# saninsteinn/django-assistant-bot

Measured on AMD Instinct MI355X. Metric: RAG queries/sec + p50 end-to-end latency, bge-base + Llama-3-8B, 1/2/4/8 MI355X, higher is better.
Workload: dtype bf16; 1 GPU; model=bge-base-en + llama-3-8b, global_batch=128, seq_len=1090, parallelism=dp1, mode=batch, index_rows=1000000, index=single shard, local top-k (no collective), sampling=temperature=1.0 top_k=50 top_p=0.95 ignore_eos, graphs=True

## Files before the change

### django_assistant_bot_amd/csrc/bindings.cpp

```cpp
#include <hip/hip_runtime.h>
#include <pybind11/numpy.h>
#include <pybind11/pybind11.h>
#include <pybind11/stl.h>

#include <stdexcept>
#include <string>

#include "kernels/launchers.h"
#include "runtime/json_grammar.h"
#include "runtime/kv_manager.h"
#include "runtime/rag.h"
#include "runtime/tokenizer.h"
#include "runtime/trace.h"

namespace py = pybind11;
using u = uintptr_t;

#define VP(x) reinterpret_cast<void*>(x)
#define CVP(x) reinterpret_cast<const void*>(x)
#define ST(x) reinterpret_cast<hipStream_t>(x)

static void check(int err, const char* name) {
  if (err) throw std::runtime_error(std::string("dab kernel '") + name + "' failed: " + hipGetErrorString((hipError_t)err));
}

PYBIND11_MODULE(_native, m) {
  m.doc() = "MI355X (gfx950) kernels and native runtime of django_assistant_bot_amd";
  m.def("roctx_available", &dab::trace::available);
  m.def("allreduce_signal_bytes", &dab::allreduce_signal_bytes);
  m.def("custom_allreduce", [](const std::vector<uintptr_t>& bases, int rank, u data, long nbytes, long half_bytes,
                               long spin_limit, u s) {
    check(dab::custom_allreduce(bases, rank, VP(data), nbytes, half_bytes, spin_limit, ST(s)), "custom_allreduce");
  });
  m.def("custom_allreduce_rmsnorm", [](const std::vector<uintptr_t>& bases, int rank, u slabs, int S, long slab_stride,
                                       u x, u res_in, u res_out, u out, u w, int rows, int cols, float eps,
                                       long half_bytes, long spin_limit, u s) {
    check(dab::custom_allreduce_rmsnorm(bases, rank, (const float*)slabs, S, slab_stride, CVP(x), CVP(res_in),
                                        VP(res_out), VP(out), CVP(w), rows, cols, eps, half_bytes, spin_limit, ST(s)),
          "custom_allreduce_rmsnorm");
  });
  m.def("allreduce_buffer_alloc", [](long bytes, bool uncached) {
    uintptr_t p = 0;
    check(dab::allreduce_buffer_alloc(bytes, uncached ? 1 : 0, &p), "allreduce_buffer_alloc");
    return p;
  }, py::arg("bytes"), py::arg("uncached") = true);
  m.def("allreduce_buffer_free", [](u ptr) { check(dab::allreduce_buffer_free(ptr), "allreduce_buffer_free"); });
  m.def("ipc_get_handle", [](u ptr) {
    std::string h;
    check(dab::ipc_get_handle(ptr, &h), "ipc_get_handle");
    return py::bytes(h);
  });
  m.def("ipc_open_handle", [](const std::string& h) {
    uintptr_t p = 0;
    check(dab::ipc_open_handle(h, &p), "ipc_open_handle");
    return p;
  });
  m.def("ipc_probe", [](u ptr) { check(dab::ipc_probe(ptr), "ipc_probe"); });
  m.def("ipc_close_handle", [](u ptr) { check(dab::ipc_close_handle(ptr), "ipc_close_handle"); });
  m.def("allreduce_error", &dab::allreduce_error, py::arg("base"), py::arg("clear") = 1);
  m.def("allreduce_error_async", [](u base, u host_word, u s) {
    check(dab::allreduce_error_async(base, VP(host_word), ST(s)), "allreduce_error_async");
  });
  m.def("roctx_push", [](const std::string& name) { return dab::trace::range_push(name.c_str()); });
  m.def("roctx_pop", &dab::trace::range_pop);
  m.def("roctx_mark", [](const std::string& name) { dab::trace::mark(name.c_str()); });

  m.def("rmsnorm", [](u out, u res_out, u x, u res_in, u w, int rows, int cols, float eps, u s) {
    check(dab::rmsnorm(VP(out), VP(res_out), CVP(x), CVP(res_in), CVP(w), rows, cols, eps, ST(s)), "rmsnorm");
  });
  m.def("layernorm", [](u out, u x, u res_in, u gamma, u beta, int rows, int cols, float eps, u s) {
    check(dab::layernorm(VP(out), CVP(x), CVP(res_in), CVP(gamma), CVP(beta), rows, cols, eps, ST(s)), "layernorm");
  });
  m.def("bert_embed", [](u out, u ids, u pos_ids, u type_ids, u word, u pos, u type, u gamma, u beta, int rows, int cols,
                         float eps, u s) {
    check(dab::bert_embed(VP(out), (const int*)ids, (const int*)pos_ids, (const int*)type_ids, CVP(word), CVP(pos),
                          CVP(type), CVP(gamma), CVP(beta), rows, cols, eps, ST(s)),
          "bert_embed");
  });
  m.def("embed_gather", [](u out, u ids, u table, int rows, int cols, u s) {
    check(dab::embed_gather(VP(out), (const int*)ids, CVP(table), rows, cols, ST(s)), "embed_gather");
  });
  m.def("mean_pool", [](u out, u out_bf16, u hidden, u cu, int batch, int cols, int normalize, u s) {
    check(dab::mean_pool((float*)out, VP(out_bf16), CVP(hidden), (const int*)cu, batch, cols, normalize, ST(s)),
          "mean_pool");
  });
  m.def("gelu", [](u out, u x, u bias, size_t rows, int cols, u s) {
    check(dab::gelu(VP(out), CVP(x), CVP(bias), rows, cols, ST(s)), "gelu");
  });
  m.def("silu_mul", [](u out, u x, size_t rows, int F, u s, int interleaved) {
    check(dab::silu_mul(VP(out), CVP(x), rows, F, ST(s), interleaved), "silu_mul");
  }, py::arg("out"), py::arg("x"), py::arg("rows"), py::arg("F"), py::arg("s"), py::arg("interleaved") = 0);
  m.def("rope_kv_write", [](u qkv, int ld, u positions, u cos_sin, u q_out, u k_cache, u v_cache, u slots, int T,
                            int Hq, int Hkv, int D, int block_size, u s, u slabs, int S, long slab_stride,
                            int slab_bf16) {
    check(dab::rope_kv_write(CVP(qkv), ld, (const int*)positions, CVP(cos_sin), VP(q_out), VP(k_cache), VP(v_cache),
                             (const int64_t*)slots, T, Hq, Hkv, D, block_size, ST(s), CVP(slabs), S, slab_stride,
                             slab_bf16),
          "rope_kv_write");
  }, py::arg("qkv"), py::arg("ld"), py::arg("positions"), py::arg("cos_sin"), py::arg("q_out"), py::arg("k_cache"),
     py::arg("v_cache"), py::arg("slots"), py::arg("T"), py::arg("Hq"), py::arg("Hkv"), py::arg("D"),
     py::arg("block_size"), py::arg("s"), py::arg("slabs") = 0, py::arg("S") = 0, py::arg("slab_stride") = 0,
     py::arg("slab_bf16") = 0);
  m.def("rmsnorm_slabs", [](u out, u res_out, u slabs, int S, long slab_stride, u res_in, u w, int rows, int cols,
                            float eps, u s, int slab_bf16) {
    check(dab::rmsnorm_slabs(VP(out), VP(res_out), CVP(slabs), S, slab_stride, CVP(res_in), CVP(w), rows, cols, eps,
                             ST(s), slab_bf16),
          "rmsnorm_slabs");
  }, py::arg("out"), py::arg("res_out"), py::arg("slabs"), py::arg("S"), py::arg("slab_stride"), py::arg("res_in"),
     py::arg("w"), py::arg("rows"), py::arg("cols"), py::arg("eps"), py::arg("s"), py::arg("slab_bf16") = 0);
  m.def("flash_attention",
        [](u q, long qst, long qsh, u k, u v, long kvst, long kvsh, u kc, u vc, u bt, int max_blocks, int bs, u out,
           long ost, long osh, u cu_q, u cu_k, u ctx_k, int batch, int max_sq, int Hq, int Hkv, int D, int causal,
           int paged, float scale, u s) {
          check(dab::flash_attention(CVP(q), qst, qsh, CVP(k), CVP(v), kvst, kvsh, CVP(kc), CVP(vc), (const int*)bt,
                                     max_blocks, bs, VP(out), ost, osh, (const int*)cu_q, (const int*)cu_k,
                                     (const int*)ctx_k, batch, max_sq, Hq, Hkv, D, causal, paged, scale, ST(s)),
                "flash_attention");
        });
  m.def("flash_attention_rope",
        [](u q, long qst, long qsh, u kc, u vc, u bt, int max_blocks, int bs, u out, long ost, long osh, u cu_q,
           u ctx_k, int batch, int max_sq, int Hq, int Hkv, int D, int causal, float scale, u rope_pos, u rope_cs,
           u s) {
          check(dab::flash_attention(CVP(q), qst, qsh, nullptr, nullptr, 0, 0, CVP(kc), CVP(vc), (const int*)bt,
                                     max_blocks, bs, VP(out), ost, osh, (const int*)cu_q, nullptr, (const int*)ctx_k,
                                     batch, max_sq, Hq, Hkv, D, causal, 1, scale, ST(s), (const int*)rope_pos,
                                     CVP(rope_cs)),
                "flash_attention_rope");
        });
  m.def("create_cu_masked_stream", [](std::vector<uint32_t> mask) {
    hipStream_t st = nullptr;
    check(hipExtStreamCreateWithCUMask(&st, (uint32_t)mask.size(), mask.data()), "hipExtStreamCreateWithCUMask");
    return reinterpret_cast<uintptr_t>(st);
  });
  m.def("destroy_stream", [](u s) { check(hipStreamDestroy(ST(s)), "hipStreamDestroy"); });
  m.def("paged_decode_attention", [](u q, u kc, u vc, u bt, int max_blocks, int bs, u ctx, u out, u po, u pm, u pl,
                                     u cnt, int batch, int Hq, int Hkv, int D, int part_size, int max_parts,
                                     float scale, u s, u order, u w0, long w0_bytes, u w1, long w1_bytes,
                                     int w_blocks) {
    dab::L3Warm warm{{(const char*)w0, (const char*)w1}, {w0_bytes, w1_bytes}, w_blocks};
    check(dab::paged_decode_attention(CVP(q), CVP(kc), CVP(vc), (const int*)bt, max_blocks, bs, (const int*)ctx, VP(out),
                                      (float*)po, (float*)pm, (float*)pl, (int*)cnt, batch, Hq, Hkv, D, part_size,
                                      max_parts, scale, ST(s), (const int*)order, &warm),
          "paged_decode_attention");
  }, py::arg("q"), py::arg("kc"), py::arg("vc"), py::arg("bt"), py::arg("max_blocks"), py::arg("bs"), py::arg("ctx"),
     py::arg("out"), py::arg("po"), py::arg("pm"), py::arg("pl"), py::arg("cnt"), py::arg("batch"), py::arg("Hq"),
     py::arg("Hkv"), py::arg("D"), py::arg("part_size"), py::arg("max_parts"), py::arg("scale"), py::arg("s"),
     py::arg("order") = 0, py::arg("w0") = 0, py::arg("w0_bytes") = 0, py::arg("w1") = 0, py::arg("w1_bytes") = 0,
     py::arg("w_blocks") = 0);
  m.def("rope_kv_write_fp8", [](u qkv, int ld, u positions, u cos_sin, u q_out, u k_data, u k_exp, u v_data, u v_exp,
                                u slots, int T, int Hq, int Hkv, int D, int block_size, u s, u slabs, int S,
                                long slab_stride, int slab_bf16) {
    check(dab::rope_kv_write_fp8(CVP(qkv), ld, (const int*)positions, CVP(cos_sin), VP(q_out), VP(k_data), VP(k_exp),
                                 VP(v_data), VP(v_exp), (const int64_t*)slots, T, Hq, Hkv, D, block_size, ST(s),
                                 CVP(slabs), S, slab_stride, slab_bf16),
          "rope_kv_write_fp8");
  }, py::arg("qkv"), py::arg("ld"), py::arg("positions"), py::arg("cos_sin"), py::arg("q_out"), py::arg("k_data"),
     py::arg("k_exp"), py::arg("v_data"), py::arg("v_exp"), py::arg("slots"), py::arg("T"), py::arg("Hq"),
     py::arg("Hkv"), py::arg("D"), py::arg("block_size"), py::arg("s"), py::arg("slabs") = 0, py::arg("S") = 0,
     py::arg("slab_stride") = 0, py::arg("slab_bf16") = 0);
  m.def("kv_fp8_dequant_blocks", [](u k_data, u k_exp, u v_data, u v_exp, u ids, int n, u k_out, u v_out, int Hkv,
                                    int block_size, int D, u s) {
    check(dab::kv_fp8_dequant_blocks(CVP(k_data), CVP(k_exp), CVP(v_data), CVP(v_exp), (const int*)ids, n, VP(k_out),
                                     VP(v_out), Hkv, block_size, D, ST(s)),
          "kv_fp8_dequant_blocks");
  });
  m.def("paged_decode_attention_fp8", [](u q, u k_data, u k_exp, u v_data, u v_exp, u bt, int max_blocks, int bs, u ctx,
                                         u out, u po, u pm, u pl, u cnt, int batch, int Hq, int Hkv, int D,
                                         int part_size, int max_parts, float scale, u s, u order) {
    check(dab::paged_decode_attention_fp8(CVP(q), CVP(k_data), CVP(k_exp), CVP(v_data), CVP(v_exp), (const int*)bt,
                                          max_blocks, bs, (const int*)ctx, VP(out), (float*)po, (float*)pm, (float*)pl,
                                          (int*)cnt, batch, Hq, Hkv, D, part_size, max_parts, scale, ST(s),
                                          (const int*)order),
          "paged_decode_attention_fp8");
  });
  m.def("gemm_bt", [](u A, long lda, u B, long ldb, u C, long ldc, u bias, u residual, long ldr, int M, int N, int K,
                      int epilogue, int out_f32, u row_group, u q_group, u allow, int allow_words, u s, int b_rows,
                      int b_group) {
    check(dab::gemm_bt(CVP(A), lda, CVP(B), ldb, VP(C), ldc, CVP(bias), CVP(residual), ldr, M, N, K, epilogue, out_f32,
                       (const int*)row_group, (const int*)q_group, (const uint32_t*)allow, allow_words, ST(s), b_rows,
                       b_group),
          "gemm_bt");
  }, py::arg("A"), py::arg("lda"), py::arg("B"), py::arg("ldb"), py::arg("C"), py::arg("ldc"), py::arg("bias"),
     py::arg("residual"), py::arg("ldr"), py::arg("M"), py::arg("N"), py::arg("K"), py::arg("epilogue"),
     py::arg("out_f32"), py::arg("row_group"), py::arg("q_group"), py::arg("allow"), py::arg("allow_words"),
     py::arg("s"), py::arg("b_rows") = 0, py::arg("b_group") = 1);
  m.def("gemm_mid_ok", &dab::gemm_mid_ok);
  m.def("gemm_mid_slab_bytes", &dab::gemm_mid_slab_bytes);
  m.def("gemm_mid_counters", &dab::gemm_mid_counters);
  m.def("gemm_mid", [](u A, long lda, u B, u C, long ldc, u residual, long ldr, int M, int N, int K, int epilogue,
                       u slabs, long slab_bytes, u cnt, int n_cnt, u s, int variant, int b_group) {
    check(dab::gemm_mid(CVP(A), lda, CVP(B), VP(C), ldc, CVP(residual), ldr, M, N, K, epilogue, VP(slabs), slab_bytes,
                        (int*)cnt, n_cnt, ST(s), variant, b_group),
          "gemm_mid");
  }, py::arg("A"), py::arg("lda"), py::arg("B"), py::arg("C"), py::arg("ldc"), py::arg("residual"), py::arg("ldr"),
     py::arg("M"), py::arg("N"), py::arg("K"), py::arg("epilogue"), py::arg("slabs"), py::arg("slab_bytes"),
     py::arg("cnt"), py::arg("n_cnt"), py::arg("s"), py::arg("variant") = 0, py::arg("b_group") = 1);
  m.def("gemm256_ok", &dab::gemm256_ok);
  m.def("gemm256_stamped", [](u A, long lda, u B, u C, u bias, u residual, int M, int N, int K, int epilogue,
                              int b_shuf, u stamps, int stamp_tiles, u s, int store_aux) {
    const int r = dab::gemm256_stamped(CVP(A), lda, CVP(B), VP(C), CVP(bias), CVP(residual), M, N, K, epilogue, b_shuf,
                                       VP(stamps), stamp_tiles, ST(s), store_aux);
    if (r < 0) check(-r, "gemm256_stamped");
    return r;
  }, py::arg("A"), py::arg("lda"), py::arg("B"), py::arg("C"), py::arg("bias"), py::arg("residual"), py::arg("M"),
     py::arg("N"), py::arg("K"), py::arg("epilogue"), py::arg("b_shuf"), py::arg("stamps"), py::arg("stamp_tiles"),
     py::arg("s"), py::arg("store_aux") = 0);
  m.def("gemm256_candidates_stamped", [](u A, long lda, u B, int M, int N, int K, int b_rows, u thr, u cnt, u cand_val,
                                          u cand_idx, int cap, u stamps, int stamp_tiles, u s) {
    const int r = dab::gemm256_candidates_stamped(CVP(A), lda, CVP(B), M, N, K, b_rows, (const float*)thr, (int*)cnt,
                                                  (float*)cand_val, (int*)cand_idx, cap, VP(stamps), stamp_tiles, ST(s));
    if (r < 0) check(-r, "gemm256_candidates_stamped");
    return r;
  });
  m.def("gemm256", [](u A, long lda, u B, long ldb, u C, long ldc, u bias, u residual, long ldr, int M, int N, int K,
                      int epilogue, u s, int b_shuf, int b_group, u rows, int src_rows) {
    check(dab::gemm256(CVP(A), lda, CVP(B), ldb, VP(C), ldc, CVP(bias), CVP(residual), ldr, M, N, K, epilogue, ST(s),
                       b_shuf, b_group, reinterpret_cast<const int*>(rows), src_rows),
          "gemm256");
  }, py::arg("A"), py::arg("lda"), py::arg("B"), py::arg("ldb"), py::arg("C"), py::arg("ldc"), py::arg("bias"),
     py::arg("residual"), py::arg("ldr"), py::arg("M"), py::arg("N"), py::arg("K"), py::arg("epilogue"), py::arg("s"),
     py::arg("b_shuf") = 0, py::arg("b_group") = 1, py::arg("rows") = 0, py::arg("src_rows") = 0);
  m.def("gemm_score_candidates", [](u A, long lda, u B, long ldb, int M, int N, int K, u row_group, u q_group, u thr,
                                    u cnt, u cand_val, u cand_idx, int cap, u s) {
    check(dab::gemm_score_candidates(CVP(A), lda, CVP(B), ldb, M, N, K, reinterpret_cast<const int*>(row_group),
                                     reinterpret_cast<const int*>(q_group), reinterpret_cast<const float*>(thr),
                                     reinterpret_cast<int*>(cnt), reinterpret_cast<float*>(cand_val),
                                     reinterpret_cast<int*>(cand_idx), cap, ST(s)),
          "gemm_score_candidates");
  });
  m.def("score_candidates_shuf", [](u A, long lda, u Wshuf, int M, int N, int K, u row_group, u q_group, u thr,
                                    u cnt, u cand_val, u cand_idx, int cap, u s, int b_rows) {
    auto* rg = reinterpret_cast<const int*>(row_group);
    auto* qg = reinterpret_cast<const int*>(q_group);
    auto* th = reinterpret_cast<const float*>(thr);
    auto* ct = reinterpret_cast<int*>(cnt);
    auto* cv = reinterpret_cast<float*>(cand_val);
    auto* ci = reinterpret_cast<int*>(cand_idx);
    int rc = hipErrorInvalidValue;
    if (K % 256 == 0 && ((M <= 64 && K <= 1024) || (M <= 96 && K <= 768)))
      rc = dab::index_scan_candidates_shuf(CVP(A), lda, CVP(Wshuf), M, N, K, rg, qg, th, ct, cv, ci, cap, ST(s));
    else if (M <= 64 || K % 128)
      rc = dab::stream_score_candidates_shuf(CVP(A), lda, CVP(Wshuf), M, N, K, rg, qg, th, ct, cv, ci, cap, ST(s));
    else
      rc = dab::gemm_score_candidates(CVP(A), lda, CVP(Wshuf), K, M, N, K, rg, qg, th, ct, cv, ci, cap, ST(s), b_rows);
    check(rc, "score_candidates_shuf");
  }, py::arg("A"), py::arg("lda"), py::arg("Wshuf"), py::arg("M"), py::arg("N"), py::arg("K"), py::arg("row_group"),
     py::arg("q_group"), py::arg("thr"), py::arg("cnt"), py::arg("cand_val"), py::arg("cand_idx"), py::arg("cap"),
     py::arg("s"), py::arg("b_rows") = 0);
  m.def("stream_gemm", [](u X, long ldx, u W, long ldw, u out, long ldo, u residual, long ldr, int M, int N, int K,
                          int S, int epilogue, u s, int nt, int cfg, float norm_eps, int slab_bf16, int w_group) {
    check(dab::stream_gemm(CVP(X), ldx, CVP(W), ldw, VP(out), ldo, CVP(residual), ldr, M, N, K, S, epilogue, ST(s), nt,
                           cfg, norm_eps, slab_bf16, w_group),
          "stream_gemm");
  }, py::arg("X"), py::arg("ldx"), py::arg("W"), py::arg("ldw"), py::arg("out"), py::arg("ldo"), py::arg("residual"),
     py::arg("ldr"), py::arg("M"), py::arg("N"), py::arg("K"), py::arg("S"), py::arg("epilogue"), py::arg("s"),
     py::arg("nt"), py::arg("cfg"), py::arg("norm_eps") = 0.f, py::arg("slab_bf16") = 0, py::arg("w_group") = 1);
  m.def("stream_gemm_fp8", [](u X, long ldx, u W, u w_exps, u out, long ldo, u residual, long ldr, int M, int N, int K,
                              int S, int epilogue, u s, int nt, int cfg, float norm_eps, int slab_bf16, int w_group) {
    check(dab::stream_gemm_fp8(CVP(X), ldx, CVP(W), CVP(w_exps), VP(out), ldo, CVP(residual), ldr, M, N, K, S, epilogue,
                               ST(s), nt, cfg, norm_eps, slab_bf16, w_group),
          "stream_gemm_fp8");
  }, py::arg("X"), py::arg("ldx"), py::arg("W"), py::arg("w_exps"), py::arg("out"), py::arg("ldo"), py::arg("residual"),
     py::arg("ldr"), py::arg("M"), py::arg("N"), py::arg("K"), py::arg("S"), py::arg("epilogue"), py::arg("s"),
     py::arg("nt"), py::arg("cfg"), py::arg("norm_eps") = 0.f, py::arg("slab_bf16") = 0, py::arg("w_group") = 1);
  m.def("stream_gemm_fp8_ok", &dab::stream_gemm_fp8_ok);
  m.def("stream_gemm_fp8_nwin", &dab::stream_gemm_fp8_nwin);
  m.def("stream_gemm_fp8_set_deep", &dab::stream_gemm_fp8_set_deep);
  m.def("stream_gemm_fp8_deep", &dab::stream_gemm_fp8_deep);
  m.def("stream_gemm_bn", &dab::stream_gemm_bn);
  m.def("stream_gemm_max_m", &dab::stream_gemm_max_m);
  m.def("stream_gemm_set_slice_xcd", &dab::stream_gemm_set_slice_xcd);
  m.def("stream_gemm_slice_xcd", &dab::stream_gemm_slice_xcd);
  m.def("stream_gemm_shuffled", &dab::stream_gemm_shuffled);
  m.def("slab_reduce", [](u out, long ldo, u slabs, int S, int M, int N, u residual, long ldr, u s, int slab_bf16) {
    check(dab::slab_reduce(VP(out), ldo, CVP(slabs), S, M, N, CVP(residual), ldr, ST(s), slab_bf16), "slab_reduce");
  }, py::arg("out"), py::arg("ldo"), py::arg("slabs"), py::arg("S"), py::arg("M"), py::arg("N"), py::arg("residual"),
     py::arg("ldr"), py::arg("s"), py::arg("slab_bf16") = 0);
  m.def("sample_tokens", [](u logits, int f32, long ld, int rows, int vocab, u temp, u top_k, u top_p,
                            unsigned long long seed, u counters, u out_tokens, u out_logprobs, u s) {
    check(dab::sample_tokens(CVP(logits), f32, ld, rows, vocab, (const float*)temp, (const int*)top_k,
                             (const float*)top_p, seed, (int64_t*)counters, (int*)out_tokens, (float*)out_logprobs,
                             ST(s)),
          "sample_tokens");
  });
  m.def("topk_rows", [](u scores, long ld, int rows, int n, int k, u out_vals, u out_idx, long long base, u out_idx64,
                        u s) {
    check(dab::topk_rows((const float*)scores, ld, rows, n, k, (float*)out_vals, (int*)out_idx, base,
                         (int64_t*)out_idx64, ST(s)),
          "topk_rows");
  });

  m.def("sample_tokens_2stage", [](u logits, int f32, long ld, int rows, int vocab, u temp, u top_k, u top_p,
                                   unsigned long long seed, u counters, u out_tokens, u ws, size_t ws_bytes, u s) {
    check(dab::sample_tokens_2stage(CVP(logits), f32, ld, rows, vocab, (const float*)temp, (const int*)top_k,
                                    (const float*)top_p, seed, (int64_t*)counters, (int*)out_tokens, VP(ws), ws_bytes,
                                    ST(s)),
          "sample_tokens_2stage");
  });
  m.def("mask_logits", [](u logits, int f32, long ld, int rows, int vocab, u mask, int words, u row_flags, u s,
                          long mask_ld) {
    check(dab::mask_logits(VP(logits), f32, ld, rows, vocab, (const uint32_t*)mask, words, (const int*)row_flags,
                           ST(s), mask_ld),
          "mask_logits");
  });
  m.def("sample_candidates", [](u logits, int f32, long ld, int rows, int vocab, int base, u keys, u idx, int ncand,
                                u s) {
    check(dab::sample_candidates(CVP(logits), f32, ld, rows, vocab, base, (uint32_t*)keys, (int*)idx, ncand, ST(s)),
          "sample_candidates");
  });
  m.def("sample_merge", [](u keys, u idx, int ncand, int rows, int vocab, u temp, u top_k, u top_p,
                           unsigned long long seed, u counters, u out_tokens, u s) {
    check(dab::sample_merge((const uint32_t*)keys, (const int*)idx, ncand, rows, vocab, (const float*)temp,
                            (const int*)top_k, (const float*)top_p, seed, (int64_t*)counters, (int*)out_tokens, ST(s)),
          "sample_merge");
  });
  m.def("topk_rows_2stage", [](u scores, long ld, int rows, int n, int k, u out_vals, u out_idx, long long base,
                               u out_idx64, u ws, size_t ws_bytes, u s) {
    check(dab::topk_rows_2stage((const float*)scores, ld, rows, n, k, (float*)out_vals, (int*)out_idx, base,
                                (int64_t*)out_idx64, VP(ws), ws_bytes, ST(s)),
          "topk_rows_2stage");
  });

  py::class_<dab::TokenizerConfig>(m, "TokenizerConfig")
      .def(py::init<>())
      .def_readwrite("vocab_size", &dab::TokenizerConfig::vocab_size)
      .def_readwrite("first_id", &dab::TokenizerConfig::first_id)
      .def_readwrite("last_id", &dab::TokenizerConfig::last_id)
      .def_readwrite("pad_id", &dab::TokenizerConfig::pad_id)
      .def_readwrite("unk_id", &dab::TokenizerConfig::unk_id)
      .def_readwrite("cls_id", &dab::TokenizerConfig::cls_id)
      .def_readwrite("sep_id", &dab::TokenizerConfig::sep_id)
      .def_readwrite("max_word_chars", &dab::TokenizerConfig::max_word_chars);
  py::class_<dab::HashTokenizer>(m, "HashTokenizer")
      .def(py::init<const dab::TokenizerConfig&>())
      .def("encode", &dab::HashTokenizer::encode, py::arg("text"), py::arg("add_special") = true,
           py::arg("max_len") = 0)
      .def(
          "encode_batch",
          [](const dab::HashTokenizer& t, const std::vector<std::string>& texts, bool add_special, int max_len,
             int threads) {
            std::vector<int32_t> ids;
            std::vector<int64_t> offs;
            {
              py::gil_scoped_release rel;
              t.encode_batch(texts, add_special, max_len, threads, ids, offs);
            }
            py::array_t<int32_t> a(ids.size());
            std::copy(ids.begin(), ids.end(), a.mutable_data());
            py::array_t<int64_t> o(offs.size());
            std::copy(offs.begin(), offs.end(), o.mutable_data());
            return py::make_tuple(a, o);
          },
          py::arg("texts"), py::arg("add_special") = true, py::arg("max_len") = 0, py::arg("threads") = 8)
      .def("decode", &dab::HashTokenizer::decode, py::arg("ids"), py::arg("skip_special") = true)
      .def("token_texts",
           [](const dab::HashTokenizer& t) {
             py::list out;
             for (const auto& w : t.token_texts()) out.append(py::bytes(w));
             return out;
           })
      .def_static("count_words", &dab::HashTokenizer::count_words);

  py::class_<dab::JsonVocab, std::shared_ptr<dab::JsonVocab>>(m, "JsonVocab")
      .def(py::init([](const std::vector<py::bytes>& toks, const std::vector<int32_t>& eos) {
             std::vector<std::string> t;
             t.reserve(toks.size());
             for (const auto& b : toks) t.emplace_back(b);
             return std::make_shared<dab::JsonVocab>(t, eos);
           }),
           py::arg("tokens"), py::arg("eos_ids"))
      .def("vocab_size", &dab::JsonVocab::vocab_size)
      .def("words", &dab::JsonVocab::words)
      .def("trie_nodes", &dab::JsonVocab::trie_nodes)
      .def("cache_entries", &dab::JsonVocab::cache_entries);
  py::class_<dab::JsonMatcher>(m, "JsonMatcher")
      .def(py::init<std::shared_ptr<dab::JsonVocab>, int, int>(), py::arg("vocab"), py::arg("max_depth") = 24,
           py::arg("max_ws") = 8)
      .def("fill_mask",
           [](dab::JsonMatcher& j, int remaining, u out) {
             py::gil_scoped_release rel;
             return j.fill_mask(remaining, (uint32_t*)out);
           })
      .def("advance", &dab::JsonMatcher::advance)
      .def("done", &dab::JsonMatcher::done)
      .def("broken", &dab::JsonMatcher::broken)
      .def("completion", [](const dab::JsonMatcher& j) { return py::bytes(j.completion()); })
      .def("completion_len", &dab::JsonMatcher::completion_len)
      .def("text", [](const dab::JsonMatcher& j) { return py::bytes(j.text()); });
  py::class_<dab::SchemaAutomaton, std::shared_ptr<dab::SchemaAutomaton>>(m, "SchemaAutomaton")
      .def(py::init<std::shared_ptr<dab::JsonVocab>, int, int, const std::vector<int32_t>&,
                    const std::vector<std::vector<int32_t>>&, const std::vector<std::vector<int32_t>>&>(),
           py::arg("vocab"), py::arg("n_states"), py::arg("start"), py::arg("accept"), py::arg("edges"),
           py::arg("eps"))
      .def("dfa_states", &dab::SchemaAutomaton::dfa_states)
      .def("accepts", [](dab::SchemaAutomaton& a, const py::bytes& b) {
        int d = a.start();
        for (unsigned char c : std::string(b)) {
          d = a.step(d, c);
          if (d < 0) return false;
        }
        return a.accepting(d);
      });
  py::class_<dab::SchemaMatcher>(m, "SchemaMatcher")
      .def(py::init<std::shared_ptr<dab::SchemaAutomaton>>(), py::arg("automaton"))
      .def("fill_mask",
           [](dab::SchemaMatcher& j, int remaining, u out) {
             py::gil_scoped_release rel;
             return j.fill_mask(remaining, (uint32_t*)out);
           })
      .def("advance", &dab::SchemaMatcher::advance)
      .def("done", &dab::SchemaMatcher::done)
      .def("broken", &dab::SchemaMatcher::broken)
      .def("completion_len", &dab::SchemaMatcher::completion_len)
      .def("text", [](const dab::SchemaMatcher& j) { return py::bytes(j.text()); });
  m.def("json_accepts", [](const py::bytes& b, bool complete, int max_depth, int max_ws) {
    return dab::json_accepts(std::string(b), complete, max_depth, max_ws);
  }, py::arg("bytes"), py::arg("complete") = true, py::arg("max_depth") = 64, py::arg("max_ws") = 255);

  py::class_<dab::KVBlockManager>(m, "KVBlockManager")
      .def(py::init<int, int, bool>(), py::arg("num_blocks"), py::arg("block_size"), py::arg("prefix_cache") = true)
      .def("add_sequence", &dab::KVBlockManager::add_sequence)
      .def("extend", &dab::KVBlockManager::extend)
      .def("append_tokens", &dab::KVBlockManager::append_tokens)
      .def("commit_prefix", &dab::KVBlockManager::commit_prefix)
      .def("free_sequence", &dab::KVBlockManager::free_sequence)
      .def("has", &dab::KVBlockManager::has)
      .def("num_tokens", &dab::KVBlockManager::num_tokens)
      .def("capacity_tokens", &dab::KVBlockManager::capacity_tokens)
      .def("num_free_blocks", &dab::KVBlockManager::num_free_blocks)
      .def("num_blocks", &dab::KVBlockManager::num_blocks)
      .def("block_size", &dab::KVBlockManager::block_size)
      .def("prefix_hits", &dab::KVBlockManager::prefix_hits)
      .def("blocks", &dab::KVBlockManager::blocks)
      .def("slot_mapping_into",
           [](const dab::KVBlockManager& k, int64_t seq, int start, int n, u out) {
             k.slot_mapping(seq, start, n, (int64_t*)out);
           })
      .def("prepare_decode_into",
           [](dab::KVBlockManager& k, const std::vector<int64_t>& seqs, const std::vector<int32_t>& toks,
              int max_blocks, u ids, u pos, u slots, u ctx, u bt) {
             return k.prepare_decode(seqs, toks, max_blocks, (int32_t*)ids, (int32_t*)pos, (int64_t*)slots,
                                     (int32_t*)ctx, (int32_t*)bt);
           })
      .def("block_table_into", [](const dab::KVBlockManager& k, const std::vector<int64_t>& seqs, int max_blocks,
                                  u out) { k.block_table(seqs, max_blocks, (int32_t*)out); });

  m.def(
      "aggregate_documents",
      [](py::array_t<float, py::array::c_style | py::array::forcecast> dist,
         py::array_t<int64_t, py::array::c_style | py::array::forcecast> doc_ids, int max_scores_n, int top_n) {
        if (dist.size() != doc_ids.size()) throw std::invalid_argument("distances / doc_ids length mismatch");
        auto r = dab::aggregate_documents(dist.data(), doc_ids.data(), (int)dist.size(), max_scores_n, top_n);
        py::list out;
        for (auto& d : r) out.append(py::make_tuple(d.doc_id, d.score));
        return out;
      },
      py::arg("distances"), py::arg("doc_ids"), py::arg("max_scores_n"), py::arg("top_n"));
  m.def(
      "merge_topk",
      [](py::array_t<float, py::array::c_style | py::array::forcecast> vals,
         py::array_t<int64_t, py::array::c_style | py::array::forcecast> ids, int k_out) {
        if (vals.ndim() != 2 || ids.ndim() != 2 || vals.shape(0) != ids.shape(0) || vals.shape(1) != ids.shape(1))
          throw std::invalid_argument("vals / ids must be [S, k] arrays of the same shape");
        const int S = (int)vals.shape(0), k = (int)vals.shape(1);
        py::array_t<float> ov(k_out);
        py::array_t<int64_t> oi(k_out);
        dab::merge_topk(vals.data(), ids.data(), S, k, k_out, ov.mutable_data(), oi.mutable_data());
        return py::make_tuple(ov, oi);
      },
      py::arg("vals"), py::arg("ids"), py::arg("k_out"));
}
```

### django_assistant_bot_amd/csrc/kernels/launchers.h

```cpp
#pragma once
#include <hip/hip_runtime.h>
#include <stddef.h>
#include <stdint.h>

#include <string>
#include <vector>

namespace dab {

inline int div_up_host(int a, int b) { return (a + b - 1) / b; }

struct L3Warm {
  const char* ptr[2];
  long bytes[2];
  int blocks;
};

int rmsnorm(void* out, void* res_out, const void* x, const void* res_in, const void* w, int rows, int cols, float eps,
            hipStream_t s);
int rmsnorm_slabs(void* out, void* res_out, const void* slabs, int S, long slab_stride, const void* res_in,
                  const void* w, int rows, int cols, float eps, hipStream_t s, int slab_bf16 = 0);
int layernorm(void* out, const void* x, const void* res_in, const void* gamma, const void* beta, int rows, int cols,
              float eps, hipStream_t s);
int bert_embed(void* out, const int* ids, const int* pos_ids, const int* type_ids, const void* word, const void* pos,
               const void* type, const void* gamma, const void* beta, int rows, int cols, float eps, hipStream_t s);
int embed_gather(void* out, const int* ids, const void* table, int rows, int cols, hipStream_t s);
int mean_pool(float* out, void* out_bf16, const void* hidden, const int* cu_seqlens, int batch, int cols,
              int normalize, hipStream_t s);

int gelu(void* out, const void* x, const void* bias, size_t rows, int cols, hipStream_t s);
int silu_mul(void* out, const void* x, size_t rows, int F, hipStream_t s, int interleaved = 0);
int rope_kv_write(const void* qkv, int ld, const int* positions, const void* cos_sin, void* q_out, void* k_cache,
                  void* v_cache, const int64_t* slots, int T, int Hq, int Hkv, int D, int block_size, hipStream_t s,
                  const void* slabs = nullptr, int S = 0, long slab_stride = 0, int slab_bf16 = 0);

int flash_attention(const void* q, long q_stride_tok, long q_stride_head, const void* k, const void* v,
                    long kv_stride_tok, long kv_stride_head, const void* k_cache, const void* v_cache,
                    const int* block_tables, int max_blocks, int block_size, void* out, long o_stride_tok,
                    long o_stride_head, const int* cu_q, const int* cu_k, const int* ctx_k, int batch,
                    int max_seqlen_q, int Hq, int Hkv, int D, int causal, int paged, float scale, hipStream_t s,
                    const int* rope_pos = nullptr, const void* rope_cs = nullptr);
int paged_decode_attention(const void* q, const void* k_cache, const void* v_cache, const int* block_tables,
                           int max_blocks, int block_size, const int* ctx_lens, void* out, float* part_o,
                           float* part_m, float* part_l, int* counters, int batch, int Hq, int Hkv, int D,
                           int part_size, int max_parts, float scale, hipStream_t s,
                           const int* order = nullptr, const L3Warm* warm = nullptr);

int rope_kv_write_fp8(const void* qkv, int ld, const int* positions, const void* cos_sin, void* q_out, void* k_data,
                      void* k_exp, void* v_data, void* v_exp, const int64_t* slots, int T, int Hq, int Hkv, int D,
                      int block_size, hipStream_t s, const void* slabs = nullptr, int S = 0, long slab_stride = 0,
                      int slab_bf16 = 0);
int kv_fp8_dequant_blocks(const void* k_data, const void* k_exp, const void* v_data, const void* v_exp,
                          const int* block_ids, int n, void* k_out, void* v_out, int Hkv, int block_size, int D,
                          hipStream_t s);
int paged_decode_attention_fp8(const void* q, const void* k_data, const void* k_exp, const void* v_data,
                               const void* v_exp, const int* block_tables, int max_blocks, int block_size,
                               const int* ctx_lens, void* out, float* part_o, float* part_m, float* part_l,
                               int* counters, int batch, int Hq, int Hkv, int D, int part_size, int max_parts,
                               float scale, hipStream_t s, const int* order = nullptr);

int gemm_bt(const void* A, long lda, const void* B, long ldb, void* C, long ldc, const void* bias, const void* residual,
            long ldr, int M, int N, int K, int epilogue, int out_f32, const int* row_group, const int* q_group,
            const uint32_t* allow, int allow_words, hipStream_t s, int b_rows = 0, int b_group = 1);

int gemm256_ok(int M, int N, int K, long lda, long ldb);
int gemm256_candidates(const void* A, long lda, const void* B, long ldb, int M, int N, int K, const int* row_group,
                       const int* q_group, const float* thr, int* cnt, float* cand_val, int* cand_idx, int cap,
                       hipStream_t s, int b_rows = 0);
int gemm256_candidates_stamped(const void* A, long lda, const void* B, int M, int N, int K, int b_rows,
                               const float* thr, int* cnt, float* cand_val, int* cand_idx, int cap, void* stamps,
                               int stamp_tiles, hipStream_t s);
int gemm256_stamped(const void* A, long lda, const void* B, void* C, const void* bias, const void* residual, int M,
                    int N, int K, int epilogue, int b_shuf, void* stamps, int stamp_tiles, hipStream_t s, int store_aux);
int gemm256(const void* A, long lda, const void* B, long ldb, void* C, long ldc, const void* bias,
            const void* residual, long ldr, int M, int N, int K, int epilogue, hipStream_t s, int b_shuf = 0,
            int b_group = 1, const int* rows = nullptr, int src_rows = 0);

int gemm_mid_ok(int M, int N, int K, long lda);
long gemm_mid_slab_bytes();
int gemm_mid_counters(int M, int N);
int gemm_mid(const void* A, long lda, const void* B, void* C, long ldc, const void* residual, long ldr, int M, int N,
             int K, int epilogue, void* slabs, long slab_bytes, int* cnt, int n_cnt, hipStream_t s, int variant = 0,
             int b_group = 1);

int stream_gemm(const void* X, long ldx, const void* W, long ldw, void* out, long ldo, const void* residual, long ldr,
                int M, int N, int K, int S, int epilogue, hipStream_t s, int nt_weights, int cfg, float norm_eps = 0.f,
                int slab_bf16 = 0, int w_group = 1);
int stream_gemm_bn(int cfg);
int stream_gemm_fp8(const void* X, long ldx, const void* W, const void* w_exps, void* out, long ldo,
                    const void* residual, long ldr, int M, int N, int K, int S, int epilogue, hipStream_t s,
                    int nt_weights, int cfg, float norm_eps = 0.f, int slab_bf16 = 0, int w_group = 1);
int stream_gemm_fp8_ok(int cfg);
int stream_gemm_fp8_nwin(int cfg);
void stream_gemm_fp8_set_deep(int on);
int stream_gemm_fp8_deep();
int slab_reduce(void* out, long ldo, const void* slabs, int S, int M, int N, const void* residual, long ldr,
                hipStream_t s, int slab_bf16 = 0);
int index_scan_candidates(const void* X, long ldx, const void* W, long ldw, int M, int N, int K, const int* row_group,
                          const int* q_group, const float* thr, int* cnt, float* cand_val, int* cand_idx, int cap,
                          hipStream_t s);
int index_scan_candidates_shuf(const void* X, long ldx, const void* W, int M, int N, int K, const int* row_group,
                               const int* q_group, const float* thr, int* cnt, float* cand_val, int* cand_idx,
                               int cap, hipStream_t s);
int stream_score_candidates(const void* X, long ldx, const void* W, long ldw, int M, int N, int K, const int* row_group,
                            const int* q_group, const float* thr, int* cnt, float* cand_val, int* cand_idx, int cap,
                            hipStream_t s);
int stream_score_candidates_shuf(const void* X, long ldx, const void* W, int M, int N, int K, const int* row_group,
                                 const int* q_group, const float* thr, int* cnt, float* cand_val, int* cand_idx,
                                 int cap, hipStream_t s);
int stream_gemm_max_m(int cfg);
void stream_gemm_set_slice_xcd(int on);
int stream_gemm_slice_xcd();
int stream_gemm_shuffled(int cfg);

int mask_logits(void* logits, int logits_f32, long ld, int rows, int vocab, const uint32_t* mask, int words,
                const int* row_flags, hipStream_t s, long mask_ld = 0);
int sample_candidates(const void* logits, int logits_f32, long ld, int rows, int vocab, int index_base,
                      uint32_t* cand_key, int* cand_idx, int ncand, hipStream_t s);
int sample_merge(const uint32_t* cand_key, const int* cand_idx, int ncand, int rows, int vocab,
                 const float* temperature, const int* top_k, const float* top_p, unsigned long long seed,
                 int64_t* counters, int* out_tokens, hipStream_t s);
int sample_tokens(const void* logits, int logits_f32, long ld, int rows, int vocab, const float* temperature,
                  const int* top_k, const float* top_p, unsigned long long seed, int64_t* counters, int* out_tokens,
                  float* out_logprobs, hipStream_t s);
int topk_rows(const float* scores, long ld, int rows, int n, int k, float* out_vals, int* out_idx, int64_t index_base,
              int64_t* out_idx64, hipStream_t s);

int sample_tokens_2stage(const void* logits, int logits_f32, long ld, int rows, int vocab, const float* temperature,
                         const int* top_k, const float* top_p, unsigned long long seed, int64_t* counters,
                         int* out_tokens, void* workspace, size_t workspace_bytes, hipStream_t s);
int topk_rows_2stage(const float* scores, long ld, int rows, int n, int k, float* out_vals, int* out_idx,
                     int64_t index_base, int64_t* out_idx64, void* workspace, size_t workspace_bytes, hipStream_t s);

int gemm_score_candidates(const void* A, long lda, const void* B, long ldb, int M, int N, int K, const int* row_group,
                          const int* q_group, const float* thr, int* cnt, float* cand_val, int* cand_idx, int cap,
                          hipStream_t s, int b_rows = 0);

size_t allreduce_signal_bytes();
int custom_allreduce_rmsnorm(const std::vector<uintptr_t>& bases, int rank, const float* slabs, int S,
                             long slab_stride, const void* x, const void* res_in, void* res_out, void* out,
                             const void* w, int rows, int cols, float eps, long half_bytes, long spin_limit,
                             hipStream_t s);
int custom_allreduce(const std::vector<uintptr_t>& bases, int rank, void* data, long nbytes, long half_bytes,
                     long spin_limit, hipStream_t s);
int allreduce_buffer_alloc(long bytes, int uncached, uintptr_t* out);
int allreduce_buffer_free(uintptr_t ptr);
int ipc_get_handle(uintptr_t ptr, std::string* handle);
int ipc_open_handle(const std::string& handle, uintptr_t* out);
int ipc_close_handle(uintptr_t ptr);
int ipc_probe(uintptr_t ptr);
int allreduce_error(uintptr_t base, int clear);
int allreduce_error_async(uintptr_t base, void* host_word, hipStream_t s);

}
```

### django_assistant_bot_amd/csrc/kernels/select.hip

```cpp
#include "common.h"
#include "launchers.h"

namespace dab {

constexpr uint32_t kNegInfKey = 0x007FFFFFu;


constexpr int SEL_NT = 1024;
constexpr int SEL_MAXK = 1024;

struct SelShared {
  uint32_t hist[256];
  uint32_t bcast[4];
  uint32_t cnt_gt, cnt_eq;
  uint32_t cand_key[SEL_MAXK];
  int cand_idx[SEL_MAXK];
};

__device__ __forceinline__ int wave_append(uint32_t* counter, bool pred) {
  const unsigned long long m = __ballot(pred);
  if (!m) return -1;
  const int lane = threadIdx.x & 63;
  const int leader = __ffsll((long long)m) - 1;
  uint32_t base = 0;
  if (lane == leader) base = atomicAdd(counter, (uint32_t)__popcll(m));
  base = __shfl(base, leader, 64);
  const unsigned long long below = lane ? (m & ((1ull << lane) - 1ull)) : 0ull;
  return pred ? (int)(base + __popcll(below)) : -1;
}

template <class KeyAt>
__device__ uint32_t radix_kth(KeyAt key_at, int n, int k, SelShared& sh, uint32_t& ties_needed) {
  uint32_t prefix = 0, pmask = 0, kk = (uint32_t)k;
  const int tid = threadIdx.x, lane = tid & 63;
  for (int shift = 24; shift >= 0; shift -= 8) {
    for (int i = tid; i < 256; i += SEL_NT) sh.hist[i] = 0;
    __syncthreads();
    for (int i0 = 0; i0 < n; i0 += SEL_NT) {
      const int i = i0 + tid;
      int bin = -1;
      if (i < n) {
        const uint32_t key = key_at(i);
        if ((key & pmask) == prefix) bin = (int)((key >> shift) & 255u);
      }
      unsigned long long active = __ballot(bin >= 0);
      while (active) {
        const int leader = __ffsll((long long)active) - 1;
        const int lb = __shfl(bin, leader, 64);
        const unsigned long long eq = __ballot(bin == lb);
        if (lane == leader) atomicAdd(&sh.hist[lb], (uint32_t)__popcll(eq));
        active &= ~eq;
      }
    }
    __syncthreads();
    if (tid < 64) {
      uint32_t c[4], sum = 0;
#pragma unroll
      for (int j = 0; j < 4; ++j) {
        c[j] = sh.hist[255 - 4 * tid - j];
        sum += c[j];
      }
      uint32_t incl = sum;
#pragma unroll
      for (int o = 1; o < 64; o <<= 1) {
        const uint32_t t = __shfl_up(incl, o, 64);
        if (tid >= o) incl += t;
      }
      const uint32_t excl = incl - sum;
      if (excl < kk && kk <= incl) {
        uint32_t acc = excl;
#pragma unroll
        for (int j = 0; j < 4; ++j) {
          if (acc + c[j] >= kk) {
            sh.bcast[0] = 255u - 4u * tid - j;
            sh.bcast[1] = kk - acc;
            break;
          }
          acc += c[j];
        }
      }
    }
    __syncthreads();
    const uint32_t digit = sh.bcast[0];
    kk = sh.bcast[1];
    prefix |= digit << shift;
    pmask |= 255u << shift;
    __syncthreads();
  }
  ties_needed = kk;
  return prefix;
}

template <bool TIES_ALL = false, class KeyAt>
__device__ int select_topk(KeyAt key_at, int n, int k, SelShared& sh) {
  const int tid = threadIdx.x;
  uint32_t ties;
  const uint32_t kth = radix_kth(key_at, n, k, sh, ties);
  const uint32_t n_gt0 = (uint32_t)k - ties;
  if (TIES_ALL && kth > kNegInfKey) ties = (uint32_t)SEL_MAXK - n_gt0;
  if (tid == 0) {
    sh.cnt_gt = 0;
    sh.cnt_eq = 0;
  }
  __syncthreads();
  const uint32_t n_gt = n_gt0;
  for (int i0 = 0; i0 < n; i0 += SEL_NT) {
    const int i = i0 + tid;
    uint32_t key = 0;
    if (i < n) key = key_at(i);
    const int pg = wave_append(&sh.cnt_gt, i < n && key > kth);
    if (pg >= 0) {
      sh.cand_key[pg] = key;
      sh.cand_idx[pg] = i;
    }
    const int pe = wave_append(&sh.cnt_eq, i < n && key == kth);
    if (pe >= 0 && (uint32_t)pe < ties) {
      sh.cand_key[n_gt + pe] = key;
      sh.cand_idx[n_gt + pe] = i;
    }
  }
  __syncthreads();
  if (TIES_ALL) k = (int)(n_gt + min(sh.cnt_eq, ties));
  int P = 1;
  while (P < k) P <<= 1;
  for (int i = k + tid; i < P; i += SEL_NT) {
    sh.cand_key[i] = 0u;
    sh.cand_idx[i] = 0x7fffffff;
  }
  __syncthreads();
  for (int size = 2; size <= P; size <<= 1) {
    for (int stride = size >> 1; stride > 0; stride >>= 1) {
      for (int t = tid; t < P; t += SEL_NT) {
        const int u = t ^ stride;
        if (u > t) {
          const bool desc = (t & size) == 0;
          const uint32_t ka = sh.cand_key[t], kb = sh.cand_key[u];
          const int ia = sh.cand_idx[t], ib = sh.cand_idx[u];
          const bool a_first = ka > kb || (ka == kb && ia < ib);
          if (a_first != desc) {
            sh.cand_key[t] = kb;
            sh.cand_key[u] = ka;
            sh.cand_idx[t] = ib;
            sh.cand_idx[u] = ia;
          }
        }
      }
      __syncthreads();
    }
  }
  return k;
}

__device__ __forceinline__ unsigned long long splitmix64(unsigned long long x) {
  x += 0x9E3779B97F4A7C15ull;
  x = (x ^ (x >> 30)) * 0xBF58476D1CE4E5B9ull;
  x = (x ^ (x >> 27)) * 0x94D049BB133111EBull;
  return x ^ (x >> 31);
}

__global__ __launch_bounds__(SEL_NT) void sample_kernel(const void* __restrict__ logits, int logits_f32, long ld,
                                                        int vocab, const float* __restrict__ temperature,
                                                        const int* __restrict__ top_k,
                                                        const float* __restrict__ top_p, unsigned long long seed,
                                                        int64_t* __restrict__ counters, int* __restrict__ out_tokens,
                                                        float* __restrict__ out_logprobs) {
  __shared__ SelShared sh;
  __shared__ float probs[SEL_MAXK];
  const int row = blockIdx.x;
  const float T = temperature ? temperature[row] : 1.f;
  int k = (T <= 0.f) ? 1 : (top_k && top_k[row] > 0 ? top_k[row] : SEL_MAXK);
  if (k > SEL_MAXK) k = SEL_MAXK;
  if (k > vocab) k = vocab;
  const float P = top_p ? top_p[row] : 1.f;
  const bool f32 = logits_f32 != 0;
  const float* lf = reinterpret_cast<const float*>(logits) + (size_t)row * ld;
  const bf16* lb = reinterpret_cast<const bf16*>(logits) + (size_t)row * ld;
  auto key_at = [&](int i) -> uint32_t { return float_key(f32 ? lf[i] : bf2f(lb[i])); };
  k = select_topk<true>(key_at, vocab, k, sh);
  if (threadIdx.x != 0) return;
  if (T <= 0.f) {
    out_tokens[row] = sh.cand_idx[0];
    if (out_logprobs) out_logprobs[row] = 0.f;
    return;
  }
  const float x0 = key_float(sh.cand_key[0]) / T;
  float total = 0.f;
  for (int i = 0; i < k; ++i) {
    const float e = __expf(key_float(sh.cand_key[i]) / T - x0);
    probs[i] = e;
    total += e;
  }
  int keep = k;
  if (P < 1.f) {
    const float thr = (1.f - P) * total;
    float cum = 0.f;
    keep = k;
    for (int i = k - 1; i >= 1; --i) {
      cum += probs[i];
      if (cum <= thr) keep = i;
      else break;
    }
  }
  float kept = 0.f;
  for (int i = 0; i < keep; ++i) kept += probs[i];
  const long long c = counters ? counters[row] : 0;
  if (counters) counters[row] = c + 1;
  const unsigned long long r =
      splitmix64(seed ^ splitmix64((unsigned long long)c * 0x9E3779B97F4A7C15ull + (unsigned long long)row));
  const float u = (float)(r >> 40) * (1.f / 16777216.f);
  const float target = u * kept;
  float acc = 0.f;
  int pick = keep - 1;
  for (int i = 0; i < keep; ++i) {
    acc += probs[i];
    if (acc > target) {
      pick = i;
      break;
    }
  }
  out_tokens[row] = sh.cand_idx[pick];
  if (out_logprobs) out_logprobs[row] = __logf(probs[pick] / kept);
}

__global__ __launch_bounds__(SEL_NT) void topk_rows_kernel(const float* __restrict__ scores, long ld, int n, int k,
                                                           float* __restrict__ out_vals, int* __restrict__ out_idx,
                                                           int64_t index_base, int64_t* __restrict__ out_idx64) {
  __shared__ SelShared sh;
  const int row = blockIdx.x;
  const float* s = scores + (size_t)row * ld;
  auto key_at = [&](int i) -> uint32_t { return float_key(s[i]); };
  select_topk(key_at, n, k, sh);
  for (int i = threadIdx.x; i < k; i += SEL_NT) {
    out_vals[(size_t)row * k + i] = key_float(sh.cand_key[i]);
    if (out_idx) out_idx[(size_t)row * k + i] = sh.cand_idx[i];
    if (out_idx64) out_idx64[(size_t)row * k + i] = index_base + sh.cand_idx[i];
  }
}


constexpr int CH_NT = 256;
constexpr int CH_FAST_MAXK = 64;
constexpr int CH_FAST_CAP = 512;

struct ChunkFast {
  u32x4 tmax[CH_NT / 4];
  u32x4 kv[CH_FAST_CAP / 2];
  uint32_t n, thr;
};

template <int PT>
__global__ __launch_bounds__(CH_NT) void chunk_topk_kernel(const void* __restrict__ src, int src_bf16, long ld, int n,
                                                           int k, int kc, uint32_t* __restrict__ cand_key,
                                                           int* __restrict__ cand_idx, int index_base = 0) {
  __shared__ uint32_t hist[256];
  __shared__ uint32_t bc[2];
  __shared__ uint32_t cnt[2];
  __shared__ ChunkFast fst;
  const int row = blockIdx.y, c = blockIdx.x, nchunks = gridDim.x;
  const int chunk = CH_NT * PT;
  const int start = c * chunk;
  const int len = min(chunk, n - start);
  const int tid = threadIdx.x, lane = tid & 63;
  const float* sf = reinterpret_cast<const float*>(src) + (size_t)row * ld + start;
  const bf16* sb = reinterpret_cast<const bf16*>(src) + (size_t)row * ld + start;
  static_assert(CH_NT == 256 && PT % 8 == 0, "idx_of assumes 256 threads and whole 16-B vectors");
  const int lg = src_bf16 ? 3 : 2;
  auto idx_of = [&](int j) { return ((j >> lg) << (8 + lg)) + (tid << lg) + (j & ((1 << lg) - 1)); };
  const bool vec_ok = ((reinterpret_cast<uintptr_t>(src_bf16 ? (const void*)sb : (const void*)sf)) & 15) == 0;
  uint32_t key[PT];
  if (src_bf16) {
#pragma unroll
    for (int v = 0; v < PT / 8; ++v) {
      const int i0 = v * (CH_NT * 8) + tid * 8;
      if (vec_ok && i0 + 8 <= len) {
        float f[8];
        unpack8(*reinterpret_cast<const u32x4*>(sb + i0), f);
#pragma unroll
        for (int e = 0; e < 8; ++e) key[8 * v + e] = float_key(f[e]);
      } else {
#pragma unroll
        for (int e = 0; e < 8; ++e) key[8 * v + e] = i0 + e < len ? float_key(bf2f(sb[i0 + e])) : 0u;
      }
    }
  } else {
#pragma unroll
    for (int v = 0; v < PT / 4; ++v) {
      const int i0 = v * (CH_NT * 4) + tid * 4;
      if (vec_ok && i0 + 4 <= len) {
        const f32x4 f = *reinterpret_cast<const f32x4*>(sf + i0);
#pragma unroll
        for (int e = 0; e < 4; ++e) key[4 * v + e] = float_key(f[e]);
      } else {
#pragma unroll
        for (int e = 0; e < 4; ++e) key[4 * v + e] = i0 + e < len ? float_key(sf[i0 + e]) : 0u;
      }
    }
  }
  const int kk = min(k, len);
  uint32_t* ok = cand_key + ((size_t)row * nchunks + c) * kc;
  int* oi = cand_idx + ((size_t)row * nchunks + c) * kc;
  if (kk <= CH_FAST_MAXK) {
    uint32_t m = 0;
#pragma unroll
    for (int j = 0; j < PT; ++j)
      if (idx_of(j) < len) m = max(m, key[j]);
    reinterpret_cast<uint32_t*>(fst.tmax)[tid] = m;
    if (tid == 0) fst.n = 0;
    __syncthreads();
    int rank = 0;
#pragma unroll 4
    for (int j4 = 0; j4 < CH_NT / 4; ++j4) {
      const u32x4 o4 = fst.tmax[j4];
#pragma unroll
      for (int e = 0; e < 4; ++e) rank += (o4[e] > m) || (o4[e] == m && 4 * j4 + e < tid);
    }
    if (rank == kk - 1) fst.thr = m;
    __syncthreads();
    const uint32_t t = fst.thr;
#pragma unroll
    for (int j = 0; j < PT; ++j) {
      const int i = idx_of(j);
      const int slot = wave_append(&fst.n, i < len && key[j] >= t);
      if (slot >= 0 && slot < CH_FAST_CAP) {
        uint32_t* e2 = reinterpret_cast<uint32_t*>(fst.kv) + 2 * slot;
        e2[0] = key[j];
        e2[1] = (uint32_t)(index_base + start + i);
      }
    }
    __syncthreads();
    const int ns = (int)fst.n;
    if (ns <= CH_FAST_CAP) {
      const int ns8 = min(CH_FAST_CAP, (ns + 7) & ~7);
      if (tid < ns8 - ns) {
        uint32_t* e2 = reinterpret_cast<uint32_t*>(fst.kv) + 2 * (ns + tid);
        e2[0] = 0u;
        e2[1] = 0xffffffffu;
      }
      __syncthreads();
      for (int a = tid; a < ns; a += CH_NT) {
        const uint32_t* ea = reinterpret_cast<const uint32_t*>(fst.kv) + 2 * a;
        const uint32_t ka = ea[0], ia = ea[1];
        int r = 0;
        for (int u2 = 0; u2 < ns8 / 2; u2 += 4) {
          u32x4 q[4];
#pragma unroll
          for (int z = 0; z < 4; ++z) q[z] = fst.kv[u2 + z];
#pragma unroll
          for (int z = 0; z < 4; ++z) {
            r += (q[z][0] > ka) || (q[z][0] == ka && q[z][1] < ia);
            r += (q[z][2] > ka) || (q[z][2] == ka && q[z][3] < ia);
          }
        }
        if (r < kk) {
          ok[r] = ka;
          oi[r] = (int)ia;
        }
      }
      for (int i = kk + tid; i < kc; i += CH_NT) {
        ok[i] = 0u;
        oi[i] = -1;
      }
      return;
    }
    __syncthreads();
  }
  uint32_t prefix = 0, pmask = 0, need = (uint32_t)kk;
  for (int shift = 24; shift >= 0; shift -= 8) {
    for (int i = tid; i < 256; i += CH_NT) hist[i] = 0;
    __syncthreads();
#pragma unroll
    for (int j = 0; j < PT; ++j) {
      const int i = idx_of(j);
      const int bin = (i < len && (key[j] & pmask) == prefix) ? (int)((key[j] >> shift) & 255u) : -1;
      const int b0 = __builtin_amdgcn_readfirstlane(bin);
      if (__all(bin == b0)) {
        if (lane == 0 && b0 >= 0) atomicAdd(&hist[b0], 64u);
      } else if (bin >= 0) {
        atomicAdd(&hist[bin], 1u);
      }
    }
    __syncthreads();
    if (tid < 64) {
      uint32_t cc[4], sum = 0;
#pragma unroll
      for (int j = 0; j < 4; ++j) {
        cc[j] = hist[255 - 4 * tid - j];
        sum += cc[j];
      }
      uint32_t incl = sum;
#pragma unroll
      for (int o = 1; o < 64; o <<= 1) {
        const uint32_t t = __shfl_up(incl, o, 64);
        if (tid >= o) incl += t;
      }
      const uint32_t excl = incl - sum;
      if (excl < need && need <= incl) {
        uint32_t acc = excl;
#pragma unroll
        for (int j = 0; j < 4; ++j) {
          if (acc + cc[j] >= need) {
            bc[0] = 255u - 4u * tid - j;
            bc[1] = need - acc;
            break;
          }
          acc += cc[j];
        }
      }
    }
    __syncthreads();
    prefix |= bc[0] << shift;
    pmask |= 255u << shift;
    need = bc[1];
    __syncthreads();
  }
  if (tid == 0) {
    cnt[0] = 0;
    cnt[1] = 0;
  }
  __syncthreads();
  const uint32_t n_gt = (uint32_t)kk - need;
#pragma unroll
  for (int j = 0; j < PT; ++j) {
    const int i = idx_of(j);
    const bool valid = i < len;
    const int pg = wave_append(&cnt[0], valid && key[j] > prefix);
    if (pg >= 0) {
      ok[pg] = key[j];
      oi[pg] = index_base + start + i;
    }
    const int pe = wave_append(&cnt[1], valid && key[j] == prefix);
    if (pe >= 0 && (uint32_t)pe < need) {
      ok[n_gt + pe] = key[j];
      oi[n_gt + pe] = index_base + start + i;
    }
  }
  for (int i = kk + tid; i < kc; i += CH_NT) {
    ok[i] = 0u;
    oi[i] = -1;
  }
}

__global__ __launch_bounds__(SEL_NT) void sample_merge_kernel(const uint32_t* __restrict__ cand_key,
                                                              const int* __restrict__ cand_idx, int ncand,
                                                              const float* __restrict__ temperature,
                                                              const int* __restrict__ top_k,
                                                              const float* __restrict__ top_p, int vocab,
                                                              unsigned long long seed, int64_t* __restrict__ counters,
                                                              int* __restrict__ out_tokens) {
  __shared__ uint32_t skey[SEL_MAXK];
  __shared__ int sidx[SEL_MAXK];
  __shared__ float probs[SEL_MAXK];
  const int row = blockIdx.x, tid = threadIdx.x;
  const float T = temperature ? temperature[row] : 1.f;
  int k = (T <= 0.f) ? 1 : (top_k && top_k[row] > 0 ? top_k[row] : 64);
  k = min(k, min(64, vocab));
  const int nc = min(ncand, SEL_MAXK);
  for (int i = tid; i < SEL_MAXK; i += SEL_NT) {
    skey[i] = i < ncand ? cand_key[(size_t)row * ncand + i] : 0u;
    sidx[i] = i < ncand ? cand_idx[(size_t)row * ncand + i] : 0x7fffffff;
  }
  __syncthreads();
  for (int size = 2; size <= SEL_MAXK; size <<= 1) {
    for (int stride = size >> 1; stride > 0; stride >>= 1) {
      for (int t = tid; t < SEL_MAXK; t += SEL_NT) {
        const int u2 = t ^ stride;
        if (u2 > t) {
          const bool desc = (t & size) == 0;
          const uint32_t ka = skey[t], kb = skey[u2];
          const int ia = sidx[t], ib = sidx[u2];
          const bool a_first = ka > kb || (ka == kb && ia < ib);
          if (a_first != desc) {
            skey[t] = kb;
            skey[u2] = ka;
            sidx[t] = ib;
            sidx[u2] = ia;
          }
        }
      }
      __syncthreads();
    }
  }
  if (tid != 0) return;
  if (T <= 0.f) {
    out_tokens[row] = sidx[0];
    return;
  }
  while (k < nc && skey[k] == skey[k - 1] && skey[k] > kNegInfKey) ++k;
  const float P = top_p ? top_p[row] : 1.f;
  const float x0 = key_float(skey[0]) / T;
  float total = 0.f;
  for (int i = 0; i < k; ++i) {
    const float e = __expf(key_float(skey[i]) / T - x0);
    probs[i] = e;
    total += e;
  }
  int keep = k;
  if (P < 1.f) {
    const float thr = (1.f - P) * total;
    float cum = 0.f;
    for (int i = k - 1; i >= 1; --i) {
      cum += probs[i];
      if (cum <= thr) keep = i;
      else break;
    }
  }
  float kept = 0.f;
  for (int i = 0; i < keep; ++i) kept += probs[i];
  const long long cval = counters ? counters[row] : 0;
  if (counters) counters[row] = cval + 1;
  const unsigned long long r =
      splitmix64(seed ^ splitmix64((unsigned long long)cval * 0x9E3779B97F4A7C15ull + (unsigned long long)row));
  const float uu = (float)(r >> 40) * (1.f / 16777216.f);
  const float target = uu * kept;
  float acc = 0.f;
  int pick = keep - 1;
  for (int i = 0; i < keep; ++i) {
    acc += probs[i];
    if (acc > target) {
      pick = i;
      break;
    }
  }
  out_tokens[row] = sidx[pick];
}

__global__ __launch_bounds__(SEL_NT) void topk_merge_kernel(const uint32_t* __restrict__ cand_key,
                                                            const int* __restrict__ cand_idx, int ncand, int k,
                                                            float* __restrict__ out_vals, int* __restrict__ out_idx,
                                                            int64_t index_base, int64_t* __restrict__ out_idx64) {
  __shared__ SelShared sh;
  const int row = blockIdx.x;
  const uint32_t* ck = cand_key + (size_t)row * ncand;
  const int* ci = cand_idx + (size_t)row * ncand;
  auto key_at = [&](int i) -> uint32_t { return ck[i]; };
  select_topk(key_at, ncand, k, sh);
  for (int i = threadIdx.x; i < k; i += SEL_NT) {
    const int pos = sh.cand_idx[i];
    const int idx = (pos >= 0 && pos < ncand) ? ci[pos] : -1;
    out_vals[(size_t)row * k + i] = key_float(sh.cand_key[i]);
    if (out_idx) out_idx[(size_t)row * k + i] = idx;
    if (out_idx64) out_idx64[(size_t)row * k + i] = idx >= 0 ? index_base + idx : -1;
  }
}

int sample_tokens_2stage(const void* logits, int logits_f32, long ld, int rows, int vocab, const float* temperature,
                         const int* top_k, const float* top_p, unsigned long long seed, int64_t* counters,
                         int* out_tokens, void* workspace, size_t workspace_bytes, hipStream_t s) {
  if (rows <= 0) return 0;
  constexpr int PT = 32, KC = 64;
  const int chunk = CH_NT * PT;
  const int nchunks = (vocab + chunk - 1) / chunk;
  const int ncand = nchunks * KC;
  const size_t need = (size_t)rows * ncand * 8;
  if (ncand > SEL_MAXK || workspace_bytes < need) return hipErrorInvalidValue;
  uint32_t* ck = reinterpret_cast<uint32_t*>(workspace);
  int* ci = reinterpret_cast<int*>(ck + (size_t)rows * ncand);
  hipLaunchKernelGGL(chunk_topk_kernel<PT>, dim3(nchunks, rows), dim3(CH_NT), 0, s, logits, logits_f32 ? 0 : 1, ld,
                     vocab, KC, KC, ck, ci);
  hipLaunchKernelGGL(sample_merge_kernel, dim3(rows), dim3(SEL_NT), 0, s, ck, ci, ncand, temperature, top_k, top_p,
                     vocab, seed, counters, out_tokens);
  return hipGetLastError();
}

int sample_candidates(const void* logits, int logits_f32, long ld, int rows, int vocab, int index_base,
                      uint32_t* cand_key, int* cand_idx, int ncand, hipStream_t s) {
  if (rows <= 0) return 0;
  constexpr int PT = 32, KC = 64;
  const int nchunks = (vocab + CH_NT * PT - 1) / (CH_NT * PT);
  if (vocab <= 0 || ncand != nchunks * KC) return hipErrorInvalidValue;
  hipLaunchKernelGGL(chunk_topk_kernel<PT>, dim3(nchunks, rows), dim3(CH_NT), 0, s, logits, logits_f32 ? 0 : 1, ld,
                     vocab, KC, KC, cand_key, cand_idx, index_base);
  return hipGetLastError();
}

int sample_merge(const uint32_t* cand_key, const int* cand_idx, int ncand, int rows, int vocab,
                 const float* temperature, const int* top_k, const float* top_p, unsigned long long seed,
                 int64_t* counters, int* out_tokens, hipStream_t s) {
  if (rows <= 0) return 0;
  if (ncand <= 0 || ncand > SEL_MAXK) return hipErrorInvalidValue;
  hipLaunchKernelGGL(sample_merge_kernel, dim3(rows), dim3(SEL_NT), 0, s, cand_key, cand_idx, ncand, temperature, top_k,
                     top_p, vocab, seed, counters, out_tokens);
  return hipGetLastError();
}

int topk_rows_2stage(const float* scores, long ld, int rows, int n, int k, float* out_vals, int* out_idx,
                     int64_t index_base, int64_t* out_idx64, void* workspace, size_t workspace_bytes, hipStream_t s) {
  if (rows <= 0) return 0;
  if (k < 1 || k > SEL_MAXK || k > n) return hipErrorInvalidValue;
  constexpr int PT = 32;
  const int chunk = CH_NT * PT;
  const int kc = ((k + 63) / 64) * 64;
  const int nchunks = (n + chunk - 1) / chunk;
  const int ncand = nchunks * kc;
  if (workspace_bytes < (size_t)rows * ncand * 8) return hipErrorInvalidValue;
  uint32_t* ck = reinterpret_cast<uint32_t*>(workspace);
  int* ci = reinterpret_cast<int*>(ck + (size_t)rows * ncand);
  hipLaunchKernelGGL(chunk_topk_kernel<PT>, dim3(nchunks, rows), dim3(CH_NT), 0, s, scores, 0, ld, n, k, kc, ck, ci);
  hipLaunchKernelGGL(topk_merge_kernel, dim3(rows), dim3(SEL_NT), 0, s, ck, ci, ncand, k, out_vals, out_idx,
                     index_base, out_idx64);
  return hipGetLastError();
}

__global__ __launch_bounds__(256) void mask_logits_kernel(void* __restrict__ logits, int logits_f32, long ld,
                                                          int vocab, const uint32_t* __restrict__ mask, int words,
                                                          long mask_ld, const int* __restrict__ row_flags) {
  const int row = blockIdx.y;
  if (row_flags[row] == 0) return;
  const int w = blockIdx.x * 256 + threadIdx.x;
  if (w >= words) return;
  const uint32_t bits = mask[(size_t)row * mask_ld + w];
  if (bits == 0xFFFFFFFFu) return;
  const int t0 = w * 32, n = min(32, vocab - t0);
  if (logits_f32) {
    float* l = reinterpret_cast<float*>(logits) + (size_t)row * ld + t0;
    for (int j = 0; j < n; ++j)
      if (!((bits >> j) & 1u)) l[j] = -INFINITY;
  } else {
    bf16* l = reinterpret_cast<bf16*>(logits) + (size_t)row * ld + t0;
    for (int j = 0; j < n; ++j)
      if (!((bits >> j) & 1u)) l[j] = f2bf(-INFINITY);
  }
}

int mask_logits(void* logits, int logits_f32, long ld, int rows, int vocab, const uint32_t* mask, int words,
                const int* row_flags, hipStream_t s, long mask_ld) {
  if (rows <= 0) return 0;
  if (mask_ld <= 0) mask_ld = words;
  if (vocab <= 0 || words * 32 < vocab || mask_ld < words) return hipErrorInvalidValue;
  hipLaunchKernelGGL(mask_logits_kernel, dim3((words + 255) / 256, rows), dim3(256), 0, s, logits, logits_f32, ld,
                     vocab, mask, words, mask_ld, row_flags);
  return hipGetLastError();
}

int sample_tokens(const void* logits, int logits_f32, long ld, int rows, int vocab, const float* temperature,
                  const int* top_k, const float* top_p, unsigned long long seed, int64_t* counters, int* out_tokens,
                  float* out_logprobs, hipStream_t s) {
  if (rows <= 0) return 0;
  if (vocab <= 0) return hipErrorInvalidValue;
  hipLaunchKernelGGL(sample_kernel, dim3(rows), dim3(SEL_NT), 0, s, logits, logits_f32, ld, vocab, temperature, top_k,
                     top_p, seed, counters, out_tokens, out_logprobs);
  return hipGetLastError();
}

int topk_rows(const float* scores, long ld, int rows, int n, int k, float* out_vals, int* out_idx, int64_t index_base,
              int64_t* out_idx64, hipStream_t s) {
  if (rows <= 0) return 0;
  if (k < 1 || k > SEL_MAXK || k > n) return hipErrorInvalidValue;
  hipLaunchKernelGGL(topk_rows_kernel, dim3(rows), dim3(SEL_NT), 0, s, scores, ld, n, k, out_vals, out_idx, index_base,
                     out_idx64);
  return hipGetLastError();
}

}
```

### django_assistant_bot_amd/csrc/runtime/kv_manager.cpp

```cpp
#include "kv_manager.h"

#include <algorithm>
#include <functional>
#include <iterator>
#include <stdexcept>

namespace dab {

KVBlockManager::KVBlockManager(int num_blocks, int block_size, bool prefix_cache)
    : num_blocks_(num_blocks), block_size_(block_size), prefix_cache_(prefix_cache) {
  if (num_blocks <= 0 || block_size <= 0) throw std::invalid_argument("num_blocks and block_size must be > 0");
  free_.reserve(num_blocks);
  for (int b = 0; b < num_blocks; ++b) free_.push_back(b);
  lru_cap_ = std::max(64, num_blocks / 4);
  ref_.assign(num_blocks, 0);
  block_hash_.assign(num_blocks, 0);
  lru_pos_.resize(num_blocks);
  in_lru_.assign(num_blocks, 0);
}

uint64_t KVBlockManager::chain_hash(uint64_t parent, const int32_t* toks, int n) const {
  uint64_t h = parent ^ 0x9E3779B97F4A7C15ull;
  for (int i = 0; i < n; ++i) {
    h ^= (uint64_t)(uint32_t)toks[i] + 0x9E3779B97F4A7C15ull + (h << 6) + (h >> 2);
    h *= 0x100000001B3ull;
  }
  return h ? h : 1;
}

int32_t KVBlockManager::alloc_block() {
  int32_t b;
  if (!free_.empty()) {
    std::pop_heap(free_.begin(), free_.end(), std::greater<int32_t>());
    b = free_.back();
    free_.pop_back();
  } else if (!lru_.empty()) {
    b = lru_.front();
    lru_.pop_front();
    in_lru_[b] = 0;
    cached_.erase(block_hash_[b]);
    block_hash_[b] = 0;
  } else {
    return -1;
  }
  ref_[b] = 1;
  return b;
}

void KVBlockManager::release_block(int32_t b) {
  if (--ref_[b] > 0) return;
  if (prefix_cache_ && block_hash_[b] != 0) {
    lru_.push_back(b);
    lru_pos_[b] = std::prev(lru_.end());
    in_lru_[b] = 1;
    if ((int)lru_.size() > lru_cap_) {
      const int32_t e = lru_.front();
      lru_.pop_front();
      in_lru_[e] = 0;
      cached_.erase(block_hash_[e]);
      block_hash_[e] = 0;
      push_free(e);
    }
  } else {
    block_hash_[b] = 0;
    push_free(b);
  }
}

void KVBlockManager::push_free(int32_t b) {
  free_.push_back(b);
  std::push_heap(free_.begin(), free_.end(), std::greater<int32_t>());
}

int KVBlockManager::add_sequence(int64_t seq_id, const std::vector<int32_t>& tokens, int reserve) {
  if (seqs_.count(seq_id)) throw std::invalid_argument("sequence already registered");
  const int n = (int)tokens.size();
  const int need_tokens = n + (reserve > 0 ? reserve : 0);
  const int need_blocks = (need_tokens + block_size_ - 1) / block_size_;
  std::vector<int32_t> hit_blocks;
  std::vector<uint64_t> hit_hashes;
  if (prefix_cache_ && n > 1) {
    const int max_full = (n - 1) / block_size_;
    uint64_t h = 0;
    for (int i = 0; i < max_full; ++i) {
      h = chain_hash(h, tokens.data() + (size_t)i * block_size_, block_size_);
      auto it = cached_.find(h);
      if (it == cached_.end()) break;
      hit_blocks.push_back(it->second);
      hit_hashes.push_back(h);
    }
  }
  int reused_from_lru = 0;
  for (int32_t b : hit_blocks) reused_from_lru += in_lru_[b] ? 1 : 0;
  const int fresh = need_blocks - (int)hit_blocks.size();
  if (fresh > num_free_blocks() - reused_from_lru) return -1;
  Seq s;
  for (int32_t b : hit_blocks) {
    if (in_lru_[b]) {
      lru_.erase(lru_pos_[b]);
      in_lru_[b] = 0;
    }
    ++ref_[b];
    s.blocks.push_back(b);
  }
  s.hashes = hit_hashes;
  for (int i = 0; i < fresh; ++i) s.blocks.push_back(alloc_block());
  s.tokens = tokens;
  const int cached_tokens = (int)hit_blocks.size() * block_size_;
  prefix_hits_ += cached_tokens;
  seqs_.emplace(seq_id, std::move(s));
  return cached_tokens;
}

bool KVBlockManager::extend(int64_t seq_id, int n) {
  auto it = seqs_.find(seq_id);
  if (it == seqs_.end()) throw std::invalid_argument("unknown sequence");
  Seq& s = it->second;
  const int need = (int)s.tokens.size() + n;
  const int need_blocks = (need + block_size_ - 1) / block_size_;
  const int more = need_blocks - (int)s.blocks.size();
  if (more <= 0) return true;
  if (more > num_free_blocks()) return false;
  for (int i = 0; i < more; ++i) s.blocks.push_back(alloc_block());
  return true;
}

void KVBlockManager::append_tokens(int64_t seq_id, const std::vector<int32_t>& tokens) {
  auto it = seqs_.find(seq_id);
  if (it == seqs_.end()) throw std::invalid_argument("unknown sequence");
  Seq& s = it->second;
  s.tokens.insert(s.tokens.end(), tokens.begin(), tokens.end());
  if ((int)s.tokens.size() > (int)s.blocks.size() * block_size_) throw std::runtime_error("KV capacity exceeded");
}

void KVBlockManager::commit_prefix(int64_t seq_id, int n_computed) {
  if (!prefix_cache_) return;
  auto it = seqs_.find(seq_id);
  if (it == seqs_.end()) return;
  Seq& s = it->second;
  const int full = std::min<int>(n_computed, (int)s.tokens.size()) / block_size_;
  uint64_t h = s.hashes.empty() ? 0 : s.hashes.back();
  for (int i = (int)s.hashes.size(); i < full && i < (int)s.blocks.size(); ++i) {
    h = chain_hash(h, s.tokens.data() + (size_t)i * block_size_, block_size_);
    s.hashes.push_back(h);
    const int32_t b = s.blocks[i];
    if (block_hash_[b] == 0 && !cached_.count(h)) {
      block_hash_[b] = h;
      cached_[h] = b;
    }
  }
}

void KVBlockManager::free_sequence(int64_t seq_id) {
  auto it = seqs_.find(seq_id);
  if (it == seqs_.end()) return;
  for (int32_t b : it->second.blocks) release_block(b);
  seqs_.erase(it);
}

int KVBlockManager::num_tokens(int64_t seq_id) const {
  auto it = seqs_.find(seq_id);
  return it == seqs_.end() ? 0 : (int)it->second.tokens.size();
}

int KVBlockManager::capacity_tokens(int64_t seq_id) const {
  auto it = seqs_.find(seq_id);
  return it == seqs_.end() ? 0 : (int)it->second.blocks.size() * block_size_;
}

const std::vector<int32_t>& KVBlockManager::blocks(int64_t seq_id) const {
  auto it = seqs_.find(seq_id);
  if (it == seqs_.end()) throw std::invalid_argument("unknown sequence");
  return it->second.blocks;
}

void KVBlockManager::slot_mapping(int64_t seq_id, int start, int n, int64_t* out) const {
  const auto& bl = blocks(seq_id);
  for (int i = 0; i < n; ++i) {
    const int pos = start + i;
    const int bi = pos / block_size_;
    if (bi >= (int)bl.size()) throw std::out_of_range("slot beyond allocated blocks");
    out[i] = (int64_t)bl[bi] * block_size_ + (pos % block_size_);
  }
}

int KVBlockManager::prepare_decode(const std::vector<int64_t>& seq_ids, const std::vector<int32_t>& tokens,
                                   int max_blocks, int32_t* ids, int32_t* pos, int64_t* slots, int32_t* ctx,
                                   int32_t* block_table) {
  if (seq_ids.size() != tokens.size()) throw std::invalid_argument("seq_ids / tokens length mismatch");
  for (size_t i = 0; i < seq_ids.size(); ++i)
    if (!extend(seq_ids[i], 1)) return (int)i;
  for (size_t i = 0; i < seq_ids.size(); ++i) {
    Seq& s = seqs_.at(seq_ids[i]);
    s.tokens.push_back(tokens[i]);
    const int p = (int)s.tokens.size() - 1;
    ids[i] = tokens[i];
    pos[i] = p;
    slots[i] = (int64_t)s.blocks[p / block_size_] * block_size_ + (p % block_size_);
    ctx[i] = p + 1;
    if ((int)s.blocks.size() > max_blocks) throw std::out_of_range("block table wider than max_blocks");
    int32_t* row = block_table + i * (size_t)max_blocks;
    std::copy(s.blocks.begin(), s.blocks.end(), row);
    std::fill(row + s.blocks.size(), row + max_blocks, 0);
  }
  return -1;
}

void KVBlockManager::block_table(const std::vector<int64_t>& seq_ids, int max_blocks, int32_t* out) const {
  for (size_t r = 0; r < seq_ids.size(); ++r) {
    int32_t* row = out + r * max_blocks;
    int i = 0;
    if (seq_ids[r] >= 0) {
      const auto& bl = blocks(seq_ids[r]);
      if ((int)bl.size() > max_blocks) throw std::out_of_range("block table wider than max_blocks");
      for (; i < (int)bl.size(); ++i) row[i] = bl[i];
    }
    for (; i < max_blocks; ++i) row[i] = 0;
  }
}

}
```

### django_assistant_bot_amd/csrc/runtime/kv_manager.h

```cpp
#pragma once
#include <cstdint>
#include <list>
#include <unordered_map>
#include <vector>

namespace dab {

class KVBlockManager {
 public:
  KVBlockManager(int num_blocks, int block_size, bool prefix_cache);

  int add_sequence(int64_t seq_id, const std::vector<int32_t>& tokens, int reserve);
  bool extend(int64_t seq_id, int n);
  void append_tokens(int64_t seq_id, const std::vector<int32_t>& tokens);
  void commit_prefix(int64_t seq_id, int n_computed);
  void free_sequence(int64_t seq_id);

  bool has(int64_t seq_id) const { return seqs_.count(seq_id) != 0; }
  int num_tokens(int64_t seq_id) const;
  int capacity_tokens(int64_t seq_id) const;
  int num_free_blocks() const { return (int)free_.size() + (int)lru_.size(); }
  int num_blocks() const { return num_blocks_; }
  int block_size() const { return block_size_; }
  int64_t prefix_hits() const { return prefix_hits_; }
  const std::vector<int32_t>& blocks(int64_t seq_id) const;

  int prepare_decode(const std::vector<int64_t>& seq_ids, const std::vector<int32_t>& tokens, int max_blocks,
                     int32_t* ids, int32_t* pos, int64_t* slots, int32_t* ctx, int32_t* block_table);
  void slot_mapping(int64_t seq_id, int start, int n, int64_t* out) const;
  void block_table(const std::vector<int64_t>& seq_ids, int max_blocks, int32_t* out) const;

 private:
  struct Seq {
    std::vector<int32_t> blocks;
    std::vector<int32_t> tokens;
    std::vector<uint64_t> hashes;
  };
  int num_blocks_, block_size_;
  bool prefix_cache_;
  std::vector<int32_t> free_;
  int lru_cap_ = 64;
  std::vector<int32_t> ref_;
  std::vector<uint64_t> block_hash_;
  std::unordered_map<uint64_t, int32_t> cached_;
  std::list<int32_t> lru_;
  std::vector<std::list<int32_t>::iterator> lru_pos_;
  std::vector<char> in_lru_;
  std::unordered_map<int64_t, Seq> seqs_;
  int64_t prefix_hits_ = 0;

  int32_t alloc_block();
  void push_free(int32_t b);
  void release_block(int32_t b);
  uint64_t chain_hash(uint64_t parent, const int32_t* toks, int n) const;
};

}
```

### django_assistant_bot_amd/engine/llm_engine.py

```python
from __future__ import annotations

import itertools
import math
import os
import time
from collections import deque
from dataclasses import dataclass, field

import numpy as np
import torch

from .. import ops
from ..models import AttnMeta, KVCache, LlamaModel, decoder_config, random_decoder_weights
from ..models.configs import DecoderConfig
from ..ops._lib import native
from ..utils import trace
from .tokenizer import Tokenizer


@dataclass
class SamplingParams:
    max_new_tokens: int = 1024
    temperature: float = 1.0
    top_k: int = 50
    top_p: float = 0.95
    ignore_eos: bool = False
    max_length: int | None = None
    seed: int | None = None
    stop_token_ids: tuple = ()
    do_sample: bool = True
    timeout_s: float | None = None
    json_mode: bool = False
    json_schema: dict | str | None = None


@dataclass
class GenerationOutput:
    request_id: int
    prompt_ids: list
    token_ids: list
    text: str
    finish_reason: str
    usage: dict
    timings: dict


@dataclass
class _Req:
    rid: int
    prompt: list
    params: SamplingParams
    arrival: float
    out: list = field(default_factory=list)
    computed: int = 0
    admitted: bool = False
    first_token_t: float = 0.0
    finish_t: float = 0.0
    finish_reason: str = ""
    rng_base: int = 0
    prefill_s: float = 0.0
    preempted: int = 0
    matcher: object = None

    @property
    def seq(self):
        return self.rid

    def full_prompt(self):
        return self.prompt + self.out if self.preempted else self.prompt




def _bucket_sizes(max_batch):
    b = [1, 2, 4, 8, 16, 24, 32, 48, 64, 96, 128, 160, 192, 224, 256, 320, 384, 448, 512]
    return [x for x in b if x < max_batch] + [max_batch]


class LLMEngine:
    def __init__(self, model: str | DecoderConfig = "llama-3-8b", device=None, weights: dict | None = None,
                 checkpoint: str | None = None, seed: int = 0, max_batch: int = 256, block_size: int = 64,
                 max_model_len: int | None = None, kv_cache_gb: float | None = None, num_blocks: int | None = None,
                 max_prefill_tokens: int = 16384, use_graphs: bool = True, prefix_cache: bool = True,
                 tp_group=None, tp_size: int = 1, tp_rank: int = 0, interleaved_mlp: bool = True,
                 part_size: int = 512, kv_memory_fraction: float = 0.85, mixed_prefill_tokens: int = 0,
                 pipeline_decode: bool = True, shared_model: LlamaModel | None = None,
                 kv_cache_dtype: str | None = None, kv_scratch_blocks: int | None = None,
                 weight_dtype: str | None = None):
        self.cfg = decoder_config(model) if isinstance(model, str) else model
        cfg = self.cfg
        if shared_model is not None:
            have = getattr(shared_model, "weight_dtype", "bf16")
            if weight_dtype is not None and weight_dtype != have:
                raise ValueError(f"weight_dtype={weight_dtype!r} conflicts with the shared model's {have!r}")
            weight_dtype = have
        elif weight_dtype is None:
            weight_dtype = os.environ.get("DAB_WEIGHT_DTYPE") or "bf16"
        if weight_dtype not in ("bf16", "fp8"):
            raise ValueError(f"weight_dtype must be 'bf16' or 'fp8', got {weight_dtype!r}")
        if weight_dtype == "fp8" and tp_size > 1:
            raise ValueError("weight_dtype='fp8' does not support tensor parallelism (tp_size > 1) yet")
        self.weight_dtype = weight_dtype
        if kv_cache_dtype is None:
            kv_cache_dtype = os.environ.get("DAB_KV_CACHE_DTYPE") or "bf16"
        if kv_cache_dtype not in ("bf16", "fp8"):
            raise ValueError(f"kv_cache_dtype must be 'bf16' or 'fp8', got {kv_cache_dtype!r}")
        if kv_cache_dtype == "fp8" and tp_size > 1:
            raise ValueError("kv_cache_dtype='fp8' does not support tensor parallelism (tp_size > 1) yet")
        self.kv_cache_dtype = kv_cache_dtype
        if checkpoint is None and weights is None and shared_model is None:
            from ..models.configs import checkpoint_dir

            checkpoint = checkpoint_dir(model)
        self.device = torch.device(device if device is not None else ("cuda" if torch.cuda.is_available() else "cpu"))
        self.is_gpu = self.device.type == "cuda"
        if kv_cache_dtype == "fp8" and self.is_gpu and cfg.head_dim != 128:
            raise ValueError(f"kv_cache_dtype='fp8' needs head_dim 128 on the GPU (model has {cfg.head_dim})")
        self.tp_group, self.tp_size, self.tp_rank = tp_group, tp_size, tp_rank
        own_weights = weights is None
        if shared_model is not None:
            weights = {}
        elif weights is None:
            if checkpoint:
                from ..models import load_decoder_checkpoint

                weights = load_decoder_checkpoint(checkpoint, cfg, tp_rank=tp_rank, tp_size=tp_size,
                                                  interleave_mlp=interleaved_mlp)
            else:
                weights = random_decoder_weights(cfg, self.device, seed=seed, tp_rank=tp_rank, tp_size=tp_size,
                                                 interleave_mlp=interleaved_mlp)
        if shared_model is not None:
            self.model = shared_model
        else:
            self.model = LlamaModel(cfg, weights, self.device, tp_group=tp_group, tp_size=tp_size,
                                    interleaved_mlp=interleaved_mlp, consume=own_weights, tp_rank=tp_rank,
                                    weight_dtype=weight_dtype)
        del weights
        if self.is_gpu and shared_model is None:
            torch.cuda.empty_cache()
        if tp_size > 1 and self.is_gpu and shared_model is None:
            from ..parallel.custom_allreduce import maybe_create

            self.model.custom_ar = maybe_create(tp_group, self.device, tp_size)
        self.tokenizer = Tokenizer.for_decoder(cfg, checkpoint)
        self.max_batch = max_batch
        self.block_size = block_size
        self.max_model_len = min(max_model_len or cfg.max_position, cfg.max_position)
        self.max_blocks_per_seq = math.ceil(self.max_model_len / block_size)
        self.max_prefill_tokens = max_prefill_tokens
        self.mixed_prefill_tokens = mixed_prefill_tokens
        self.part_size = part_size
        self.long_part_size = max(part_size, 2048)
        hkv = cfg.kv_heads // tp_size
        fp8 = kv_cache_dtype == "fp8"
        per_block = KVCache.bytes_per_block(cfg.layers, hkv, block_size, cfg.head_dim, kv_dtype=kv_cache_dtype)
        scratch = 0
        if fp8 and self.is_gpu:
            scratch = kv_scratch_blocks or (math.ceil(max(max_prefill_tokens, self.max_model_len) / block_size) + max_batch)
            scratch = max(int(scratch), self.max_blocks_per_seq)
        if num_blocks is None:
            if kv_cache_gb:
                num_blocks = int(kv_cache_gb * (1 << 30) // per_block)
            elif self.is_gpu:
                free, _ = torch.cuda.mem_get_info(self.device)
                free -= KVCache.scratch_bytes(scratch, hkv, block_size, cfg.head_dim)
                num_blocks = int(free * kv_memory_fraction // per_block)
            else:
                num_blocks = 4 * self.max_blocks_per_seq
            num_blocks = max(2, min(num_blocks, max_batch * self.max_blocks_per_seq + 8))
        self.kv = KVCache(cfg.layers, num_blocks, hkv, block_size, cfg.head_dim, self.device, kv_dtype=kv_cache_dtype,
                          scratch_blocks=scratch)
        self.blocks = native().KVBlockManager(num_blocks, block_size, prefix_cache)
        self._prefix_cache = prefix_cache
        self.seed = seed
        self.waiting: deque[_Req] = deque()
        self.prefilling: list[_Req] = []
        self.running: list[_Req] = []
        self.finished: dict[int, _Req] = {}
        self._ids = itertools.count()
        self.stats = {"prefill_tokens": 0, "decode_tokens": 0, "decode_steps": 0, "prefill_steps": 0,
                      "preemptions": 0, "graph_replays": 0, "mixed_steps": 0,
                      "kv_cache_bits": 8 if fp8 else 16,
                      "weight_bits": 8 if weight_dtype == "fp8" else 16}
        self.use_graphs = use_graphs and self.is_gpu
        dev = self.device
        mb = max_batch
        self._d_ids = torch.zeros(mb, dtype=torch.int32, device=dev)
        self._d_pos = torch.zeros(mb, dtype=torch.int32, device=dev)
        self._d_slots = torch.full((mb,), -1, dtype=torch.int64, device=dev)
        self._d_ctx = torch.ones(mb, dtype=torch.int32, device=dev)
        self._d_bt = torch.zeros((mb, self.max_blocks_per_seq), dtype=torch.int32, device=dev)
        self._d_temp = torch.ones(mb, dtype=torch.float32, device=dev)
        self._d_topk = torch.full((mb,), 50, dtype=torch.int32, device=dev)
        self._d_topp = torch.ones(mb, dtype=torch.float32, device=dev)
        self._d_cnt = torch.zeros(mb, dtype=torch.int64, device=dev)
        self._d_tokens = torch.zeros(mb, dtype=torch.int32, device=dev)
        self._d_order = torch.arange(mb, dtype=torch.int32, device=dev)
        pin = self.is_gpu
        mk = lambda *a, **k: torch.zeros(*a, **k, pin_memory=pin)
        self._h_ids = mk(mb, dtype=torch.int32)
        self._h_pos = mk(mb, dtype=torch.int32)
        self._h_slots = mk(mb, dtype=torch.int64)
        self._h_ctx = mk(mb, dtype=torch.int32)
        self._h_bt = mk((mb, self.max_blocks_per_seq), dtype=torch.int32)
        self._h_temp = mk(mb, dtype=torch.float32)
        self._h_topk = mk(mb, dtype=torch.int32)
        self._h_topp = mk(mb, dtype=torch.float32)
        self._h_cnt = mk(mb, dtype=torch.int64)
        self._h_tokens = mk(mb, dtype=torch.int32)
        self._h_order = mk(mb, dtype=torch.int32)
        self.pipeline_decode = bool(pipeline_decode) and tp_size == 1
        self._h_alt = {k: mk(*(getattr(self, k).shape,), dtype=getattr(self, k).dtype)
                       for k in ("_h_ids", "_h_pos", "_h_slots", "_h_ctx", "_h_bt", "_h_temp", "_h_topk", "_h_topp",
                                 "_h_cnt", "_h_tokens", "_h_order")}
        self._inflight = None
        self._d_mask = None
        self._masked = False
        self._pending_prefill = None
        max_parts = math.ceil(self.max_model_len / part_size)
        self._workspace = ops.DecodeWorkspace(mb, cfg.heads // tp_size, cfg.head_dim, max_parts, dev) if self.is_gpu \
            else None
        self._sample_ws = ops.kernels.sample_workspace(mb, cfg.vocab_size, dev) if self.is_gpu else None
        self.vp = bool(getattr(self.model, "vocab_parallel", False))
        self._vp_cand = None
        if self.vp and self.is_gpu:
            ncl = ops.kernels.sample_candidates_per_row(self.model.vocab_local)
            self._vp_cand = torch.zeros((2, mb, ncl), dtype=torch.int32, device=dev)
        self._graphs: dict = {}
        self._buckets = _bucket_sizes(max_batch)
        self._graph_pool = None
        self.timer = trace.GpuTimer(enabled=self.is_gpu)
        self.fault_hook = None
        self.auto_expire = True

    def add_request(self, prompt_ids: list, params: SamplingParams | None = None, request_id: int | None = None) -> int:
        params = params or SamplingParams()
        rid = next(self._ids) if request_id is None else request_id
        prompt = [int(t) for t in prompt_ids]
        if not prompt:
            prompt = [self.cfg.bos_id]
        if len(prompt) >= self.max_model_len:
            prompt = prompt[-(self.max_model_len - 1):]
        seed = params.seed if params.seed is not None else self.seed
        r = _Req(rid, prompt, params, time.perf_counter(), rng_base=((seed * 1000003 + rid) & 0xFFFFFFFF) << 20)
        r.matcher = self.check_params(params, matcher=True)
        if r.matcher is not None:
            self._ensure_mask_buffers()
        self.waiting.append(r)
        return rid

    def check_params(self, params: SamplingParams, matcher: bool = False):
        if params.json_schema is not None and self.tokenizer.byte_exact:
            from .json_schema import automaton_for, matcher_for

            if not matcher:
                automaton_for(self.tokenizer, self.cfg.eos_ids, params.json_schema)
                return None
            return matcher_for(self.tokenizer, self.cfg.eos_ids, params.json_schema)
        if params.json_mode or params.json_schema is not None:
            from .json_constraint import matcher_for

            if params.json_schema is not None:
                from .json_schema import compile_schema

                compile_schema(params.json_schema)
            return matcher_for(self.tokenizer, self.cfg.eos_ids) if matcher else None
        return None

    def rejected_output(self, rid: int, prompt_ids, reason: str) -> GenerationOutput:
        return GenerationOutput(request_id=rid, prompt_ids=list(prompt_ids), token_ids=[], text="",
                                finish_reason=f"error: {reason}",
                                usage={"prompt_tokens": len(prompt_ids), "completion_tokens": 0,
                                       "total_tokens": len(prompt_ids)},
                                timings={"queue_s": 0.0, "ttft_s": 0.0, "total_s": 0.0, "decode_s": 0.0,
                                         "prefill_s": 0.0})

    def has_unfinished(self) -> bool:
        return bool(self.waiting or self.prefilling or self.running)

    def generate(self, prompts: list, params: SamplingParams | list | None = None) -> list[GenerationOutput]:
        plist = params if isinstance(params, list) else [params or SamplingParams()] * len(prompts)
        rids = []
        for p, sp in zip(prompts, plist):
            ids = self.tokenizer.encode(p) if isinstance(p, str) else p
            rids.append(self.add_request(ids, sp))
        while self.has_unfinished():
            self.step()
        return [self.pop_output(r) for r in rids]

    def pop_output(self, rid: int) -> GenerationOutput:
        r = self.finished.pop(rid)
        n_out = len(r.out)
        return GenerationOutput(
            request_id=rid, prompt_ids=r.prompt, token_ids=list(r.out),
            text=self.tokenizer.decode(r.out), finish_reason=r.finish_reason,
            usage={"prompt_tokens": len(r.prompt), "completion_tokens": n_out, "total_tokens": len(r.prompt) + n_out},
            timings={"queue_s": max(0.0, r.first_token_t - r.arrival - r.prefill_s),
                     "ttft_s": r.first_token_t - r.arrival, "total_s": r.finish_t - r.arrival,
                     "decode_s": r.finish_t - r.first_token_t, "prefill_s": r.prefill_s},
        )

    def step(self) -> list[int]:
        done_before = set(self.finished)
        if self.fault_hook is not None:
            self.fault_hook(self)
        if self.auto_expire:
            self.expire_deadlines()
        if self._pending_prefill is not None:
            chunks = self._schedule_prefill() if not self.running or self.mixed_prefill_tokens <= 0 else []
            if chunks:
                prev, self._pending_prefill = self._pending_prefill, None
                self._run_prefill(chunks)
                self._finish_prefill(prev)
                return [k for k in self.finished if k not in done_before]
            self._finish_prefill(self._pending_prefill)
            self._pending_prefill = None
        if self._inflight is not None and not self._can_pipeline():
            self._finish_inflight()
        if self._can_pipeline():
            self._step_pipelined()
        elif self.running and self.mixed_prefill_tokens > 0 and (self.waiting or self.prefilling):
            batch = self._reserve_decode()
            chunks = self._schedule_prefill(self.mixed_prefill_tokens) if batch else self._schedule_prefill()
            if chunks and batch:
                self._run_mixed(batch, chunks)
            elif chunks:
                self._run_prefill(chunks)
            elif batch:
                self._run_decode(batch)
        else:
            chunks = self._schedule_prefill()
            if chunks:
                self._run_prefill(chunks)
            elif self.running:
                batch = self._reserve_decode()
                if batch:
                    self._run_decode(batch)
        return [k for k in self.finished if k not in done_before]

    def abort(self, rid: int, reason: str = "abort") -> bool:
        if self._inflight is not None:
            self._finish_inflight()
        if self._pending_prefill is not None:
            pend, self._pending_prefill = self._pending_prefill, None
            self._finish_prefill(pend)
        for q in (self.waiting, self.prefilling, self.running):
            for r in q:
                if r.rid == rid:
                    q.remove(r)
                    if r.admitted:
                        self.blocks.free_sequence(r.seq)
                    r.finish_reason = reason
                    r.finish_t = time.perf_counter()
                    self.finished[rid] = r
                    self.stats["aborted"] = self.stats.get("aborted", 0) + 1
                    return True
        return False

    def fail_all(self) -> list[int]:
        ids = [r.rid for q in (self.waiting, self.prefilling, self.running) for r in q]
        self._inflight = None
        self._pending_prefill = None
        self.waiting.clear()
        self.prefilling.clear()
        self.running.clear()
        self.blocks = native().KVBlockManager(self.blocks.num_blocks(), self.block_size, self._prefix_cache)
        self.timer.collect()
        return ids

    def expired(self) -> list[int]:
        now = time.perf_counter()
        return [r.rid for q in (self.waiting, self.prefilling, self.running) for r in q
                if r.params.timeout_s is not None and now - r.arrival > r.params.timeout_s]

    def expire_deadlines(self) -> list[int]:
        ids = self.expired()
        for rid in ids:
            self.abort(rid, "timeout")
        return ids

    def _schedule_prefill(self, budget: int | None = None):
        budget = self.max_prefill_tokens if budget is None else budget
        chunks = []
        for r in self.prefilling:
            if budget <= 0:
                break
            total = len(r.full_prompt())
            n = min(total - r.computed, budget)
            if n > 0:
                chunks.append((r, r.computed, n))
                self.blocks.commit_prefix(r.seq, r.computed + n)
                budget -= n
        while self.waiting and budget > 0 and len(self.running) + len(self.prefilling) < self.max_batch:
            r = self.waiting[0]
            toks = r.full_prompt()
            cached = self.blocks.add_sequence(r.seq, toks, 1)
            if cached < 0:
                if not self.running and not self.prefilling:
                    raise RuntimeError("KV cache too small for a single request")
                break
            self.waiting.popleft()
            r.admitted = True
            r.computed = cached
            self.prefilling.append(r)
            n = min(len(toks) - cached, budget)
            chunks.append((r, cached, n))
            self.blocks.commit_prefix(r.seq, cached + n)
            budget -= n
        return chunks

    def _build_block_tables(self, seqs, out_host):
        self.blocks.block_table_into(seqs, self.max_blocks_per_seq, out_host.data_ptr())

    def _kv_prefill_plan(self, bt, ctx, cu) -> dict:
        if not (self.kv.fp8 and self.is_gpu):
            return {}
        p = ops.kv_prefill_plan(bt, ctx, cu, self.block_size, self.kv.scratch_blocks, self.device)
        return {"kv_blocks": p.blocks, "kv_scratch_bt": p.scratch_bt, "kv_groups": p.groups}

    def _run_prefill(self, chunks):
        t0 = time.perf_counter()
        B = len(chunks)
        T = sum(n for _, _, n in chunks)
        ids = np.empty(T, dtype=np.int32)
        pos = np.empty(T, dtype=np.int32)
        slots = torch.empty(T, dtype=torch.int64)
        cu = np.zeros(B + 1, dtype=np.int32)
        ctx = np.empty(B, dtype=np.int32)
        o = 0
        for i, (r, s, n) in enumerate(chunks):
            toks = r.full_prompt()
            ids[o:o + n] = toks[s:s + n]
            pos[o:o + n] = np.arange(s, s + n, dtype=np.int32)
            self.blocks.slot_mapping_into(r.seq, s, n, slots.data_ptr() + 8 * o)
            o += n
            cu[i + 1] = o
            ctx[i] = s + n
        bt = torch.zeros((B, self.max_blocks_per_seq), dtype=torch.int32)
        self._build_block_tables([r.seq for r, _, _ in chunks], bt)
        to = self._h2d
        meta = AttnMeta(decode=False, positions=to(pos), slots=to(slots), block_tables=to(bt), ctx_lens=to(ctx),
                        cu_q=to(cu), max_q=max(n for _, _, n in chunks), **self._kv_prefill_plan(bt, ctx, cu))
        last_rows = [i for i, (r, s, n) in enumerate(chunks) if s + n == len(r.full_prompt())]
        if last_rows:
            sel = self._h2d(torch.as_tensor([int(cu[i + 1]) - 1 for i in last_rows], dtype=torch.int32))
        else:
            sel = torch.empty(0, dtype=torch.int32, device=self.device)
        with self.timer.phase("prefill"):
            hidden = self.model.forward(to(ids), meta, self.kv, out_rows=sel)
        self.stats["prefill_tokens"] += T
        self.stats["prefill_steps"] += 1
        reqs, toks = [], []
        if last_rows:
            logits = self.model.logits(hidden)
            reqs = [chunks[i][0] for i in last_rows]
            toks = self._sample(logits, reqs, to_host=not self.is_gpu)
        for r, s, n in chunks:
            r.computed = s + n
            self.blocks.commit_prefix(r.seq, s + n)
        pend = (chunks, reqs, toks, t0)
        self._tp_fault_enqueue()
        if self.is_gpu:
            self._pending_prefill = pend
        else:
            self._finish_prefill(pend)

    def _finish_prefill(self, pend):
        chunks, reqs, toks, t0 = pend
        if torch.is_tensor(toks):
            toks = toks.cpu().tolist()
            self._tp_fault_check()
        self._collect_gpu_times(block=bool(reqs))
        now = time.perf_counter()
        for r, s, n in chunks:
            r.prefill_s += now - t0
        if reqs:
            for r, t in zip(reqs, toks):
                self.blocks.commit_prefix(r.seq, len(r.full_prompt()))
                self.prefilling.remove(r)
                r.first_token_t = r.first_token_t or now
                r.preempted = 0
                self.running.append(r)
                self._accept_token(r, int(t), now)

    def _h2d(self, a):
        t = torch.as_tensor(a)
        if not self.is_gpu:
            return t
        return t.pin_memory().to(self.device, non_blocking=True)

    def _run_mixed(self, batch: list, chunks):
        t0 = time.perf_counter()
        dev = self.device
        B = len(batch)
        P = len(chunks)
        Tp = sum(n for _, _, n in chunks)
        Bp = B + (-(Tp + B)) % 64 if self.is_gpu else B
        Bp = min(Bp, self.max_batch)
        T = Tp + Bp
        ids = torch.empty(T, dtype=torch.int32, pin_memory=self.is_gpu)
        pos = torch.empty(T, dtype=torch.int32, pin_memory=self.is_gpu)
        slots = torch.empty(T, dtype=torch.int64, pin_memory=self.is_gpu)
        cu = np.zeros(P + 1, dtype=np.int32)
        ctx = np.empty(P, dtype=np.int32)
        ids_np, pos_np = ids.numpy(), pos.numpy()
        o = 0
        for i, (r, s, n) in enumerate(chunks):
            toks = r.full_prompt()
            ids_np[o:o + n] = toks[s:s + n]
            pos_np[o:o + n] = np.arange(s, s + n, dtype=np.int32)
            self.blocks.slot_mapping_into(r.seq, s, n, slots.data_ptr() + 8 * o)
            o += n
            cu[i + 1] = o
            ctx[i] = s + n
        if Bp > B:
            self._h_ids[B:Bp] = 0
            self._h_pos[B:Bp] = 0
            self._h_slots[B:Bp] = -1
            self._h_ctx[B:Bp] = 1
            self._h_bt[B:Bp] = 0
        ids[Tp:] = self._h_ids[:Bp]
        pos[Tp:] = self._h_pos[:Bp]
        slots[Tp:] = self._h_slots[:Bp]
        bt = torch.zeros((P, self.max_blocks_per_seq), dtype=torch.int32)
        self._build_block_tables([r.seq for r, _, _ in chunks], bt)
        to = lambda a: torch.as_tensor(a).to(dev, non_blocking=True)
        self._d_ctx[:Bp].copy_(self._h_ctx[:Bp], non_blocking=True)
        self._d_bt[:Bp].copy_(self._h_bt[:Bp], non_blocking=True)
        order = None
        if self.is_gpu:
            self._fill_order(Bp)
            self._d_order[:Bp].copy_(self._h_order[:Bp], non_blocking=True)
            order = self._d_order[:Bp]
        meta = AttnMeta(decode=False, positions=to(pos), slots=to(slots), block_tables=to(bt), ctx_lens=to(ctx),
                        cu_q=to(cu), max_q=max(n for _, _, n in chunks), workspace=self._workspace,
                        part_size=self._decode_part(Bp), n_decode=Bp, dec_block_tables=self._d_bt[:Bp],
                        dec_ctx_lens=self._d_ctx[:Bp], order=order, **self._kv_prefill_plan(bt, ctx, cu))
        last_rows = [i for i, (r, s, n) in enumerate(chunks) if s + n == len(r.full_prompt())]
        sel = [int(cu[i + 1]) - 1 for i in last_rows] + list(range(Tp, Tp + B))
        sel_d = torch.as_tensor(sel, dtype=torch.int32).to(dev, non_blocking=True)
        with self.timer.phase("mixed"):
            hidden = self.model.forward(to(ids), meta, self.kv, out_rows=sel_d)
        logits = self.model.logits(hidden)
        preqs = [chunks[i][0] for i in last_rows]
        self._tp_fault_enqueue()
        toks = self._sample(logits, preqs + batch)
        self._tp_fault_check()
        self._collect_gpu_times()
        now = time.perf_counter()
        self.stats["prefill_tokens"] += Tp
        self.stats["decode_tokens"] += B
        self.stats["decode_steps"] += 1
        self.stats["mixed_steps"] += 1
        for r, s, n in chunks:
            r.computed = s + n
            r.prefill_s += now - t0
        for r, t in zip(batch, toks[len(preqs):]):
            self._accept_token(r, int(t), now)
        for r, t in zip(preqs, toks[:len(preqs)]):
            self.blocks.commit_prefix(r.seq, len(r.full_prompt()))
            self.prefilling.remove(r)
            r.first_token_t = r.first_token_t or now
            r.preempted = 0
            self.running.append(r)
            self._accept_token(r, int(t), now)

    def _collect_gpu_times(self, block: bool = True):
        for name, ms in self.timer.collect(block).items():
            key = f"gpu_{name}_ms"
            self.stats[key] = self.stats.get(key, 0.0) + ms

    def _ensure_mask_buffers(self) -> None:
        if getattr(self, "_d_mask", None) is not None:
            return
        W = -(-self.cfg.vocab_size // 32)
        mb = self.max_batch
        pin = self.is_gpu
        self._h_masks = [(torch.zeros((mb, W), dtype=torch.int32, pin_memory=pin),
                          torch.zeros(mb, dtype=torch.int32, pin_memory=pin)) for _ in range(2)]
        self._mask_events = [None, None]
        self._mask_turn = 0
        self._d_mask = torch.zeros((mb, W), dtype=torch.int32, device=self.device)
        self._d_mflag = torch.zeros(mb, dtype=torch.int32, device=self.device)

    def _budget(self, r: _Req) -> int:
        n, p = len(r.out), r.params
        left = min(p.max_new_tokens - n, self.max_model_len - len(r.prompt) - n)
        if p.max_length is not None:
            left = min(left, p.max_length - len(r.prompt) - n)
        return max(left, 1)

    def _fill_masks(self, reqs, n_rows: int) -> bool:
        if not any(r.matcher is not None for r in reqs):
            return False
        t = self._mask_turn
        self._mask_turn ^= 1
        if self._mask_events[t] is not None:
            self._mask_events[t].synchronize()
        h_mask, h_flag = self._h_masks[t]
        h_flag[:n_rows] = 0
        row_bytes = h_mask.shape[1] * 4
        base = h_mask.data_ptr()
        for i, r in enumerate(reqs):
            if r.matcher is not None:
                r.matcher.fill_mask(self._budget(r), base + i * row_bytes)
                h_flag[i] = 1
        self._d_mask[:n_rows].copy_(h_mask[:n_rows], non_blocking=True)
        self._d_mflag[:n_rows].copy_(h_flag[:n_rows], non_blocking=True)
        if self.is_gpu:
            ev = torch.cuda.Event()
            ev.record()
            self._mask_events[t] = ev
        return True

    def _mask(self, logits, rows: int):
        m = self.model
        ops.mask_logits(logits, self._d_mask[:rows], self._d_mflag[:rows], vocab=getattr(m, "vocab_local", None),
                        word_offset=getattr(m, "vocab_start", 0) // 32)

    def _vp_merge(self, cand, temp, topk, topp, cnt, out=None):
        import torch.distributed as dist

        src = cand.contiguous()
        if dist.get_backend(self.tp_group) != "nccl":
            src = src.cpu()
        parts = [torch.empty_like(src) for _ in range(self.tp_size)]
        dist.all_gather(parts, src, group=self.tp_group)
        allc = torch.stack(parts, 2).to(self.device)
        allc = allc.reshape(2, allc.shape[1], -1).contiguous()
        return ops.sample_merge(allc, temp, topk, topp, self.seed, cnt, self.cfg.vocab_size, out=out)

    def _sample(self, logits, reqs, to_host: bool = True):
        n = len(reqs)
        if self._fill_masks(reqs, n):
            self._mask(logits, n)
        temps = torch.tensor([r.params.temperature if r.params.do_sample else 0.0 for r in reqs], dtype=torch.float32)
        topk = torch.tensor([r.params.top_k for r in reqs], dtype=torch.int32)
        topp = torch.tensor([r.params.top_p for r in reqs], dtype=torch.float32)
        cnt = torch.tensor([r.rng_base + len(r.out) for r in reqs], dtype=torch.int64)
        if self.is_gpu:
            fast = all((0 < r.params.top_k <= ops.kernels.SAMPLE_FAST_MAX_K) or not r.params.do_sample
                       or r.params.temperature <= 0 for r in reqs)
            h = self._h2d
            if self.vp and fast:
                cand = ops.sample_candidates(logits, self.model.vocab_local, self.model.vocab_start)
                toks = self._vp_merge(cand, h(temps), h(topk), h(topp), h(cnt))
            else:
                if self.vp:
                    logits = self.model.full_logits(logits)
                toks = ops.sample_tokens(logits, h(temps), h(topk), h(topp), self.seed, h(cnt), fast=fast)
                toks = self._tp_sync_tokens(toks)
            return toks.cpu().tolist() if to_host else toks
        if self.vp:
            logits = self.model.full_logits(logits)
        g = torch.Generator().manual_seed(int(self.seed * 7919 + int(cnt[0]) if n else 0))
        return ops.sample_tokens(logits, temps, topk, topp, self.seed, cnt, generator=g).tolist()

    def _tp_fault_enqueue(self) -> None:
        ar = getattr(self.model, "custom_ar", None)
        if ar is not None and self.is_gpu:
            ar.enqueue_error_check()

    def _tp_fault_check(self) -> None:
        ar = getattr(self.model, "custom_ar", None)
        if ar is not None and self.is_gpu:
            ar.raise_if_error()

    def _tp_sync_tokens(self, toks):
        if self.tp_size > 1:
            import torch.distributed as dist

            src = dist.get_global_rank(self.tp_group, 0) if self.tp_group is not None else 0
            dist.broadcast(toks, src=src, group=self.tp_group)
        return toks

    def _accept_token(self, r: _Req, tok: int, now: float):
        r.out.append(tok)
        p = r.params
        reason = ""
        json_done = False
        if r.matcher is not None:
            if r.matcher.advance(tok):
                json_done = r.matcher.done()
            else:
                self.stats["json_broken"] = self.stats.get("json_broken", 0) + 1
        if json_done:
            reason = "stop"
        elif not p.ignore_eos and (tok in self.cfg.eos_ids or tok in p.stop_token_ids):
            reason = "stop"
        elif len(r.out) >= p.max_new_tokens:
            reason = "length"
        elif p.max_length is not None and len(r.prompt) + len(r.out) >= p.max_length:
            reason = "length"
        elif len(r.prompt) + len(r.out) >= self.max_model_len:
            reason = "length"
        if reason:
            r.finish_reason = reason
            r.finish_t = now
            self.running.remove(r)
            self.blocks.free_sequence(r.seq)
            self.finished[r.rid] = r

    def _preempt_one(self, protect: _Req | None) -> bool:
        for victim in reversed(self.running):
            if victim is protect:
                continue
            self.running.remove(victim)
            self.blocks.free_sequence(victim.seq)
            victim.preempted = 1
            victim.computed = 0
            self.waiting.appendleft(victim)
            self.stats["preemptions"] += 1
            return True
        return False

    def _can_pipeline(self) -> bool:
        return bool(self.pipeline_decode and self.running and not self.waiting and not self.prefilling
                    and not any(r.matcher is not None for r in self.running))

    def _swap_host_buffers(self) -> None:
        for k, alt in self._h_alt.items():
            cur = getattr(self, k)
            setattr(self, k, alt)
            self._h_alt[k] = cur

    def _length_done(self, r: _Req, extra: int) -> bool:
        n, p = len(r.out) + extra, r.params
        return (n >= p.max_new_tokens or (p.max_length is not None and len(r.prompt) + n >= p.max_length)
                or len(r.prompt) + n >= self.max_model_len)

    def _step_pipelined(self):
        prev = self._inflight
        if prev is None:
            batch = self._reserve_decode()
            if not batch:
                return
            self._launch_decode(batch, None)
            prev = self._inflight
        nxt = [r for r in prev["batch"] if not r.finish_reason and not self._length_done(r, 1)]
        launched = False
        if nxt:
            self._swap_host_buffers()
            fail = self.blocks.prepare_decode_into(
                [r.seq for r in nxt], [r.out[-1] if r.out else 0 for r in nxt], self.max_blocks_per_seq,
                self._h_ids.data_ptr(), self._h_pos.data_ptr(), self._h_slots.data_ptr(), self._h_ctx.data_ptr(),
                self._h_bt.data_ptr())
            if fail < 0:
                pos = {id(r): i for i, r in enumerate(prev["batch"])}
                self._launch_decode(nxt, [pos[id(r)] for r in nxt], pending=1)
                launched = True
            else:
                self._swap_host_buffers()
        cur = self._inflight if launched else None
        self._inflight = prev
        self._finish_inflight()
        self._inflight = cur

    def _launch_decode(self, batch: list, src_rows, pending: int = 0):
        t0 = time.perf_counter()
        B = len(batch)
        self._h_temp[:B] = torch.tensor([r.params.temperature if r.params.do_sample else 0.0 for r in batch])
        self._h_topk[:B] = torch.tensor([r.params.top_k for r in batch], dtype=torch.int32)
        self._h_topp[:B] = torch.tensor([r.params.top_p for r in batch])
        self._h_cnt[:B] = torch.tensor([r.rng_base + len(r.out) + pending for r in batch], dtype=torch.int64)
        self._fast = all((0 < r.params.top_k <= ops.kernels.SAMPLE_FAST_MAX_K) or not r.params.do_sample
                         or r.params.temperature <= 0 for r in batch)
        Bp = next(b for b in self._buckets if b >= B) if self.use_graphs else B
        if Bp > B:
            self._h_ids[B:Bp] = 0
            self._h_pos[B:Bp] = 0
            self._h_slots[B:Bp] = -1
            self._h_ctx[B:Bp] = 1
            self._h_bt[B:Bp] = 0
            self._h_temp[B:Bp] = 0.0
            self._h_topk[B:Bp] = 1
            self._h_topp[B:Bp] = 1.0
            self._h_cnt[B:Bp] = 0
        self._fill_order(Bp)
        pairs = [(self._d_pos, self._h_pos), (self._d_slots, self._h_slots), (self._d_ctx, self._h_ctx),
                 (self._d_temp, self._h_temp), (self._d_topk, self._h_topk), (self._d_topp, self._h_topp),
                 (self._d_cnt, self._h_cnt), (self._d_bt, self._h_bt), (self._d_order, self._h_order)]
        if src_rows is None:
            pairs.append((self._d_ids, self._h_ids))
        else:
            if src_rows == list(range(B)):
                self._d_ids[:B].copy_(self._d_tokens[:B])
            else:
                idx = torch.as_tensor(src_rows, dtype=torch.long).to(self.device, non_blocking=True)
                self._d_ids[:B].copy_(self._d_tokens.index_select(0, idx))
            if Bp > B:
                self._d_ids[B:Bp].zero_()
        for d, h in pairs:
            d[:Bp].copy_(h[:Bp], non_blocking=True)
        self._masked = False
        g = None
        if self.use_graphs:
            g = self._graphs.get((Bp, self._fast, False))
            if g is None:
                g = self._capture(Bp)
        with self.timer.phase("decode"):
            if g is not None:
                g.replay()
                self.stats["graph_replays"] += 1
            else:
                self._decode_body(Bp)
        ev = None
        if self.is_gpu:
            self._h_tokens[:Bp].copy_(self._d_tokens[:Bp], non_blocking=True)
            ev = torch.cuda.Event()
            ev.record()
        self._inflight = {"batch": list(batch), "Bp": Bp, "tokens": self._h_tokens, "event": ev}
        self.stats["decode_host_s"] = self.stats.get("decode_host_s", 0.0) + time.perf_counter() - t0

    def _finish_inflight(self):
        inf, self._inflight = self._inflight, None
        if inf is None:
            return
        t1 = time.perf_counter()
        if inf["event"] is not None:
            inf["event"].synchronize()
        t2 = time.perf_counter()
        self._collect_gpu_times(block=False)
        batch = inf["batch"]
        toks = inf["tokens"][:len(batch)].tolist()
        now = time.perf_counter()
        self.stats["decode_steps"] += 1
        for r, t in zip(batch, toks):
            if r.finish_reason:
                continue
            self.stats["decode_tokens"] += 1
            self._accept_token(r, int(t), now)
        t3 = time.perf_counter()
        self.stats["decode_host_s"] = self.stats.get("decode_host_s", 0.0) + (t3 - t2)
        self.stats["decode_gpu_wait_s"] = self.stats.get("decode_gpu_wait_s", 0.0) + (t2 - t1)

    def _reserve_decode(self) -> list:
        while True:
            batch = list(self.running)
            B = len(batch)
            if B == 0:
                return batch
            fail = self.blocks.prepare_decode_into(
                [r.seq for r in batch], [r.out[-1] for r in batch], self.max_blocks_per_seq,
                self._h_ids.data_ptr(), self._h_pos.data_ptr(), self._h_slots.data_ptr(), self._h_ctx.data_ptr(),
                self._h_bt.data_ptr())
            if fail < 0:
                return batch
            if not self._preempt_one(protect=None if B == 1 else batch[fail]):
                raise RuntimeError("KV cache exhausted")

    def _run_decode(self, batch: list):
        t0 = time.perf_counter()
        B = len(batch)
        self._h_temp[:B] = torch.tensor([r.params.temperature if r.params.do_sample else 0.0 for r in batch])
        self._h_topk[:B] = torch.tensor([r.params.top_k for r in batch], dtype=torch.int32)
        self._h_topp[:B] = torch.tensor([r.params.top_p for r in batch])
        self._h_cnt[:B] = torch.tensor([r.rng_base + len(r.out) for r in batch], dtype=torch.int64)
        self._fast = all((0 < r.params.top_k <= ops.kernels.SAMPLE_FAST_MAX_K) or not r.params.do_sample
                         or r.params.temperature <= 0 for r in batch)
        Bp = next(b for b in self._buckets if b >= B) if self.use_graphs else B
        if Bp > B:
            self._h_ids[B:Bp] = 0
            self._h_pos[B:Bp] = 0
            self._h_slots[B:Bp] = -1
            self._h_ctx[B:Bp] = 1
            self._h_bt[B:Bp] = 0
            self._h_temp[B:Bp] = 0.0
            self._h_topk[B:Bp] = 1
            self._h_topp[B:Bp] = 1.0
            self._h_cnt[B:Bp] = 0
        self._fill_order(Bp)
        for d, h in ((self._d_ids, self._h_ids), (self._d_pos, self._h_pos), (self._d_slots, self._h_slots),
                     (self._d_ctx, self._h_ctx), (self._d_temp, self._h_temp), (self._d_topk, self._h_topk),
                     (self._d_topp, self._h_topp), (self._d_cnt, self._h_cnt), (self._d_order, self._h_order)):
            d[:Bp].copy_(h[:Bp], non_blocking=True)
        self._d_bt[:Bp].copy_(self._h_bt[:Bp], non_blocking=True)
        self._masked = self._fill_masks(batch, Bp)
        t1 = time.perf_counter()
        g = None
        if self.use_graphs and not (self.vp and not self._fast):
            g = self._graphs.get((Bp, self._fast, self._masked))
            if g is None:
                g = self._capture(Bp)
        with self.timer.phase("decode"):
            if g is not None:
                g.replay()
                self.stats["graph_replays"] += 1
            else:
                self._decode_body(Bp)
        if self.is_gpu:
            if self.vp and self._fast:
                self._vp_merge(self._vp_cand[:, :Bp], self._d_temp[:Bp], self._d_topk[:Bp], self._d_topp[:Bp],
                               self._d_cnt[:Bp], out=self._d_tokens[:Bp])
            else:
                self._tp_sync_tokens(self._d_tokens[:Bp])
            self._h_tokens[:Bp].copy_(self._d_tokens[:Bp], non_blocking=True)
            self._tp_fault_enqueue()
            torch.cuda.current_stream(self.device).synchronize()
            self._tp_fault_check()
        t2 = time.perf_counter()
        self._collect_gpu_times()
        toks = self._h_tokens[:B].tolist()
        now = time.perf_counter()
        self.stats["decode_steps"] += 1
        self.stats["decode_tokens"] += B
        for r, t in zip(batch, toks):
            self._accept_token(r, int(t), now)
        t3 = time.perf_counter()
        self.stats["decode_host_s"] = self.stats.get("decode_host_s", 0.0) + (t1 - t0) + (t3 - t2)
        self.stats["decode_gpu_wait_s"] = self.stats.get("decode_gpu_wait_s", 0.0) + (t2 - t1)

    def _fill_order(self, Bp: int) -> None:
        ctx = self._h_ctx[:Bp].numpy()
        self._h_order[:Bp] = torch.from_numpy(np.argsort(-ctx, kind="stable").astype(np.int32))

    def _decode_part(self, Bp: int) -> int:
        hkv = self.cfg.kv_heads // self.tp_size
        return self.long_part_size if Bp * hkv >= 512 else self.part_size

    def _decode_body(self, Bp: int):
        meta = AttnMeta(decode=True, positions=self._d_pos[:Bp], slots=self._d_slots[:Bp],
                        block_tables=self._d_bt[:Bp], ctx_lens=self._d_ctx[:Bp], workspace=self._workspace,
                        part_size=self._decode_part(Bp), order=self._d_order[:Bp] if self.is_gpu else None)
        h = self.model.forward(self._d_ids[:Bp], meta, self.kv)
        logits = self.model.logits(h)
        if self._masked:
            self._mask(logits, Bp)
        if self.is_gpu and self.vp and self._fast:
            ops.sample_candidates(logits, self.model.vocab_local, self.model.vocab_start, out=self._vp_cand[:, :Bp])
        elif self.is_gpu:
            if self.vp:
                logits = self.model.full_logits(logits)
            ops.sample_tokens(logits, self._d_temp[:Bp], self._d_topk[:Bp], self._d_topp[:Bp], self.seed,
                              self._d_cnt[:Bp], out=self._d_tokens[:Bp], fast=self._fast,
                              workspace=self._sample_ws)
        else:
            if self.vp:
                logits = self.model.full_logits(logits)
            g = torch.Generator().manual_seed(int(self.seed * 7919 + int(self._h_cnt[0])))
            self._d_tokens[:Bp] = ops.sample_tokens(logits, self._d_temp[:Bp], self._d_topk[:Bp], self._d_topp[:Bp],
                                                    self.seed, self._d_cnt[:Bp], generator=g)
            self._h_tokens[:Bp] = self._d_tokens[:Bp]

    def _capture(self, Bp: int):
        try:
            s = torch.cuda.Stream(self.device)
            s.wait_stream(torch.cuda.current_stream(self.device))
            with torch.cuda.stream(s):
                self._decode_body(Bp)
            torch.cuda.current_stream(self.device).wait_stream(s)
            torch.cuda.synchronize(self.device)
            self._d_cnt[:Bp].copy_(self._h_cnt[:Bp])
            g = torch.cuda.CUDAGraph()
            if self._graph_pool is None:
                self._graph_pool = torch.cuda.graph_pool_handle()
            with torch.cuda.graph(g, pool=self._graph_pool, stream=s):
                self._decode_body(Bp)
            torch.cuda.synchronize(self.device)
            self._graphs[(Bp, self._fast, self._masked)] = g
            return g
        except Exception as exc:
            import logging

            logging.getLogger(__name__).warning("HIP graph capture failed (%s); decode runs eagerly", exc)
            self.use_graphs = False
            return None

    def capture_all(self, sizes=None):
        self._fast = True
        self._masked = False
        for b in sizes or self._buckets:
            if (b, True, False) not in self._graphs:
                self._capture(b)
```

### django_assistant_bot_amd/ops/kernels.py

```python
from __future__ import annotations

import math

import torch
import torch.nn.functional as F

from . import reference as ref
from ._lib import expect, expect_bf16_contig, native, ptr, same_device, stream

EPI_NONE, EPI_GELU, EPI_SWIGLU, EPI_SCORES = ref.EPI_NONE, ref.EPI_GELU, ref.EPI_SWIGLU, ref.EPI_SCORES
EPI_SWIGLU8 = ref.EPI_SWIGLU8


def _i32(t: torch.Tensor) -> None:
    if t.dtype != torch.int32 or not t.is_contiguous():
        raise TypeError("expected a contiguous int32 tensor")




def rmsnorm(x: torch.Tensor, w: torch.Tensor, eps: float, residual: torch.Tensor | None = None):
    slabs = x.dim() == 3 and x.dtype in (torch.float32, torch.bfloat16)
    if not x.is_cuda:
        if slabs:
            x = x.float().sum(0).to(torch.bfloat16)
        return ref.rmsnorm(x, w, eps, residual)
    expect_bf16_contig(w, residual)
    same_device(x, w, residual)
    cols = x.shape[-1]
    expect(w.numel() == cols, "rmsnorm weight size mismatch")
    if slabs:
        expect(x.is_contiguous(), "slabs must be contiguous")
        S, rows = x.shape[0], x.shape[1]
        shape = (rows, cols)
    else:
        expect_bf16_contig(x)
        rows = x.numel() // cols
        shape = tuple(x.shape)
    expect(residual is None or tuple(residual.shape) == shape, "residual shape mismatch")
    out = torch.empty(shape, dtype=torch.bfloat16, device=x.device)
    res_out = torch.empty(shape, dtype=torch.bfloat16, device=x.device) if residual is not None else None
    if slabs:
        native().rmsnorm_slabs(ptr(out), ptr(res_out), ptr(x), S, rows * cols, ptr(residual), ptr(w), rows, cols,
                               float(eps), stream(x), int(x.dtype == torch.bfloat16))
    else:
        native().rmsnorm(ptr(out), ptr(res_out), ptr(x), ptr(residual), ptr(w), rows, cols, float(eps), stream(x))
    return out, res_out


def layernorm(x, gamma, beta, eps, residual=None):
    if not x.is_cuda:
        return ref.layernorm(x, gamma, beta, eps, residual)
    expect_bf16_contig(x, gamma, beta, residual)
    same_device(x, gamma, beta, residual)
    cols = x.shape[-1]
    rows = x.numel() // cols
    expect(gamma.numel() == cols and beta.numel() == cols, "layernorm affine size mismatch")
    expect(residual is None or residual.shape == x.shape, "residual shape mismatch")
    out = torch.empty_like(x)
    native().layernorm(ptr(out), ptr(x), ptr(residual), ptr(gamma), ptr(beta), rows, cols, float(eps), stream(x))
    return out


def bert_embed(ids, pos_ids, type_ids, word, pos, typ, gamma, beta, eps):
    if not ids.is_cuda:
        return ref.bert_embed(ids, pos_ids, type_ids, word, pos, typ, gamma, beta, eps)
    _i32(ids)
    _i32(pos_ids)
    if type_ids is not None:
        _i32(type_ids)
    expect_bf16_contig(word, pos, typ, gamma, beta)
    expect(ids.shape == pos_ids.shape, "ids / position ids mismatch")
    H = word.shape[1]
    out = torch.empty((ids.numel(), H), dtype=word.dtype, device=ids.device)
    native().bert_embed(ptr(out), ptr(ids), ptr(pos_ids), ptr(type_ids), ptr(word), ptr(pos), ptr(typ), ptr(gamma),
                        ptr(beta), ids.numel(), H, float(eps), stream(ids))
    return out


def embed_gather(ids, table):
    if not ids.is_cuda:
        return ref.embed_gather(ids, table)
    _i32(ids)
    expect_bf16_contig(table)
    out = torch.empty((ids.numel(), table.shape[1]), dtype=table.dtype, device=ids.device)
    native().embed_gather(ptr(out), ptr(ids), ptr(table), ids.numel(), table.shape[1], stream(ids))
    return out


def mean_pool(hidden, cu_seqlens, normalize=False, want_bf16=False):
    if not hidden.is_cuda:
        out = ref.mean_pool(hidden, cu_seqlens, normalize)
        return (out, out.to(torch.bfloat16)) if want_bf16 else out
    expect_bf16_contig(hidden)
    _i32(cu_seqlens)
    B = cu_seqlens.numel() - 1
    H = hidden.shape[1]
    expect(H <= 4096, "mean_pool supports hidden <= 4096")
    out = torch.empty((B, H), dtype=torch.float32, device=hidden.device)
    ob = torch.empty((B, H), dtype=torch.bfloat16, device=hidden.device) if want_bf16 else None
    native().mean_pool(ptr(out), ptr(ob), ptr(hidden), ptr(cu_seqlens), B, H, int(bool(normalize)), stream(hidden))
    return (out, ob) if want_bf16 else out




def gelu(x, bias=None, out=None):
    if not x.is_cuda:
        return ref.gelu(x, bias)
    expect_bf16_contig(x, bias)
    cols = x.shape[-1]
    out = torch.empty_like(x) if out is None else out
    native().gelu(ptr(out), ptr(x), ptr(bias), x.numel() // cols, cols, stream(x))
    return out


def silu_mul(x, interleaved=False, group: int | None = None):
    group = (16 if interleaved else 0) if group is None else int(group)
    if not x.is_cuda:
        if group:
            F2 = x.shape[-1]
            v = x.reshape(*x.shape[:-1], F2 // (2 * group), 2, group)
            x = torch.cat([v[..., 0, :].reshape(*x.shape[:-1], F2 // 2), v[..., 1, :].reshape(*x.shape[:-1], F2 // 2)], -1)
        return ref.silu_mul(x)
    expect(group in (0, 16), "the GPU silu_mul takes stacked or 16-column groups (8-row groups: EPI_SWIGLU8)")
    expect_bf16_contig(x)
    F2 = x.shape[-1]
    rows = x.numel() // F2
    out = torch.empty((*x.shape[:-1], F2 // 2), dtype=x.dtype, device=x.device)
    native().silu_mul(ptr(out), ptr(x), rows, F2 // 2, stream(x), int(group == 16))
    return out


def rope_kv_write(qkv, positions, cos_sin, k_cache, v_cache, slots, Hq, Hkv, D, write_q=True):
    block_size = k_cache.shape[2]
    slabs = qkv.dim() == 3 and qkv.dtype in (torch.float32, torch.bfloat16)
    if not qkv.is_cuda:
        if slabs:
            qkv = qkv.float().sum(0).to(torch.bfloat16)
        return ref.rope_kv_write(qkv, positions, cos_sin, k_cache, v_cache, slots, Hq, Hkv, D, block_size)
    expect_bf16_contig(k_cache, v_cache)
    _i32(positions)
    expect(slots.dtype == torch.int64 and slots.is_contiguous(), "slots must be contiguous int64")
    expect(cos_sin.dtype == torch.float32 and cos_sin.is_contiguous(), "cos_sin must be contiguous fp32")
    T = qkv.shape[-2]
    expect(qkv.shape[-1] == (Hq + 2 * Hkv) * D, "qkv width mismatch")
    expect(positions.numel() == T and slots.numel() == T, "positions / slots length mismatch")
    expect(tuple(k_cache.shape[1:]) == (Hkv, block_size, D) and k_cache.shape == v_cache.shape, "cache shape mismatch")
    expect(cos_sin.shape[1] == D // 2, "cos/sin table width mismatch")
    if not write_q:
        expect(not slabs, "write_q=False needs a bf16 qkv")
        expect_bf16_contig(qkv)
        native().rope_kv_write(ptr(qkv), qkv.stride(0), ptr(positions), ptr(cos_sin), 0, ptr(k_cache),
                               ptr(v_cache), ptr(slots), T, Hq, Hkv, D, block_size, stream(qkv))
        return None
    q = torch.empty((T, Hq, D), dtype=torch.bfloat16, device=qkv.device)
    if slabs:
        expect(qkv.is_contiguous(), "slabs must be contiguous")
        native().rope_kv_write(0, qkv.shape[-1], ptr(positions), ptr(cos_sin), ptr(q), ptr(k_cache), ptr(v_cache),
                               ptr(slots), T, Hq, Hkv, D, block_size, stream(qkv), ptr(qkv), qkv.shape[0],
                               T * qkv.shape[-1], int(qkv.dtype == torch.bfloat16))
    else:
        expect_bf16_contig(qkv)
        native().rope_kv_write(ptr(qkv), qkv.stride(0), ptr(positions), ptr(cos_sin), ptr(q), ptr(k_cache),
                               ptr(v_cache), ptr(slots), T, Hq, Hkv, D, block_size, stream(qkv))
    return q




def _head_strides(t: torch.Tensor):
    expect(t.stride(-1) == 1, "attention operands need unit stride on the head dim")
    return t.stride(0), t.stride(1)


def flash_attention_packed(q, k, v, cu_q, cu_k, max_seqlen_q, causal=False, scale=None, out=None):
    D = q.shape[-1]
    scale = 1.0 / math.sqrt(D) if scale is None else scale
    if not q.is_cuda:
        return ref.flash_attention_packed(q, k, v, cu_q, cu_k, causal, scale)
    _i32(cu_q)
    _i32(cu_k)
    expect(q.dtype == torch.bfloat16 and k.dtype == torch.bfloat16 and v.dtype == torch.bfloat16, "bf16 required")
    expect(D in (32, 64, 128), "head dim must be 32, 64 or 128")
    Hq, Hkv = q.shape[1], k.shape[1]
    expect(Hq % Hkv == 0, "GQA requires Hq % Hkv == 0")
    expect(k.stride() == v.stride(), "k and v must share strides")
    qst, qsh = _head_strides(q)
    kst, ksh = _head_strides(k)
    for s in (qst, qsh, kst, ksh):
        expect(s % 8 == 0, "attention strides must be multiples of 8 elements (16 B)")
    out = torch.empty((q.shape[0], Hq, D), dtype=q.dtype, device=q.device) if out is None else out
    B = cu_q.numel() - 1
    native().flash_attention(ptr(q), qst, qsh, ptr(k), ptr(v), kst, ksh, 0, 0, 0, 0, 0, ptr(out), out.stride(0),
                             out.stride(1), ptr(cu_q), ptr(cu_k), 0, B, int(max_seqlen_q), Hq, Hkv, D,
                             int(bool(causal)), 0, float(scale), stream(q))
    return out


def flash_rope_ok(D: int, block_size: int) -> bool:
    return D == 128 and block_size % 64 == 0


def flash_attention_paged(q, k_cache, v_cache, block_tables, cu_q, ctx_lens, max_seqlen_q, causal=True, scale=None,
                          out=None, rope=None):
    D = q.shape[-1]
    scale = 1.0 / math.sqrt(D) if scale is None else scale
    if not q.is_cuda:
        if rope is not None:
            pos, cs = rope
            T, Hq = q.shape[0], q.shape[1]
            q = ref.rope_q(q.reshape(T, Hq, D), pos, cs)
        return ref.flash_attention_paged(q, k_cache, v_cache, block_tables, cu_q, ctx_lens, causal, scale)
    _i32(cu_q)
    _i32(ctx_lens)
    _i32(block_tables)
    expect_bf16_contig(k_cache, v_cache)
    expect(D in (32, 64, 128), "head dim must be 32, 64 or 128")
    Hq, Hkv, bs = q.shape[1], k_cache.shape[1], k_cache.shape[2]
    qst, qsh = _head_strides(q)
    out = torch.empty((q.shape[0], Hq, D), dtype=q.dtype, device=q.device) if out is None else out
    B = cu_q.numel() - 1
    expect(block_tables.shape[0] >= B and ctx_lens.numel() >= B, "block table / ctx_lens rows < batch")
    if rope is not None:
        pos, cs = rope
        _i32(pos)
        expect(flash_rope_ok(D, bs) and cs.dtype == torch.float32 and cs.is_contiguous() and pos.numel() == q.shape[0],
               "q RoPE in the attention needs D 128, block size % 64, fp32 cos/sin and one position per query")
        native().flash_attention_rope(ptr(q), qst, qsh, ptr(k_cache), ptr(v_cache), ptr(block_tables),
                                      block_tables.shape[1], bs, ptr(out), out.stride(0), out.stride(1), ptr(cu_q),
                                      ptr(ctx_lens), B, int(max_seqlen_q), Hq, Hkv, D, int(bool(causal)),
                                      float(scale), ptr(pos), ptr(cs), stream(q))
        return out
    native().flash_attention(ptr(q), qst, qsh, 0, 0, 0, 0, ptr(k_cache), ptr(v_cache), ptr(block_tables),
                             block_tables.shape[1], bs, ptr(out), out.stride(0), out.stride(1), ptr(cu_q), 0,
                             ptr(ctx_lens), B, int(max_seqlen_q), Hq, Hkv, D, int(bool(causal)), 1, float(scale),
                             stream(q))
    return out


class DecodeWorkspace:

    def __init__(self, max_batch, Hq, D, max_parts, device):
        self.max_parts = max_parts
        self.o = torch.empty((max_batch * Hq * max_parts * D,), dtype=torch.float32, device=device)
        self.m = torch.empty((max_batch * Hq * max_parts,), dtype=torch.float32, device=device)
        self.l = torch.empty((max_batch * Hq * max_parts,), dtype=torch.float32, device=device)
        self.cnt = torch.zeros((max_batch * Hq,), dtype=torch.int32, device=device)


def paged_decode(q, k_cache, v_cache, block_tables, ctx_lens, part_size=512, workspace: DecodeWorkspace | None = None,
                 scale=None, out=None, order=None, warm=None):
    B, Hq, D = q.shape
    scale = 1.0 / math.sqrt(D) if scale is None else scale
    if not q.is_cuda:
        return ref.paged_decode(q, k_cache, v_cache, block_tables, ctx_lens, scale)
    _i32(ctx_lens)
    _i32(block_tables)
    expect_bf16_contig(q, k_cache, v_cache)
    Hkv, bs = k_cache.shape[1], k_cache.shape[2]
    expect(D in (64, 128), "decode head dim must be 64 or 128")
    expect(Hq % Hkv == 0 and Hq // Hkv <= 16, "GQA group must be <= 16")
    expect(part_size % 128 == 0, "part_size must be a multiple of 128")
    expect(block_tables.shape[0] >= B and ctx_lens.numel() >= B, "block table / ctx_lens rows < batch")
    max_parts = workspace.max_parts if workspace is not None else 1
    if workspace is None:
        part_size = max(part_size, ((block_tables.shape[1] * bs + 127) // 128) * 128)
        ws_o = ws_m = ws_l = ws_c = None
    else:
        expect(workspace.o.numel() >= B * Hq * max_parts * D and workspace.cnt.numel() >= B * Hkv,
               "decode workspace too small")
        ws_o, ws_m, ws_l, ws_c = workspace.o, workspace.m, workspace.l, workspace.cnt
    out = torch.empty_like(q) if out is None else out
    if order is not None:
        _i32(order)
        expect(order.is_cuda and order.numel() >= B, "decode order must hold the batch")
    wargs = {}
    if warm is not None and warm[1] > 0:
        ranges, blocks = warm
        expect(1 <= len(ranges) <= 2 and 0 < blocks <= 1024, "warm: 1-2 ranges, 1-1024 workgroups")
        for i, (t, nb) in enumerate(ranges):
            expect(t.is_cuda and t.is_contiguous() and 0 < nb <= t.numel() * t.element_size() and nb % 16 == 0,
                   "warm range must be a 16-B multiple inside a contiguous device tensor")
            wargs[f"w{i}"], wargs[f"w{i}_bytes"] = ptr(t), int(nb)
        wargs["w_blocks"] = int(blocks)
    native().paged_decode_attention(ptr(q), ptr(k_cache), ptr(v_cache), ptr(block_tables), block_tables.shape[1], bs,
                                    ptr(ctx_lens), ptr(out), ptr(ws_o), ptr(ws_m), ptr(ws_l), ptr(ws_c), B, Hq, Hkv,
                                    D, int(part_size), int(max_parts), float(scale), stream(q), ptr(order), **wargs)
    return out



kv_quantize = ref.kv_quantize
kv_dequantize = ref.kv_dequantize


def _expect_fp8_cache(k_data, k_exp, v_data, v_exp):
    for t in (k_data, k_exp, v_data, v_exp):
        if t.dtype != torch.uint8 or not t.is_contiguous():
            raise TypeError("the FP8 KV cache is contiguous uint8 (data and exponent bytes)")
    same_device(k_data, k_exp, v_data, v_exp)
    expect(k_data.dim() == 4 and k_data.shape == v_data.shape and tuple(k_exp.shape) == tuple(k_data.shape[:3])
           and k_exp.shape == v_exp.shape, "FP8 cache: data [blocks, Hkv, block_size, D], exponents [blocks, Hkv, block_size]")
    expect(k_data.shape[3] == 128, "the FP8 KV cache kernels take head dim 128 only")


def rope_kv_write_fp8(qkv, positions, cos_sin, k_data, k_exp, v_data, v_exp, slots, Hq, Hkv, D, write_q=True):
    block_size = k_data.shape[2]
    slabs = qkv.dim() == 3 and qkv.dtype in (torch.float32, torch.bfloat16)
    if not qkv.is_cuda:
        if slabs:
            qkv = qkv.float().sum(0).to(torch.bfloat16)
        q = ref.rope_kv_write_fp8(qkv, positions, cos_sin, k_data, k_exp, v_data, v_exp, slots, Hq, Hkv, D, block_size)
        return q if write_q else None
    expect(D == 128, "the FP8 KV cache kernels take head dim 128 only")
    _expect_fp8_cache(k_data, k_exp, v_data, v_exp)
    _i32(positions)
    expect(slots.dtype == torch.int64 and slots.is_contiguous(), "slots must be contiguous int64")
    expect(cos_sin.dtype == torch.float32 and cos_sin.is_contiguous(), "cos_sin must be contiguous fp32")
    T = qkv.shape[-2]
    expect(qkv.shape[-1] == (Hq + 2 * Hkv) * D, "qkv width mismatch")
    expect(positions.numel() == T and slots.numel() == T, "positions / slots length mismatch")
    expect(k_data.shape[1] == Hkv, "cache shape mismatch")
    expect(cos_sin.shape[1] == D // 2, "cos/sin table width mismatch")
    caches = (ptr(k_data), ptr(k_exp), ptr(v_data), ptr(v_exp))
    if not write_q:
        expect(not slabs, "write_q=False needs a bf16 qkv")
        expect_bf16_contig(qkv)
        native().rope_kv_write_fp8(ptr(qkv), qkv.stride(0), ptr(positions), ptr(cos_sin), 0, *caches, ptr(slots), T,
                                   Hq, Hkv, D, block_size, stream(qkv))
        return None
    q = torch.empty((T, Hq, D), dtype=torch.bfloat16, device=qkv.device)
    if slabs:
        expect(qkv.is_contiguous(), "slabs must be contiguous")
        native().rope_kv_write_fp8(0, qkv.shape[-1], ptr(positions), ptr(cos_sin), ptr(q), *caches, ptr(slots), T, Hq,
                                   Hkv, D, block_size, stream(qkv), ptr(qkv), qkv.shape[0], T * qkv.shape[-1],
                                   int(qkv.dtype == torch.bfloat16))
    else:
        expect_bf16_contig(qkv)
        native().rope_kv_write_fp8(ptr(qkv), qkv.stride(0), ptr(positions), ptr(cos_sin), ptr(q), *caches, ptr(slots),
                                   T, Hq, Hkv, D, block_size, stream(qkv))
    return q


def paged_decode_fp8(q, k_data, k_exp, v_data, v_exp, block_tables, ctx_lens, part_size=512,
                     workspace: DecodeWorkspace | None = None, scale=None, out=None, order=None, warm=None):
    B, Hq, D = q.shape
    scale = 1.0 / math.sqrt(D) if scale is None else scale
    expect(warm is None, "paged_decode_fp8 does not take warm= (the L3 warm-up rides on the bf16 kernel only)")
    if not q.is_cuda:
        return ref.paged_decode_fp8(q, k_data, k_exp, v_data, v_exp, block_tables, ctx_lens, scale)
    expect(D == 128, "the FP8 KV cache kernels take head dim 128 only")
    _i32(ctx_lens)
    _i32(block_tables)
    expect_bf16_contig(q)
    _expect_fp8_cache(k_data, k_exp, v_data, v_exp)
    Hkv, bs = k_data.shape[1], k_data.shape[2]
    expect(bs % 32 == 0, "block size must be a multiple of 32")
    expect(Hq % Hkv == 0 and Hq // Hkv <= 16, "GQA group must be <= 16")
    expect(part_size % 128 == 0, "part_size must be a multiple of 128")
    expect(block_tables.shape[0] >= B and ctx_lens.numel() >= B, "block table / ctx_lens rows < batch")
    max_parts = workspace.max_parts if workspace is not None else 1
    if workspace is None:
        part_size = max(part_size, ((block_tables.shape[1] * bs + 127) // 128) * 128)
        ws_o = ws_m = ws_l = ws_c = None
    else:
        expect(workspace.o.numel() >= B * Hq * max_parts * D and workspace.cnt.numel() >= B * Hkv,
               "decode workspace too small")
        ws_o, ws_m, ws_l, ws_c = workspace.o, workspace.m, workspace.l, workspace.cnt
    out = torch.empty_like(q) if out is None else out
    expect(out.dtype == torch.bfloat16 and out.is_contiguous() and out.shape == q.shape, "out: contiguous bf16 like q")
    if order is not None:
        _i32(order)
        expect(order.is_cuda and order.numel() >= B, "decode order must hold the batch")
    native().paged_decode_attention_fp8(ptr(q), ptr(k_data), ptr(k_exp), ptr(v_data), ptr(v_exp), ptr(block_tables),
                                        block_tables.shape[1], bs, ptr(ctx_lens), ptr(out), ptr(ws_o), ptr(ws_m),
                                        ptr(ws_l), ptr(ws_c), B, Hq, Hkv, D, int(part_size), int(max_parts),
                                        float(scale), stream(q), ptr(order))
    return out


def kv_dequant_blocks(k_data, k_exp, v_data, v_exp, block_ids, k_out, v_out):
    n = block_ids.numel()
    expect(k_out.shape == v_out.shape and k_out.shape[0] >= n and tuple(k_out.shape[1:]) == tuple(k_data.shape[1:]),
           "scratch: [cap >= n, Hkv, block_size, D]")
    if not k_data.is_cuda:
        ref.kv_dequant_blocks(k_data, k_exp, block_ids, k_out)
        ref.kv_dequant_blocks(v_data, v_exp, block_ids, v_out)
        return k_out, v_out
    _expect_fp8_cache(k_data, k_exp, v_data, v_exp)
    _i32(block_ids)
    expect_bf16_contig(k_out, v_out)
    same_device(k_data, block_ids, k_out, v_out)
    native().kv_fp8_dequant_blocks(ptr(k_data), ptr(k_exp), ptr(v_data), ptr(v_exp), ptr(block_ids), n, ptr(k_out),
                                   ptr(v_out), k_data.shape[1], k_data.shape[2], k_data.shape[3], stream(k_data))
    return k_out, v_out


class KVPrefillPlan:

    __slots__ = ("blocks", "scratch_bt", "groups")

    def __init__(self, blocks, scratch_bt, groups):
        self.blocks, self.scratch_bt, self.groups = blocks, scratch_bt, groups


def kv_prefill_plan(block_tables, ctx_lens, cu_q, block_size: int, cap: int, device=None) -> KVPrefillPlan:
    bt = torch.as_tensor(block_tables).cpu()
    ctx = [int(x) for x in torch.as_tensor(ctx_lens).cpu().tolist()]
    cu = [int(x) for x in torch.as_tensor(cu_q).cpu().tolist()]
    B = len(cu) - 1
    nblk = [-(-ctx[b] // block_size) for b in range(B)]
    cols = max(1, bt.shape[1])
    sbt = torch.zeros((B, cols), dtype=torch.int32)
    blocks, groups = [], []
    lo = 0
    while lo < B:
        expect(nblk[lo] <= cap, f"a sequence of {nblk[lo]} KV blocks exceeds the FP8 prefill scratch ({cap} blocks)")
        hi, used = lo, 0
        while hi < B and used + nblk[hi] <= cap:
            used += nblk[hi]
            hi += 1
        blk_lo, run = len(blocks), 0
        for b in range(lo, hi):
            blocks.extend(bt[b, :nblk[b]].tolist())
            sbt[b, :nblk[b]] = torch.arange(run, run + nblk[b], dtype=torch.int32)
            sbt[b, nblk[b]:] = run if nblk[b] else 0
            run += nblk[b]
        groups.append([lo, hi, blk_lo, len(blocks), cu[lo], cu[hi], max(cu[b + 1] - cu[b] for b in range(lo, hi))])
        lo = hi
    dev = torch.device(device) if device is not None else torch.device("cpu")

    def to(t):
        if dev.type != "cuda":
            return t
        return t.pin_memory().to(dev, non_blocking=True)

    single = len(groups) == 1
    out_groups = []
    for g in groups:
        cu_g = None if single else to(torch.tensor([c - g[4] for c in cu[g[0]:g[1] + 1]], dtype=torch.int32))
        out_groups.append((*g, cu_g))
    return KVPrefillPlan(to(torch.tensor(blocks, dtype=torch.int32)), to(sbt), out_groups)


def flash_attention_paged_fp8(q, k_data, k_exp, v_data, v_exp, block_tables, cu_q, ctx_lens, max_seqlen_q, causal=True,
                              scale=None, out=None, rope=None, scratch=None, plan: KVPrefillPlan | None = None):
    if not q.is_cuda:
        D = q.shape[-1]
        scale = 1.0 / math.sqrt(D) if scale is None else scale
        if rope is not None:
            q = ref.rope_q(q.reshape(q.shape[0], q.shape[1], D), rope[0], rope[1])
        res = ref.flash_attention_paged_fp8(q, k_data, k_exp, v_data, v_exp, block_tables, cu_q, ctx_lens, causal, scale)
        return res if out is None else out.copy_(res)
    expect(scratch is not None, "the FP8 prefill attention needs the cache's bf16 scratch pool")
    sk, sv = scratch
    if plan is None:
        plan = kv_prefill_plan(block_tables, ctx_lens, cu_q, k_data.shape[2], sk.shape[0], q.device)
    Hq, D = q.shape[1], q.shape[2]
    out = torch.empty((q.shape[0], Hq, D), dtype=q.dtype, device=q.device) if out is None else out
    for lo, hi, b0, b1, t0, t1, max_q, cu_g in plan.groups:
        kv_dequant_blocks(k_data, k_exp, v_data, v_exp, plan.blocks[b0:b1], sk, sv)
        if cu_g is None:
            flash_attention_paged(q, sk, sv, plan.scratch_bt, cu_q, ctx_lens, max_seqlen_q, causal, scale, out, rope)
            continue
        if t1 == t0:
            continue
        r = None if rope is None else (rope[0][t0:t1], rope[1])
        flash_attention_paged(q[t0:t1], sk, sv, plan.scratch_bt[lo:hi], cu_g, ctx_lens[lo:hi], max_q, causal, scale,
                              out[t0:t1], r)
    return out




GEMM256_MIN_M = 1024


GEMM_MID_MIN_M = 1
GEMM_MID_FILL = 192


def _g256_fill(M: int, N: int) -> tuple[int, float]:
    tiles = -(-M // 256) * (N // 256)
    return tiles, tiles / (-(-tiles // 256) * 256)


def use_gemm_mid(M: int, N: int, K: int, lda: int) -> bool:
    if M < GEMM_MID_MIN_M or N % 256 or not gemm_mid_ok(M, N, K, lda):
        return False
    tiles, fill = _g256_fill(M, N)
    return tiles < GEMM_MID_FILL or fill < 0.7


def use_gemm256(M: int, N: int, K: int, lda: int, ldb: int) -> bool:
    wide = M >= 256 and N % 256 == 0 and -(-M // 256) * (N // 256) >= GEMM_MID_FILL
    return (M >= GEMM256_MIN_M or wide) and bool(native().gemm256_ok(M, N, K, lda, ldb))


def gemm_bt(A, B, bias=None, residual=None, epilogue=EPI_NONE, out_f32=False, row_group=None, q_group=None,
            allow=None, out=None, shuffled=False, n=None, b_group: int = 1, rows=None, as_m=None):
    expect(b_group == 1 or (shuffled and b_group == 8), "b_group: 1, or 8 with a shuffled copy")
    if rows is not None or as_m is not None:
        expect(out_f32 is False and row_group is None and q_group is None and allow is None and bias is None
               and n is None and epilogue in (EPI_NONE, EPI_SWIGLU8),
               "row subsets: plain / residual / SwiGLU8 projections only")
        expect(rows is None or as_m is None, "row subsets: rows or as_m, not both")
        if not A.is_cuda:
            y = gemm_bt(A, B, residual=residual, epilogue=epilogue, shuffled=shuffled, b_group=b_group)
            y = y if rows is None else y.index_select(0, rows.long())
            return y if out is None else out.copy_(y)
        return _gemm256_rows(A, B, residual, epilogue, shuffled, b_group, rows, as_m, out)
    if shuffled:
        R = B.shape[0]
        N = R if n is None else int(n)
        expect(R % (16 * b_group) == 0 and B.shape[1] % 32 == 0 and B.is_contiguous() and R >= N,
               "shuffled B: contiguous [R, K] copy, R % (16 b_group) == 0, K % 32 == 0, R >= n")
        if not A.is_cuda:
            Bu = unshuffle_weights(B, b_group)[:N]
            return ref.gemm_bt(A, Bu, bias, residual, epilogue, out_f32, row_group, q_group, allow)
    if not A.is_cuda:
        return ref.gemm_bt(A, B, bias, residual, epilogue, out_f32, row_group, q_group, allow)
    expect(A.dtype == torch.bfloat16 and B.dtype == torch.bfloat16, "bf16 operands required")
    expect(A.stride(-1) == 1 and B.stride(-1) == 1, "operands must be K-contiguous")
    M, K = A.shape
    N = (B.shape[0] if n is None else int(n)) if shuffled else B.shape[0]
    expect(B.shape[1] == K, "inner dims mismatch")
    expect(K % 64 == 0 and N % 4 == 0, "gemm_bt needs K % 64 == 0 and N % 4 == 0")
    expect(A.stride(0) % 8 == 0 and B.stride(0) % 8 == 0, "row strides must be multiples of 8")
    if bias is not None:
        expect_bf16_contig(bias)
        expect(bias.numel() == N, "bias size mismatch")
    n_out = N // 2 if epilogue in (EPI_SWIGLU, EPI_SWIGLU8) else N
    if epilogue == EPI_SWIGLU:
        expect(N % 32 == 0 and not out_f32 and residual is None,
               "swiglu epilogue needs N % 32 == 0, bf16 output, no residual")
    if epilogue == EPI_SWIGLU8:
        expect(N % 32 == 0 and not out_f32 and bias is None and residual is None,
               "swiglu8 epilogue needs N % 32 == 0, bf16 output, no bias / residual")
    if residual is not None:
        expect(residual.dtype == torch.bfloat16 and residual.stride(-1) == 1, "residual must be bf16 row-major")
        expect(tuple(residual.shape) == (M, n_out), "residual shape mismatch")
    allow_words = 0
    if allow is not None:
        expect(allow.dtype == torch.int32 and allow.is_contiguous() and allow.shape[0] == M, "allow mask shape")
        allow_words = allow.shape[1]
        expect(allow_words * 32 >= N, "allow mask too narrow")
    if row_group is not None:
        _i32(row_group)
        expect(row_group.numel() >= N, "row_group shorter than N")
    if q_group is not None:
        _i32(q_group)
        expect(q_group.numel() >= M, "q_group shorter than M")
    dtype = torch.float32 if out_f32 else torch.bfloat16
    if out is None:
        out = torch.empty((M, n_out), dtype=dtype, device=A.device)
    expect(out.dtype == dtype and out.stride(-1) == 1 and tuple(out.shape) == (M, n_out), "bad output buffer")
    plain = not out_f32 and row_group is None and q_group is None and allow is None
    if (plain and shuffled and N == B.shape[0] and bias is None and epilogue in (EPI_NONE, EPI_SWIGLU8)
            and use_gemm_mid(M, N, K, A.stride(0))):
        return gemm_mid(A, B, residual=residual, epilogue=epilogue, out=out, b_group=b_group)
    if (epilogue in (EPI_NONE, EPI_GELU, EPI_SWIGLU, EPI_SWIGLU8) and plain and (not shuffled or N == B.shape[0])
            and use_gemm256(M, N, K, A.stride(0), B.stride(0))):
        return _gemm256_into(A, B, out, bias, residual, epilogue, shuffled, b_group)
    native().gemm_bt(ptr(A), A.stride(0), ptr(B), B.stride(0), ptr(out), out.stride(0), ptr(bias), ptr(residual),
                     residual.stride(0) if residual is not None else 0, M, N, K, int(epilogue), int(out_f32),
                     ptr(row_group), ptr(q_group), ptr(allow), allow_words, stream(A),
                     B.shape[0] if shuffled else 0, int(b_group))
    return out


def _gemm256_into(A, B, out, bias, residual, epilogue, shuffled, b_group=1, rows=None):
    M, K = A.shape
    native().gemm256(ptr(A), A.stride(0), ptr(B), B.stride(0), ptr(out), out.stride(0), ptr(bias), ptr(residual),
                     residual.stride(0) if residual is not None else 0, M if rows is None else rows.numel(), B.shape[0],
                     K, int(epilogue), stream(A), int(shuffled), int(b_group), ptr(rows), M if rows is not None else 0)
    return out


def _gemm256_rows(A, B, residual, epilogue, shuffled, b_group, rows, as_m, out=None, direct=False):
    expect(A.dtype == torch.bfloat16 and B.dtype == torch.bfloat16, "bf16 operands required")
    expect(A.dim() == 2 and B.dim() == 2 and A.stride(-1) == 1 and B.stride(-1) == 1 and B.shape[1] == A.shape[1],
           "operands must be K-contiguous [M, K] / [N, K]")
    (M, K), N = A.shape, B.shape[0]
    full = M if rows is not None else int(as_m)
    n_out = N // 2 if epilogue == EPI_SWIGLU8 else N
    if rows is not None:
        _i32(rows)
        expect(rows.is_cuda and rows.dim() == 1, "rows: int32 [n] on the device")
    else:
        expect(full >= M, "as_m: at least the rows of A")
    expect(epilogue == EPI_NONE or residual is None, "swiglu8 epilogue takes no residual")
    if residual is not None:
        expect(residual.dtype == torch.bfloat16 and residual.stride(-1) == 1 and tuple(residual.shape) == (M, n_out),
               "residual must be bf16 row-major [M, N]")
    lda = A.stride(0)
    mid = shuffled and use_gemm_mid(full, N, K, lda)
    expect(direct or (not mid and use_gemm256(full, N, K, lda, B.stride(0))),
           "row subsets need the shape's full call on gemm256 (not gemm_mid or the 128 x 128 kernel)")
    expect(bool(native().gemm256_ok(M, N, K, lda, B.stride(0))), "gemm256: N % 256, K % 128, 16-B rows")
    expect(not shuffled or (B.is_contiguous() and B.shape[1] == K), "shuffled B must be a contiguous [N, K] copy")
    n = M if rows is None else rows.numel()
    if out is None:
        out = torch.empty((n, n_out), dtype=torch.bfloat16, device=A.device)
    expect(out.dtype == torch.bfloat16 and out.stride(-1) == 1 and tuple(out.shape) == (n, n_out)
           and (n <= 1 or out.stride(0) % 8 == 0), "bad output buffer")
    if n == 0:
        return out
    return _gemm256_into(A, B, out, None, residual, epilogue, shuffled, b_group, rows)


def gemm256(A, B, bias=None, residual=None, epilogue=EPI_NONE, shuffled=False, b_group: int = 1, rows=None,
            out=None):
    if rows is not None:
        expect(A.is_cuda and bias is None, "gemm256 rows: CUDA operands, no bias")
        return _gemm256_rows(A, B, residual, epilogue, shuffled, b_group, rows, None, out, direct=True)
    M, K = A.shape
    N = B.shape[0]
    expect(A.is_cuda and A.dtype == torch.bfloat16 and B.dtype == torch.bfloat16, "bf16 CUDA operands required")
    expect(bool(native().gemm256_ok(M, N, K, A.stride(0), B.stride(0))), "gemm256: N % 256, K % 128, 16-B rows")
    expect(not shuffled or (B.is_contiguous() and B.shape[1] == K), "shuffled B must be a contiguous [N, K] copy")
    n_out = N // 2 if epilogue in (EPI_SWIGLU, EPI_SWIGLU8) else N
    out = torch.empty((M, n_out), dtype=torch.bfloat16, device=A.device)
    return _gemm256_into(A, B, out, bias, residual, epilogue, shuffled, b_group)


_MID_WS: dict = {}


def _mid_workspace(device: torch.device, s: int):
    key = (device.index, s)
    ws = _MID_WS.get(key)
    if ws is None:
        nat = native()
        slabs = torch.empty((nat.gemm_mid_slab_bytes() // 4,), dtype=torch.float32, device=device)
        cnt = torch.zeros((1 << 16,), dtype=torch.int32, device=device)
        ws = _MID_WS[key] = (slabs, cnt)
    return ws


def gemm_mid_ok(M: int, N: int, K: int, lda: int) -> bool:
    return bool(native().gemm_mid_ok(M, N, K, lda)) and -(-M // 128) * (N // 256) <= (1 << 16)


def gemm_mid(A, B, residual=None, epilogue=EPI_NONE, out=None, variant: int = 0, b_group: int = 1):
    M, K = A.shape
    N = B.shape[0]
    expect(A.is_cuda and A.dtype == torch.bfloat16 and B.dtype == torch.bfloat16, "bf16 CUDA operands required")
    expect(A.stride(-1) == 1 and B.is_contiguous() and B.shape[1] == K, "A K-contiguous, B a contiguous [N, K] copy")
    expect(epilogue in (EPI_NONE, EPI_SWIGLU8), "gemm_mid epilogues: none (+residual) or SwiGLU8")
    expect(gemm_mid_ok(M, N, K, A.stride(0)), "gemm_mid: N % 256, K % 64, M <= 4096, 16-B rows")
    expect(b_group in (1, 8), "gemm_mid: b_group 1 or 8")
    n_out = N // 2 if epilogue == EPI_SWIGLU8 else N
    if residual is not None:
        expect(epilogue == EPI_NONE and residual.dtype == torch.bfloat16 and residual.stride(-1) == 1
               and tuple(residual.shape) == (M, N), "residual must be bf16 [M, N]")
    if out is None:
        out = torch.empty((M, n_out), dtype=torch.bfloat16, device=A.device)
    expect(out.dtype == torch.bfloat16 and out.stride(-1) == 1 and tuple(out.shape) == (M, n_out), "bad output")
    s = stream(A)
    slabs, cnt = _mid_workspace(A.device, s)
    native().gemm_mid(ptr(A), A.stride(0), ptr(B), ptr(out), out.stride(0), ptr(residual),
                      residual.stride(0) if residual is not None else 0, M, N, K, int(epilogue), ptr(slabs),
                      slabs.numel() * 4, ptr(cnt), cnt.numel(), s, int(variant), int(b_group))
    return out


def score_candidates(A, B, thr, cap, row_group=None, q_group=None):
    expect(A.is_cuda and A.dtype == torch.bfloat16 and B.dtype == torch.bfloat16, "bf16 CUDA operands required")
    expect(A.stride(-1) == 1 and B.stride(-1) == 1 and A.stride(0) % 8 == 0 and B.stride(0) % 8 == 0,
           "operands must be K-contiguous with row strides % 8 == 0")
    M, K = A.shape
    N = B.shape[0]
    expect(B.shape[1] == K and K % 64 == 0 and N % 4 == 0, "score_candidates needs K % 64 == 0 and N % 4 == 0")
    expect(thr.dtype == torch.float32 and thr.is_contiguous() and thr.numel() >= M, "thr must be fp32 [M]")
    if row_group is not None:
        _i32(row_group)
        expect(row_group.numel() >= N, "row_group shorter than N")
    if q_group is not None:
        _i32(q_group)
        expect(q_group.numel() >= M, "q_group shorter than M")
    cand_val = torch.full((M, cap), float("-inf"), dtype=torch.float32, device=A.device)
    cand_idx = torch.empty((M, cap), dtype=torch.int32, device=A.device)
    cnt = torch.zeros(M, dtype=torch.int32, device=A.device)
    native().gemm_score_candidates(ptr(A), A.stride(0), ptr(B), B.stride(0), M, N, K, ptr(row_group), ptr(q_group),
                                   ptr(thr), ptr(cnt), ptr(cand_val), ptr(cand_idx), int(cap), stream(A))
    return cand_val, cand_idx, cnt


def score_candidates_shuffled(A, B_shuf, N, thr, cap, row_group=None, q_group=None):
    expect(A.is_cuda and A.dtype == torch.bfloat16 and B_shuf.dtype == torch.bfloat16, "bf16 CUDA operands required")
    M, K = A.shape
    expect(shuffled_scan_ok(M, K) and A.stride(-1) == 1 and A.stride(0) % 8 == 0, "queries need K % 128 == 0")
    expect(B_shuf.is_contiguous() and B_shuf.shape[1] == K, "shuffled copy [R, K]")
    expect(B_shuf.shape[0] % 16 == 0 and B_shuf.shape[0] >= -(-N // 128) * 128, "shuffled copy needs round_up(N, 128) rows")
    expect(thr.dtype == torch.float32 and thr.is_contiguous() and thr.numel() >= M, "thr must be fp32 [M]")
    if row_group is not None:
        _i32(row_group)
        expect(row_group.numel() >= N, "row_group shorter than N")
    if q_group is not None:
        _i32(q_group)
        expect(q_group.numel() >= M, "q_group shorter than M")
    cand_val = torch.full((M, cap), float("-inf"), dtype=torch.float32, device=A.device)
    cand_idx = torch.empty((M, cap), dtype=torch.int32, device=A.device)
    cnt = torch.zeros(M, dtype=torch.int32, device=A.device)
    native().score_candidates_shuf(ptr(A), A.stride(0), ptr(B_shuf), M, int(N), K, ptr(row_group), ptr(q_group),
                                   ptr(thr), ptr(cnt), ptr(cand_val), ptr(cand_idx), int(cap), stream(A),
                                   B_shuf.shape[0])
    return cand_val, cand_idx, cnt


def shuffled_scan_ok(M: int, K: int) -> bool:
    return M >= 1 and K % 128 == 0


def shuffle_rows_into(dst: torch.Tensor, rows: torch.Tensor, vals: torch.Tensor) -> None:
    R, K = dst.shape
    v5 = dst.view(R // 16, K // 32, 4, 16, 8)
    rows = rows.to(dst.device, torch.long)
    v5[rows // 16, :, :, rows % 16, :] = vals.to(dst.dtype).reshape(-1, K // 32, 4, 8)


def _ref_stream_gemm(x, w, splits=1, epilogue=EPI_NONE, residual=None, norm_eps=0.0):
    if norm_eps > 0:
        xf = x.float()
        r = torch.rsqrt(xf.pow(2).mean(-1, keepdim=True) + norm_eps)
        y = xf @ w.float().t() * r
        if epilogue in (EPI_SWIGLU, EPI_SWIGLU8):
            grp = 16 if epilogue == EPI_SWIGLU else 8
            v = y.view(y.shape[0], -1, 2, grp)
            y = (torch.nn.functional.silu(v[:, :, 0]) * v[:, :, 1]).reshape(y.shape[0], -1)
        if splits > 1:
            return torch.cat([y[None], torch.zeros((splits - 1,) + tuple(y.shape))], 0)
        return y.to(torch.bfloat16)
    y = ref.gemm_bt(x, w, None, None, epilogue, out_f32=splits > 1)
    if splits > 1:
        return torch.cat([y[None], torch.zeros((splits - 1,) + tuple(y.shape), dtype=y.dtype)], 0)
    return y if residual is None else (y.float() + residual.float()).to(torch.bfloat16)


STREAM_KS = 128
STREAM_MAX_M = 256


def shuffle_weights(w: torch.Tensor, group: int = 1) -> torch.Tensor:
    N, K = w.shape
    expect(N % (16 * group) == 0 and K % 32 == 0, "shuffle_weights needs N % (16 group) == 0 and K % 32 == 0")
    f = w.reshape(N // 16, 16, K // 32, 4, 8).permute(0, 2, 3, 1, 4)
    if group > 1:
        f = f.reshape(N // (16 * group), group, K // 32, 512).permute(0, 2, 1, 3)
    return f.contiguous().view(N, K)


def unshuffle_weights(w: torch.Tensor, group: int = 1) -> torch.Tensor:
    N, K = w.shape
    if group > 1:
        w = w.reshape(N // (16 * group), K // 32, group, 512).permute(0, 2, 1, 3)
    return w.reshape(N // 16, K // 32, 4, 16, 8).permute(0, 3, 1, 2, 4).contiguous().view(N, K)


weight_quantize_fp8 = ref.weight_quantize_fp8
weight_dequantize_fp8 = ref.weight_dequantize_fp8


def shuffle_weights_fp8(data: torch.Tensor, group: int = 1) -> torch.Tensor:
    N, K = data.shape
    expect(data.dtype == torch.uint8, "shuffle_weights_fp8 takes e4m3fn bytes (uint8)")
    expect(N % (16 * group) == 0 and K % 64 == 0, "shuffle_weights_fp8 needs N % (16 group) == 0 and K % 64 == 0")
    f = data.reshape(N // 16, 16, K // 64, 2, 4, 8).permute(0, 2, 4, 1, 3, 5)
    if group > 1:
        f = f.reshape(N // (16 * group), group, K // 64, 1024).permute(0, 2, 1, 3)
    return f.contiguous().view(N, K)


def unshuffle_weights_fp8(data: torch.Tensor, group: int = 1) -> torch.Tensor:
    N, K = data.shape
    if group > 1:
        data = data.reshape(N // (16 * group), K // 64, group, 1024).permute(0, 2, 1, 3)
    return data.reshape(N // 16, K // 64, 4, 16, 2, 8).permute(0, 3, 1, 4, 2, 5).contiguous().view(N, K)


def stream_gemm(x, w, splits=1, epilogue=EPI_NONE, residual=None, out=None, nt=False, cfg=0, norm_eps: float = 0.0,
                slab_dtype=torch.float32, w_group: int = 1, w_exps=None):
    fp8 = w_exps is not None
    if not x.is_cuda:
        if fp8:
            w = weight_dequantize_fp8(w, w_exps).to(x.dtype)
        y = _ref_stream_gemm(x, w, splits=splits, epilogue=epilogue, residual=residual, norm_eps=norm_eps)
        return y.to(slab_dtype) if splits > 1 else y
    expect(norm_eps <= 0 or residual is None, "the consumer RMSNorm takes no residual add")
    if fp8:
        expect(x.dtype == torch.bfloat16 and w.dtype == torch.uint8, "FP8 weights: bf16 x, uint8 fragment copy")
        expect(native().stream_gemm_fp8_ok(cfg), f"stream_gemm cfg {cfg} has no FP8-weight instantiation")
        expect(w.dim() == 2 and w.shape[1] % 64 == 0, "FP8 weights need K % 64 == 0")
        expect(w_exps.dtype == torch.uint8 and w_exps.is_cuda and w_exps.dim() == 1 and w_exps.shape[0] == w.shape[0]
               and w_exps.is_contiguous() and w_exps.data_ptr() % 4 == 0,
               "w_exps must be the uint8 [N] row exponents (contiguous, 4-byte aligned)")
    else:
        expect(x.dtype == torch.bfloat16 and w.dtype == torch.bfloat16, "bf16 operands required")
    expect(x.stride(-1) == 1 and w.stride(-1) == 1, "operands must be K-contiguous")
    M, K = x.shape
    N = w.shape[0]
    bn = native().stream_gemm_bn(cfg)
    expect(bn > 0 and M <= native().stream_gemm_max_m(cfg), f"stream_gemm cfg {cfg}: bad config or M too large")
    expect(w.shape[1] == K and N % bn == 0 and K % (splits * STREAM_KS) == 0,
           f"stream_gemm needs N % {bn} == 0 and K % ({STREAM_KS}*splits) == 0")
    expect(x.stride(0) % 8 == 0 and w.stride(0) % 8 == 0, "row strides must be multiples of 8")
    if native().stream_gemm_shuffled(cfg):
        expect(w.is_contiguous(), "shuffled-layout configurations take a contiguous shuffle_weights() tensor")
    if splits > 1:
        expect(epilogue == EPI_NONE and residual is None, "split-K writes raw slabs")
        expect(slab_dtype in (torch.float32, torch.bfloat16), "slabs are fp32 or bf16")
        if out is None:
            out = torch.empty((splits, M, N), dtype=slab_dtype, device=x.device)
        expect(out.dtype == slab_dtype and out.is_contiguous() and tuple(out.shape) == (splits, M, N), "bad slabs")
        ldo = N
    else:
        n_out = N // 2 if epilogue in (EPI_SWIGLU, EPI_SWIGLU8) else N
        if residual is not None:
            expect(epilogue == EPI_NONE and residual.dtype == torch.bfloat16 and residual.stride(-1) == 1
                   and tuple(residual.shape) == (M, N), "residual must be bf16 [M, N]")
        if epilogue == EPI_SWIGLU:
            expect(bn % 32 == 0, f"stream_gemm cfg {cfg}: EPI_SWIGLU needs 32-row tiles (use EPI_SWIGLU8)")
        if out is None:
            out = torch.empty((M, n_out), dtype=torch.bfloat16, device=x.device)
        expect(out.dtype == torch.bfloat16 and out.stride(-1) == 1 and tuple(out.shape) == (M, n_out), "bad output")
        ldo = out.stride(0)
    if fp8:
        native().stream_gemm_fp8(ptr(x), x.stride(0), ptr(w), ptr(w_exps), ptr(out), ldo, ptr(residual),
                                 residual.stride(0) if residual is not None else 0, M, N, K, splits, int(epilogue),
                                 stream(x), int(bool(nt)), int(cfg), float(norm_eps),
                                 int(splits > 1 and out.dtype == torch.bfloat16), int(w_group))
        return out
    native().stream_gemm(ptr(x), x.stride(0), ptr(w), w.stride(0), ptr(out), ldo, ptr(residual),
                         residual.stride(0) if residual is not None else 0, M, N, K, splits, int(epilogue), stream(x),
                         int(bool(nt)), int(cfg), float(norm_eps), int(splits > 1 and out.dtype == torch.bfloat16),
                         int(w_group))
    return out


def slab_reduce(slabs, residual=None, out=None):
    if not slabs.is_cuda:
        y = slabs.float().sum(0).to(torch.bfloat16)
        return y if residual is None else (y.float() + residual.float()).to(torch.bfloat16)
    S, M, N = slabs.shape
    expect(slabs.dtype in (torch.float32, torch.bfloat16) and slabs.is_contiguous() and N % 8 == 0, "bad slabs")
    if out is None:
        out = torch.empty((M, N), dtype=torch.bfloat16, device=slabs.device)
    if residual is not None:
        expect(residual.dtype == torch.bfloat16 and tuple(residual.shape) == (M, N) and residual.stride(-1) == 1,
               "residual must be bf16 [M, N]")
    native().slab_reduce(ptr(out), out.stride(0), ptr(slabs), S, M, N, ptr(residual),
                         residual.stride(0) if residual is not None else 0, stream(slabs),
                         int(slabs.dtype == torch.bfloat16))
    return out


def interleave_gate_up(w_gate: torch.Tensor, w_up: torch.Tensor, group: int = 16) -> torch.Tensor:
    Fd, H = w_gate.shape
    assert Fd % group == 0
    g = w_gate.reshape(Fd // group, group, H)
    u = w_up.reshape(Fd // group, group, H)
    return torch.stack([g, u], dim=1).reshape(2 * Fd, H).contiguous()


def regroup_gate_up(w: torch.Tensor, src: int = 16, dst: int = 8) -> torch.Tensor:
    n2, H = w.shape
    v = w.reshape(n2 // (2 * src), 2, src, H)
    gate, up = v[:, 0].reshape(n2 // 2, H), v[:, 1].reshape(n2 // 2, H)
    return interleave_gate_up(gate, up, dst)




SAMPLE_FAST_MAX_K = 64
_CHUNK = 256 * 32


def sample_workspace(rows: int, vocab: int, device) -> torch.Tensor:
    ncand = -(-vocab // _CHUNK) * SAMPLE_FAST_MAX_K
    return torch.empty((rows * ncand * 8,), dtype=torch.uint8, device=device)


def sample_tokens(logits, temperature, top_k, top_p, seed: int, counters, generator=None, out=None,
                  fast: bool | None = None, workspace: torch.Tensor | None = None):
    if not logits.is_cuda:
        return ref.sample_hf(logits, temperature, top_k, top_p, generator)
    rows, vocab = logits.shape
    expect(logits.stride(-1) == 1, "logits rows must be contiguous")
    expect(logits.dtype in (torch.float32, torch.bfloat16), "logits must be fp32 or bf16")
    expect(temperature.dtype == torch.float32 and temperature.numel() >= rows, "temperature")
    expect(top_p.dtype == torch.float32 and top_p.numel() >= rows, "top_p")
    _i32(top_k)
    expect(counters.dtype == torch.int64 and counters.numel() >= rows, "counters")
    out = torch.empty((rows,), dtype=torch.int32, device=logits.device) if out is None else out
    if fast is None:
        fast = False
    ncand = -(-vocab // _CHUNK) * SAMPLE_FAST_MAX_K
    if fast and ncand <= 1024:
        ws = workspace if workspace is not None else sample_workspace(rows, vocab, logits.device)
        expect(ws.numel() >= rows * ncand * 8, "sampling workspace too small")
        native().sample_tokens_2stage(ptr(logits), int(logits.dtype == torch.float32), logits.stride(0), rows, vocab,
                                      ptr(temperature), ptr(top_k), ptr(top_p), int(seed) & ((1 << 64) - 1),
                                      ptr(counters), ptr(out), ptr(ws), ws.numel(), stream(logits))
    else:
        native().sample_tokens(ptr(logits), int(logits.dtype == torch.float32), logits.stride(0), rows, vocab,
                               ptr(temperature), ptr(top_k), ptr(top_p), int(seed) & ((1 << 64) - 1), ptr(counters),
                               ptr(out), 0, stream(logits))
    return out


def mask_logits(logits, mask, row_flags, vocab: int | None = None, word_offset: int = 0):
    rows = logits.shape[0]
    vocab = logits.shape[1] if vocab is None else int(vocab)
    words = -(-vocab // 32)
    expect(mask.dtype == torch.int32 and mask.is_contiguous() and mask.shape[0] >= rows
           and mask.shape[1] >= word_offset + words, "mask: int32 [rows, >= ceil(vocab / 32) words past the offset]")
    if not logits.is_cuda:
        m = mask[:rows, word_offset:word_offset + words]
        bits = (m.view(torch.int32).unsqueeze(-1) >> torch.arange(32, dtype=torch.int32)) & 1
        allow = bits.reshape(rows, -1)[:, :vocab].bool() | (row_flags[:rows] == 0).unsqueeze(1)
        logits[:, :vocab].masked_fill_(~allow, float("-inf"))
        return logits
    expect(logits.stride(-1) == 1 and logits.dtype in (torch.float32, torch.bfloat16), "logits: fp32/bf16 rows")
    _i32(row_flags)
    native().mask_logits(ptr(logits), int(logits.dtype == torch.float32), logits.stride(0), rows, vocab,
                         ptr(mask) + 4 * int(word_offset), words, ptr(row_flags), stream(logits), mask.stride(0))
    return logits


def sample_candidates(logits, vocab: int, index_base: int = 0, out=None):
    expect(logits.is_cuda and logits.stride(-1) == 1 and logits.dtype in (torch.float32, torch.bfloat16),
           "logits: CUDA fp32/bf16 rows")
    rows = logits.shape[0]
    ncand = sample_candidates_per_row(vocab)
    if out is None:
        out = torch.empty((2, rows, ncand), dtype=torch.int32, device=logits.device)
    expect(out.dtype == torch.int32 and tuple(out.shape) == (2, rows, ncand) and out.stride(2) == 1
           and out.stride(1) == ncand, "candidates: int32 [2, rows, ncand] with contiguous halves")
    native().sample_candidates(ptr(logits), int(logits.dtype == torch.float32), logits.stride(0), rows, int(vocab),
                               int(index_base), ptr(out[0]), ptr(out[1]), ncand, stream(logits))
    return out


def sample_candidates_per_row(vocab: int) -> int:
    return -(-int(vocab) // _CHUNK) * SAMPLE_FAST_MAX_K


def sample_merge(cands, temperature, top_k, top_p, seed: int, counters, vocab: int, out=None):
    two, rows, n = cands.shape
    expect(two == 2 and n <= 1024 and cands.dtype == torch.int32 and cands.is_contiguous(),
           "candidates: contiguous int32 [2, rows, <= 1024]")
    out = torch.empty((rows,), dtype=torch.int32, device=cands.device) if out is None else out
    _i32(top_k)
    native().sample_merge(ptr(cands[0]), ptr(cands[1]), n, rows, int(vocab), ptr(temperature), ptr(top_k), ptr(top_p),
                          int(seed) & ((1 << 64) - 1), ptr(counters), ptr(out), stream(cands))
    return out


def topk_rows(scores, k, index_base=0, want_global=False):
    rows, n = scores.shape
    expect(1 <= k <= min(n, 1024), "1 <= k <= min(n, 1024)")
    if rows == 0:
        return (torch.empty((0, k), dtype=torch.float32, device=scores.device),
                torch.empty((0, k), dtype=torch.int64 if want_global else torch.int32, device=scores.device))
    if not scores.is_cuda:
        v, i = ref.topk_rows(scores, k)
        return (v, i.long() + index_base) if want_global else (v, i)
    expect(scores.dtype == torch.float32 and scores.stride(-1) == 1, "scores must be fp32 with contiguous rows")
    vals = torch.empty((rows, k), dtype=torch.float32, device=scores.device)
    if want_global:
        idx = torch.empty((rows, k), dtype=torch.int64, device=scores.device)
        i32, i64 = 0, ptr(idx)
    else:
        idx = torch.empty((rows, k), dtype=torch.int32, device=scores.device)
        i32, i64 = ptr(idx), 0
    if n >= 4 * _CHUNK:
        kc = -(-k // 64) * 64
        ncand = -(-n // _CHUNK) * kc
        ws = torch.empty((rows * ncand * 8,), dtype=torch.uint8, device=scores.device)
        native().topk_rows_2stage(ptr(scores), scores.stride(0), rows, n, k, ptr(vals), i32, int(index_base), i64,
                                  ptr(ws), ws.numel(), stream(scores))
    else:
        native().topk_rows(ptr(scores), scores.stride(0), rows, n, k, ptr(vals), i32, int(index_base), i64,
                           stream(scores))
    return vals, idx


def linear(x, w, b=None, residual=None, act=None):
    epi = {None: EPI_NONE, "gelu": EPI_GELU, "swiglu": EPI_SWIGLU}[act]
    if not x.is_cuda:
        return ref.gemm_bt(x, w, b, residual, epi)
    K, N = x.shape[-1], w.shape[0]
    expect(epi != EPI_SWIGLU or N % 32 == 0, "swiglu linear needs 16-row [gate | up] groups (N % 32 == 0)")
    x2 = x.reshape(-1, K)
    r2 = residual.reshape(x2.shape[0], -1) if residual is not None else None
    pk, pn = (-K) % 64, (-N) % 4
    if pk or pn:
        x2 = F.pad(x2, (0, pk)) if pk else x2
        w = F.pad(w, (0, pk, 0, pn))
        b = F.pad(b, (0, pn)) if (b is not None and pn) else b
        r2 = F.pad(r2, (0, pn)) if (r2 is not None and pn) else r2
    y = gemm_bt(x2, w, b, r2, epi)
    if pn:
        y = y[:, :N].contiguous()
    return y.view(*x.shape[:-1], y.shape[-1])
```

Before: 40.21 queries/s.

## Pack decode step inputs into one block and let sampler write next ids

Adds a packed per-step input layout so the KV manager fills ids, positions, slots, block tables, sampling params and attention order into a single contiguous host block. The aim is to replace many small host-to-device copies per decode step with fewer, larger ones. It also adds an optional sampler output that writes sampled tokens straight into the next step's ids buffer, which would remove a later copy. That option defaults to off. The change adds engine plumbing and capture-time resets, and risks stale inputs if the graph-captured buffers and the packed views fall out of sync.

```diff
diff --git a/django_assistant_bot_amd/csrc/bindings.cpp b/django_assistant_bot_amd/csrc/bindings.cpp
--- a/django_assistant_bot_amd/csrc/bindings.cpp
+++ b/django_assistant_bot_amd/csrc/bindings.cpp
@@ -277,10 +277,10 @@
   }, py::arg("out"), py::arg("ldo"), py::arg("slabs"), py::arg("S"), py::arg("M"), py::arg("N"), py::arg("residual"),
      py::arg("ldr"), py::arg("s"), py::arg("slab_bf16") = 0);
   m.def("sample_tokens", [](u logits, int f32, long ld, int rows, int vocab, u temp, u top_k, u top_p,
-                            unsigned long long seed, u counters, u out_tokens, u out_logprobs, u s) {
+                            unsigned long long seed, u counters, u out_tokens, u out_logprobs, u s, u ids_out) {
     check(dab::sample_tokens(CVP(logits), f32, ld, rows, vocab, (const float*)temp, (const int*)top_k,
                              (const float*)top_p, seed, (int64_t*)counters, (int*)out_tokens, (float*)out_logprobs,
-                             ST(s)),
+                             ST(s), (int*)ids_out),
           "sample_tokens");
   });
   m.def("topk_rows", [](u scores, long ld, int rows, int n, int k, u out_vals, u out_idx, long long base, u out_idx64,
@@ -291,10 +291,11 @@
   });
 
   m.def("sample_tokens_2stage", [](u logits, int f32, long ld, int rows, int vocab, u temp, u top_k, u top_p,
-                                   unsigned long long seed, u counters, u out_tokens, u ws, size_t ws_bytes, u s) {
+                                   unsigned long long seed, u counters, u out_tokens, u ws, size_t ws_bytes, u s,
+                                   u ids_out) {
     check(dab::sample_tokens_2stage(CVP(logits), f32, ld, rows, vocab, (const float*)temp, (const int*)top_k,
                                     (const float*)top_p, seed, (int64_t*)counters, (int*)out_tokens, VP(ws), ws_bytes,
-                                    ST(s)),
+                                    ST(s), (int*)ids_out),
           "sample_tokens_2stage");
   });
   m.def("mask_logits", [](u logits, int f32, long ld, int rows, int vocab, u mask, int words, u row_flags, u s,
@@ -309,9 +310,10 @@
           "sample_candidates");
   });
   m.def("sample_merge", [](u keys, u idx, int ncand, int rows, int vocab, u temp, u top_k, u top_p,
-                           unsigned long long seed, u counters, u out_tokens, u s) {
+                           unsigned long long seed, u counters, u out_tokens, u s, u ids_out) {
     check(dab::sample_merge((const uint32_t*)keys, (const int*)idx, ncand, rows, vocab, (const float*)temp,
-                            (const int*)top_k, (const float*)top_p, seed, (int64_t*)counters, (int*)out_tokens, ST(s)),
+                            (const int*)top_k, (const float*)top_p, seed, (int64_t*)counters, (int*)out_tokens, ST(s),
+                            (int*)ids_out),
           "sample_merge");
   });
   m.def("topk_rows_2stage", [](u scores, long ld, int rows, int n, int k, u out_vals, u out_idx, long long base,
@@ -442,8 +444,30 @@
              return k.prepare_decode(seqs, toks, max_blocks, (int32_t*)ids, (int32_t*)pos, (int64_t*)slots,
                                      (int32_t*)ctx, (int32_t*)bt);
            })
+      .def("prepare_decode_packed",
+           [](dab::KVBlockManager& k, const std::vector<int64_t>& seqs, const std::vector<int32_t>& toks,
+              int max_blocks, int rows, const std::vector<float>& temp, const std::vector<int32_t>& top_k,
+              const std::vector<float>& top_p, const std::vector<int64_t>& counters, u block) {
+             return k.prepare_decode_packed(seqs, toks, max_blocks, rows, temp, top_k, top_p, counters, (void*)block);
+           })
       .def("block_table_into", [](const dab::KVBlockManager& k, const std::vector<int64_t>& seqs, int max_blocks,
                                   u out) { k.block_table(seqs, max_blocks, (int32_t*)out); });
+  m.def("decode_step_layout", [](int rows, int max_blocks) {
+    const dab::DecodeStepLayout L = dab::decode_step_layout(rows, max_blocks);
+    py::dict d;
+    d["ids"] = L.ids;
+    d["pos"] = L.pos;
+    d["slots"] = L.slots;
+    d["ctx"] = L.ctx;
+    d["order"] = L.order;
+    d["block_table"] = L.block_table;
+    d["temperature"] = L.temperature;
+    d["top_k"] = L.top_k;
+    d["top_p"] = L.top_p;
+    d["counters"] = L.counters;
+    d["bytes"] = L.bytes;
+    return d;
+  }, py::arg("rows"), py::arg("max_blocks"));
 
   m.def(
       "aggregate_documents",
diff --git a/django_assistant_bot_amd/csrc/kernels/launchers.h b/django_assistant_bot_amd/csrc/kernels/launchers.h
--- a/django_assistant_bot_amd/csrc/kernels/launchers.h
+++ b/django_assistant_bot_amd/csrc/kernels/launchers.h
@@ -119,16 +119,17 @@
                       uint32_t* cand_key, int* cand_idx, int ncand, hipStream_t s);
 int sample_merge(const uint32_t* cand_key, const int* cand_idx, int ncand, int rows, int vocab,
                  const float* temperature, const int* top_k, const float* top_p, unsigned long long seed,
-                 int64_t* counters, int* out_tokens, hipStream_t s);
+                 int64_t* counters, int* out_tokens, hipStream_t s, int* ids_out = nullptr);
 int sample_tokens(const void* logits, int logits_f32, long ld, int rows, int vocab, const float* temperature,
                   const int* top_k, const float* top_p, unsigned long long seed, int64_t* counters, int* out_tokens,
-                  float* out_logprobs, hipStream_t s);
+                  float* out_logprobs, hipStream_t s, int* ids_out = nullptr);
 int topk_rows(const float* scores, long ld, int rows, int n, int k, float* out_vals, int* out_idx, int64_t index_base,
               int64_t* out_idx64, hipStream_t s);
 
 int sample_tokens_2stage(const void* logits, int logits_f32, long ld, int rows, int vocab, const float* temperature,
                          const int* top_k, const float* top_p, unsigned long long seed, int64_t* counters,
-                         int* out_tokens, void* workspace, size_t workspace_bytes, hipStream_t s);
+                         int* out_tokens, void* workspace, size_t workspace_bytes, hipStream_t s,
+                         int* ids_out = nullptr);
 int topk_rows_2stage(const float* scores, long ld, int rows, int n, int k, float* out_vals, int* out_idx,
                      int64_t index_base, int64_t* out_idx64, void* workspace, size_t workspace_bytes, hipStream_t s);
 
diff --git a/django_assistant_bot_amd/csrc/kernels/select.hip b/django_assistant_bot_amd/csrc/kernels/select.hip
--- a/django_assistant_bot_amd/csrc/kernels/select.hip
+++ b/django_assistant_bot_amd/csrc/kernels/select.hip
@@ -163,7 +163,7 @@
                                                         const int* __restrict__ top_k,
                                                         const float* __restrict__ top_p, unsigned long long seed,
                                                         int64_t* __restrict__ counters, int* __restrict__ out_tokens,
-                                                        float* __restrict__ out_logprobs) {
+                                                        float* __restrict__ out_logprobs, int* __restrict__ ids_out) {
   __shared__ SelShared sh;
   __shared__ float probs[SEL_MAXK];
   const int row = blockIdx.x;
@@ -180,6 +180,7 @@
   if (threadIdx.x != 0) return;
   if (T <= 0.f) {
     out_tokens[row] = sh.cand_idx[0];
+    if (ids_out) ids_out[row] = sh.cand_idx[0];
     if (out_logprobs) out_logprobs[row] = 0.f;
     return;
   }
@@ -219,6 +220,7 @@
     }
   }
   out_tokens[row] = sh.cand_idx[pick];
+  if (ids_out) ids_out[row] = sh.cand_idx[pick];
   if (out_logprobs) out_logprobs[row] = __logf(probs[pick] / kept);
 }
 
@@ -446,7 +448,7 @@
                                                               const int* __restrict__ top_k,
                                                               const float* __restrict__ top_p, int vocab,
                                                               unsigned long long seed, int64_t* __restrict__ counters,
-                                                              int* __restrict__ out_tokens) {
+                                                              int* __restrict__ out_tokens, int* __restrict__ ids_out) {
   __shared__ uint32_t skey[SEL_MAXK];
   __shared__ int sidx[SEL_MAXK];
   __shared__ float probs[SEL_MAXK];
@@ -483,6 +485,7 @@
   if (tid != 0) return;
   if (T <= 0.f) {
     out_tokens[row] = sidx[0];
+    if (ids_out) ids_out[row] = sidx[0];
     return;
   }
   while (k < nc && skey[k] == skey[k - 1] && skey[k] > kNegInfKey) ++k;
@@ -522,6 +525,7 @@
     }
   }
   out_tokens[row] = sidx[pick];
+  if (ids_out) ids_out[row] = sidx[pick];
 }
 
 __global__ __launch_bounds__(SEL_NT) void topk_merge_kernel(const uint32_t* __restrict__ cand_key,
@@ -545,7 +549,7 @@
 
 int sample_tokens_2stage(const void* logits, int logits_f32, long ld, int rows, int vocab, const float* temperature,
                          const int* top_k, const float* top_p, unsigned long long seed, int64_t* counters,
-                         int* out_tokens, void* workspace, size_t workspace_bytes, hipStream_t s) {
+                         int* out_tokens, void* workspace, size_t workspace_bytes, hipStream_t s, int* ids_out) {
   if (rows <= 0) return 0;
   constexpr int PT = 32, KC = 64;
   const int chunk = CH_NT * PT;
@@ -558,7 +562,7 @@
   hipLaunchKernelGGL(chunk_topk_kernel<PT>, dim3(nchunks, rows), dim3(CH_NT), 0, s, logits, logits_f32 ? 0 : 1, ld,
                      vocab, KC, KC, ck, ci);
   hipLaunchKernelGGL(sample_merge_kernel, dim3(rows), dim3(SEL_NT), 0, s, ck, ci, ncand, temperature, top_k, top_p,
-                     vocab, seed, counters, out_tokens);
+                     vocab, seed, counters, out_tokens, ids_out);
   return hipGetLastError();
 }
 
@@ -575,11 +579,11 @@
 
 int sample_merge(const uint32_t* cand_key, const int* cand_idx, int ncand, int rows, int vocab,
                  const float* temperature, const int* top_k, const float* top_p, unsigned long long seed,
-                 int64_t* counters, int* out_tokens, hipStream_t s) {
+                 int64_t* counters, int* out_tokens, hipStream_t s, int* ids_out) {
   if (rows <= 0) return 0;
   if (ncand <= 0 || ncand > SEL_MAXK) return hipErrorInvalidValue;
   hipLaunchKernelGGL(sample_merge_kernel, dim3(rows), dim3(SEL_NT), 0, s, cand_key, cand_idx, ncand, temperature, top_k,
-                     top_p, vocab, seed, counters, out_tokens);
+                     top_p, vocab, seed, counters, out_tokens, ids_out);
   return hipGetLastError();
 }
 
@@ -634,11 +638,11 @@
 
 int sample_tokens(const void* logits, int logits_f32, long ld, int rows, int vocab, const float* temperature,
                   const int* top_k, const float* top_p, unsigned long long seed, int64_t* counters, int* out_tokens,
-                  float* out_logprobs, hipStream_t s) {
+                  float* out_logprobs, hipStream_t s, int* ids_out) {
   if (rows <= 0) return 0;
   if (vocab <= 0) return hipErrorInvalidValue;
   hipLaunchKernelGGL(sample_kernel, dim3(rows), dim3(SEL_NT), 0, s, logits, logits_f32, ld, vocab, temperature, top_k,
-                     top_p, seed, counters, out_tokens, out_logprobs);
+                     top_p, seed, counters, out_tokens, out_logprobs, ids_out);
   return hipGetLastError();
 }
 
diff --git a/django_assistant_bot_amd/csrc/runtime/kv_manager.cpp b/django_assistant_bot_amd/csrc/runtime/kv_manager.cpp
--- a/django_assistant_bot_amd/csrc/runtime/kv_manager.cpp
+++ b/django_assistant_bot_amd/csrc/runtime/kv_manager.cpp
@@ -206,6 +206,69 @@
   return -1;
 }
 
+DecodeStepLayout decode_step_layout(int rows, int max_blocks) {
+  if (rows < 0 || max_blocks < 0) throw std::invalid_argument("decode_step_layout: negative size");
+  DecodeStepLayout L{};
+  int64_t o = 0;
+  auto section = [&o](int64_t bytes) {
+    const int64_t at = o;
+    o = (o + bytes + 15) & ~(int64_t)15;
+    return at;
+  };
+  L.ids = section(4LL * rows);
+  L.pos = section(4LL * rows);
+  L.slots = section(8LL * rows);
+  L.ctx = section(4LL * rows);
+  L.order = section(4LL * rows);
+  L.block_table = section(4LL * rows * max_blocks);
+  L.temperature = section(4LL * rows);
+  L.top_k = section(4LL * rows);
+  L.top_p = section(4LL * rows);
+  L.counters = section(8LL * rows);
+  L.bytes = o;
+  return L;
+}
+
+int KVBlockManager::prepare_decode_packed(const std::vector<int64_t>& seq_ids, const std::vector<int32_t>& tokens,
+                                          int max_blocks, int rows, const std::vector<float>& temperature,
+                                          const std::vector<int32_t>& top_k, const std::vector<float>& top_p,
+                                          const std::vector<int64_t>& counters, void* block) {
+  const size_t B = seq_ids.size();
+  if ((size_t)rows < B) throw std::invalid_argument("prepare_decode_packed: fewer rows than sequences");
+  if (temperature.size() != B || top_k.size() != B || top_p.size() != B || counters.size() != B)
+    throw std::invalid_argument("prepare_decode_packed: one sampling parameter set per sequence");
+  const DecodeStepLayout L = decode_step_layout(rows, max_blocks);
+  char* base = static_cast<char*>(block);
+  int32_t* ids = reinterpret_cast<int32_t*>(base + L.ids);
+  int32_t* pos = reinterpret_cast<int32_t*>(base + L.pos);
+  int64_t* slots = reinterpret_cast<int64_t*>(base + L.slots);
+  int32_t* ctx = reinterpret_cast<int32_t*>(base + L.ctx);
+  int32_t* order = reinterpret_cast<int32_t*>(base + L.order);
+  int32_t* bt = reinterpret_cast<int32_t*>(base + L.block_table);
+  const int fail = prepare_decode(seq_ids, tokens, max_blocks, ids, pos, slots, ctx, bt);
+  if (fail >= 0) return fail;
+  float* temp = reinterpret_cast<float*>(base + L.temperature);
+  int32_t* tk = reinterpret_cast<int32_t*>(base + L.top_k);
+  float* tp = reinterpret_cast<float*>(base + L.top_p);
+  int64_t* cnt = reinterpret_cast<int64_t*>(base + L.counters);
+  std::copy(temperature.begin(), temperature.end(), temp);
+  std::copy(top_k.begin(), top_k.end(), tk);
+  std::copy(top_p.begin(), top_p.end(), tp);
+  std::copy(counters.begin(), counters.end(), cnt);
+  std::fill(ids + B, ids + rows, 0);
+  std::fill(pos + B, pos + rows, 0);
+  std::fill(slots + B, slots + rows, (int64_t)-1);
+  std::fill(ctx + B, ctx + rows, 1);
+  std::fill(bt + B * (size_t)max_blocks, bt + rows * (size_t)max_blocks, 0);
+  std::fill(temp + B, temp + rows, 0.f);
+  std::fill(tk + B, tk + rows, 1);
+  std::fill(tp + B, tp + rows, 1.f);
+  std::fill(cnt + B, cnt + rows, (int64_t)0);
+  for (int i = 0; i < rows; ++i) order[i] = i;
+  std::stable_sort(order, order + rows, [ctx](int32_t a, int32_t b) { return ctx[a] > ctx[b]; });
+  return -1;
+}
+
 void KVBlockManager::block_table(const std::vector<int64_t>& seq_ids, int max_blocks, int32_t* out) const {
   for (size_t r = 0; r < seq_ids.size(); ++r) {
     int32_t* row = out + r * max_blocks;
diff --git a/django_assistant_bot_amd/csrc/runtime/kv_manager.h b/django_assistant_bot_amd/csrc/runtime/kv_manager.h
--- a/django_assistant_bot_amd/csrc/runtime/kv_manager.h
+++ b/django_assistant_bot_amd/csrc/runtime/kv_manager.h
@@ -5,6 +5,21 @@
 #include <vector>
 
 namespace dab {
+
+struct DecodeStepLayout {
+  int64_t ids;
+  int64_t pos;
+  int64_t slots;
+  int64_t ctx;
+  int64_t order;
+  int64_t block_table;
+  int64_t temperature;
+  int64_t top_k;
+  int64_t top_p;
+  int64_t counters;
+  int64_t bytes;
+};
+DecodeStepLayout decode_step_layout(int rows, int max_blocks);
 
 class KVBlockManager {
  public:
@@ -27,6 +42,9 @@
 
   int prepare_decode(const std::vector<int64_t>& seq_ids, const std::vector<int32_t>& tokens, int max_blocks,
                      int32_t* ids, int32_t* pos, int64_t* slots, int32_t* ctx, int32_t* block_table);
+  int prepare_decode_packed(const std::vector<int64_t>& seq_ids, const std::vector<int32_t>& tokens, int max_blocks,
+                            int rows, const std::vector<float>& temperature, const std::vector<int32_t>& top_k,
+                            const std::vector<float>& top_p, const std::vector<int64_t>& counters, void* block);
   void slot_mapping(int64_t seq_id, int start, int n, int64_t* out) const;
   void block_table(const std::vector<int64_t>& seq_ids, int max_blocks, int32_t* out) const;
 
diff --git a/django_assistant_bot_amd/engine/llm_engine.py b/django_assistant_bot_amd/engine/llm_engine.py
--- a/django_assistant_bot_amd/engine/llm_engine.py
+++ b/django_assistant_bot_amd/engine/llm_engine.py
@@ -6,6 +6,7 @@
 import time
 from collections import deque
 from dataclasses import dataclass, field
+from types import SimpleNamespace
 
 import numpy as np
 import torch
@@ -86,8 +87,8 @@
                  part_size: int = 512, kv_memory_fraction: float = 0.85, mixed_prefill_tokens: int = 0,
                  pipeline_decode: bool = True, shared_model: LlamaModel | None = None,
                  kv_cache_dtype: str | None = None, kv_scratch_blocks: int | None = None,
-                 weight_dtype: str | None = None):
-        self.cfg = decoder_config(model) if isinstance(model, str) else model
+                 weight_dtype: str | None = None, packed_step: bool = True, sampler_writes_ids: bool = False):
+        self.cfg =decoder_config(model) if isinstance(model, str) else model
         cfg = self.cfg
         if shared_model is not None:
             have = getattr(shared_model, "weight_dtype", "bf16")
@@ -185,19 +186,19 @@
         self.use_graphs = use_graphs and self.is_gpu
         dev = self.device
         mb = max_batch
-        self._d_ids = torch.zeros(mb, dtype=torch.int32, device=dev)
-        self._d_pos = torch.zeros(mb, dtype=torch.int32, device=dev)
-        self._d_slots = torch.full((mb,), -1, dtype=torch.int64, device=dev)
-        self._d_ctx = torch.ones(mb, dtype=torch.int32, device=dev)
-        self._d_bt = torch.zeros((mb, self.max_blocks_per_seq), dtype=torch.int32, device=dev)
-        self._d_temp = torch.ones(mb, dtype=torch.float32, device=dev)
-        self._d_topk = torch.full((mb,), 50, dtype=torch.int32, device=dev)
-        self._d_topp = torch.ones(mb, dtype=torch.float32, device=dev)
-        self._d_cnt = torch.zeros(mb, dtype=torch.int64, device=dev)
+        self.packed_step = bool(packed_step)
+        self._sampler_writes_ids = bool(sampler_writes_ids)
+        self._step_bytes = native().decode_step_layout(mb, self.max_blocks_per_seq)["bytes"]
+        self._d_block = torch.zeros(self._step_bytes, dtype=torch.uint8, device=dev)
+        self._d_views: dict = {}
+        v = self._dv(mb)
+        self._d_ctx, self._d_bt, self._d_order = v.ctx, v.bt, v.order
+        self._reset_step_inputs(mb)
         self._d_tokens = torch.zeros(mb, dtype=torch.int32, device=dev)
-        self._d_order = torch.arange(mb, dtype=torch.int32, device=dev)
         pin = self.is_gpu
         mk = lambda *a, **k: torch.zeros(*a, **k, pin_memory=pin)
+        self._h_block = mk(self._step_bytes, dtype=torch.uint8)
+        self._h_block_alt = mk(self._step_bytes, dtype=torch.uint8)
         self._h_ids = mk(mb, dtype=torch.int32)
         self._h_pos = mk(mb, dtype=torch.int32)
         self._h_slots = mk(mb, dtype=torch.int64)
@@ -723,6 +724,57 @@
             cur = getattr(self, k)
             setattr(self, k, alt)
             self._h_alt[k] = cur
+        self._h_block, self._h_block_alt = self._h_block_alt, self._h_block
+
+    @property
+    def sampler_writes_ids(self) -> bool:
+        return self._sampler_writes_ids
+
+    @sampler_writes_ids.setter
+    def sampler_writes_ids(self, on: bool) -> None:
+        if bool(on) != self._sampler_writes_ids:
+            if self._inflight is not None:
+                self._finish_inflight()
+            self._sampler_writes_ids = bool(on)
+            self._graphs.clear()
+
+    @staticmethod
+    def _step_views(block: torch.Tensor, rows: int, max_blocks: int) -> SimpleNamespace:
+        L = native().decode_step_layout(rows, max_blocks)
+
+        def sec(name, dtype, n):
+            o = L[name]
+            return block[o:o + n * torch.empty((), dtype=dtype).element_size()].view(dtype)
+
+        i32, i64, f32 = torch.int32, torch.int64, torch.float32
+        return SimpleNamespace(
+            ids=sec("ids", i32, rows), pos=sec("pos", i32, rows), slots=sec("slots", i64, rows),
+            ctx=sec("ctx", i32, rows), order=sec("order", i32, rows),
+            bt=sec("block_table", i32, rows * max_blocks).view(rows, max_blocks),
+            temp=sec("temperature", f32, rows), topk=sec("top_k", i32, rows), topp=sec("top_p", f32, rows),
+            cnt=sec("counters", i64, rows), lo=L["pos"], bytes=L["bytes"])
+
+    def _dv(self, rows: int) -> SimpleNamespace:
+        v = self._d_views.get(rows)
+        if v is None:
+            v = self._d_views[rows] = self._step_views(self._d_block, rows, self.max_blocks_per_seq)
+        return v
+
+    def _reset_step_inputs(self, rows: int) -> None:
+        v = self._dv(rows)
+        for t, val in ((v.ids, 0), (v.pos, 0), (v.slots, -1), (v.ctx, 1), (v.bt, 0), (v.temp, 1.0), (v.topk, 50),
+                       (v.topp, 1.0), (v.cnt, 0)):
+            t.fill_(val)
+        v.order.copy_(torch.arange(rows, dtype=torch.int32))
+
+    def _bucket(self, B: int) -> int:
+        return next(b for b in self._buckets if b >= B) if self.use_graphs else B
+
+    @staticmethod
+    def _sampling_lists(batch: list, pending: int = 0):
+        return ([r.params.temperature if r.params.do_sample else 0.0 for r in batch],
+                [r.params.top_k for r in batch], [r.params.top_p for r in batch],
+                [r.rng_base + len(r.out) + pending for r in batch])
 
     def _length_done(self, r: _Req, extra: int) -> bool:
         n, p = len(r.out) + extra, r.params
@@ -741,13 +793,18 @@
         launched = False
         if nxt:
             self._swap_host_buffers()
-            fail = self.blocks.prepare_decode_into(
-                [r.seq for r in nxt], [r.out[-1] if r.out else 0 for r in nxt], self.max_blocks_per_seq,
-                self._h_ids.data_ptr(), self._h_pos.data_ptr(), self._h_slots.data_ptr(), self._h_ctx.data_ptr(),
-                self._h_bt.data_ptr())
+            packed = self.packed_step
+            seqs, last = [r.seq for r in nxt], [r.out[-1] if r.out else 0 for r in nxt]
+            if packed:
+                fail = self.blocks.prepare_decode_packed(seqs, last, self.max_blocks_per_seq, self._bucket(len(nxt)),
+                                                         *self._sampling_lists(nxt, 1), self._h_block.data_ptr())
+            else:
+                fail = self.blocks.prepare_decode_into(
+                    seqs, last, self.max_blocks_per_seq, self._h_ids.data_ptr(), self._h_pos.data_ptr(),
+                    self._h_slots.data_ptr(), self._h_ctx.data_ptr(), self._h_bt.data_ptr())
             if fail < 0:
                 pos = {id(r): i for i, r in enumerate(prev["batch"])}
-                self._launch_decode(nxt, [pos[id(r)] for r in nxt], pending=1)
+                self._launch_decode(nxt, [pos[id(r)] for r in nxt], pending=1, packed=packed)
                 launched = True
             else:
                 self._swap_host_buffers()
@@ -756,42 +813,51 @@
         self._finish_inflight()
         self._inflight = cur
 
-    def _launch_decode(self, batch: list, src_rows, pending: int = 0):
+    def _launch_decode(self, batch: list, src_rows, pending: int = 0, packed: bool = False):
         t0 = time.perf_counter()
         B = len(batch)
-        self._h_temp[:B] = torch.tensor([r.params.temperature if r.params.do_sample else 0.0 for r in batch])
-        self._h_topk[:B] = torch.tensor([r.params.top_k for r in batch], dtype=torch.int32)
-        self._h_topp[:B] = torch.tensor([r.params.top_p for r in batch])
-        self._h_cnt[:B] = torch.tensor([r.rng_base + len(r.out) + pending for r in batch], dtype=torch.int64)
         self._fast = all((0 < r.params.top_k <= ops.kernels.SAMPLE_FAST_MAX_K) or not r.params.do_sample
                          or r.params.temperature <= 0 for r in batch)
-        Bp = next(b for b in self._buckets if b >= B) if self.use_graphs else B
-        if Bp > B:
-            self._h_ids[B:Bp] = 0
-            self._h_pos[B:Bp] = 0
-            self._h_slots[B:Bp] = -1
-            self._h_ctx[B:Bp] = 1
-            self._h_bt[B:Bp] = 0
-            self._h_temp[B:Bp] = 0.0
-            self._h_topk[B:Bp] = 1
-            self._h_topp[B:Bp] = 1.0
-            self._h_cnt[B:Bp] = 0
-        self._fill_order(Bp)
-        pairs = [(self._d_pos, self._h_pos), (self._d_slots, self._h_slots), (self._d_ctx, self._h_ctx),
-                 (self._d_temp, self._h_temp), (self._d_topk, self._h_topk), (self._d_topp, self._h_topp),
-                 (self._d_cnt, self._h_cnt), (self._d_bt, self._h_bt), (self._d_order, self._h_order)]
-        if src_rows is None:
-            pairs.append((self._d_ids, self._h_ids))
-        else:
+        Bp = self._bucket(B)
+        dv = self._dv(Bp)
+        if src_rows is not None:
             if src_rows == list(range(B)):
-                self._d_ids[:B].copy_(self._d_tokens[:B])
+                if not (self._inflight or {}).get("ids_written"):
+                    dv.ids[:B].copy_(self._d_tokens[:B])
+                    if Bp > B:
+                        dv.ids[B:Bp].zero_()
             else:
                 idx = torch.as_tensor(src_rows, dtype=torch.long).to(self.device, non_blocking=True)
-                self._d_ids[:B].copy_(self._d_tokens.index_select(0, idx))
+                dv.ids[:B].copy_(self._d_tokens.index_select(0, idx))
+                if Bp > B:
+                    dv.ids[B:Bp].zero_()
+        if packed:
+            lo = 0 if src_rows is None else dv.lo
+            self._d_block[lo:dv.bytes].copy_(self._h_block[lo:dv.bytes], non_blocking=True)
+        else:
+            temp, topk, topp, cnt = self._sampling_lists(batch, pending)
+            self._h_temp[:B] = torch.tensor(temp)
+            self._h_topk[:B] = torch.tensor(topk, dtype=torch.int32)
+            self._h_topp[:B] = torch.tensor(topp)
+            self._h_cnt[:B] = torch.tensor(cnt, dtype=torch.int64)
             if Bp > B:
-                self._d_ids[B:Bp].zero_()
-        for d, h in pairs:
-            d[:Bp].copy_(h[:Bp], non_blocking=True)
+                self._h_ids[B:Bp] = 0
+                self._h_pos[B:Bp] = 0
+                self._h_slots[B:Bp] = -1
+                self._h_ctx[B:Bp] = 1
+                self._h_bt[B:Bp] = 0
+                self._h_temp[B:Bp] = 0.0
+                self._h_topk[B:Bp] = 1
+                self._h_topp[B:Bp] = 1.0
+                self._h_cnt[B:Bp] = 0
+            self._fill_order(Bp)
+            pairs = [(dv.pos, self._h_pos), (dv.slots, self._h_slots), (dv.ctx, self._h_ctx),
+                     (dv.temp, self._h_temp), (dv.topk, self._h_topk), (dv.topp, self._h_topp),
+                     (dv.cnt, self._h_cnt), (dv.bt, self._h_bt), (dv.order, self._h_order)]
+            if src_rows is None:
+                pairs.append((dv.ids, self._h_ids))
+            for d, h in pairs:
+                d.copy_(h[:Bp], non_blocking=True)
         self._masked = False
         g = None
         if self.use_graphs:
@@ -809,7 +875,8 @@
             self._h_tokens[:Bp].copy_(self._d_tokens[:Bp], non_blocking=True)
             ev = torch.cuda.Event()
             ev.record()
-        self._inflight = {"batch": list(batch), "Bp": Bp, "tokens": self._h_tokens, "event": ev}
+        self._inflight = {"batch": list(batch), "Bp": Bp, "tokens": self._h_tokens, "event": ev,
+                          "ids_written": self._sampler_ids_out(dv) is not None}
         self.stats["decode_host_s"] = self.stats.get("decode_host_s", 0.0) + time.perf_counter() - t0
 
     def _finish_inflight(self):
@@ -858,7 +925,8 @@
         self._h_cnt[:B] = torch.tensor([r.rng_base + len(r.out) for r in batch], dtype=torch.int64)
         self._fast = all((0 < r.params.top_k <= ops.kernels.SAMPLE_FAST_MAX_K) or not r.params.do_sample
                          or r.params.temperature <= 0 for r in batch)
-        Bp = next(b for b in self._buckets if b >= B) if self.use_graphs else B
+        Bp = self._bucket(B)
+        dv = self._dv(Bp)
         if Bp > B:
             self._h_ids[B:Bp] = 0
             self._h_pos[B:Bp] = 0
@@ -870,11 +938,10 @@
             self._h_topp[B:Bp] = 1.0
             self._h_cnt[B:Bp] = 0
         self._fill_order(Bp)
-        for d, h in ((self._d_ids, self._h_ids), (self._d_pos, self._h_pos), (self._d_slots, self._h_slots),
-                     (self._d_ctx, self._h_ctx), (self._d_temp, self._h_temp), (self._d_topk, self._h_topk),
-                     (self._d_topp, self._h_topp), (self._d_cnt, self._h_cnt), (self._d_order, self._h_order)):
-            d[:Bp].copy_(h[:Bp], non_blocking=True)
-        self._d_bt[:Bp].copy_(self._h_bt[:Bp], non_blocking=True)
+        for d, h in ((dv.ids, self._h_ids), (dv.pos, self._h_pos), (dv.slots, self._h_slots),
+                     (dv.ctx, self._h_ctx), (dv.temp, self._h_temp), (dv.topk, self._h_topk),
+                     (dv.topp, self._h_topp), (dv.cnt, self._h_cnt), (dv.order, self._h_order), (dv.bt, self._h_bt)):
+            d.copy_(h[:Bp], non_blocking=True)
         self._masked = self._fill_masks(batch, Bp)
         t1 = time.perf_counter()
         g = None
@@ -890,8 +957,7 @@
                 self._decode_body(Bp)
         if self.is_gpu:
             if self.vp and self._fast:
-                self._vp_merge(self._vp_cand[:, :Bp], self._d_temp[:Bp], self._d_topk[:Bp], self._d_topp[:Bp],
-                               self._d_cnt[:Bp], out=self._d_tokens[:Bp])
+                self._vp_merge(self._vp_cand[:, :Bp], dv.temp, dv.topk, dv.topp, dv.cnt, out=self._d_tokens[:Bp])
             else:
                 self._tp_sync_tokens(self._d_tokens[:Bp])
             self._h_tokens[:Bp].copy_(self._d_tokens[:Bp], non_blocking=True)
@@ -918,11 +984,15 @@
         hkv = self.cfg.kv_heads // self.tp_size
         return self.long_part_size if Bp * hkv >= 512 else self.part_size
 
+    def _sampler_ids_out(self, dv):
+        return dv.ids if self._sampler_writes_ids and self.is_gpu and not self.vp else None
+
     def _decode_body(self, Bp: int):
-        meta = AttnMeta(decode=True, positions=self._d_pos[:Bp], slots=self._d_slots[:Bp],
-                        block_tables=self._d_bt[:Bp], ctx_lens=self._d_ctx[:Bp], workspace=self._workspace,
-                        part_size=self._decode_part(Bp), order=self._d_order[:Bp] if self.is_gpu else None)
-        h = self.model.forward(self._d_ids[:Bp], meta, self.kv)
+        dv = self._dv(Bp)
+        meta = AttnMeta(decode=True, positions=dv.pos, slots=dv.slots, block_tables=dv.bt, ctx_lens=dv.ctx,
+                        workspace=self._workspace, part_size=self._decode_part(Bp),
+                        order=dv.order if self.is_gpu else None)
+        h = self.model.forward(dv.ids, meta, self.kv)
         logits = self.model.logits(h)
         if self._masked:
             self._mask(logits, Bp)
@@ -931,26 +1001,27 @@
         elif self.is_gpu:
             if self.vp:
                 logits = self.model.full_logits(logits)
-            ops.sample_tokens(logits, self._d_temp[:Bp], self._d_topk[:Bp], self._d_topp[:Bp], self.seed,
-                              self._d_cnt[:Bp], out=self._d_tokens[:Bp], fast=self._fast,
-                              workspace=self._sample_ws)
+            ops.sample_tokens(logits, dv.temp, dv.topk, dv.topp, self.seed, dv.cnt, out=self._d_tokens[:Bp],
+                              fast=self._fast, workspace=self._sample_ws, ids_out=self._sampler_ids_out(dv))
         else:
             if self.vp:
                 logits = self.model.full_logits(logits)
-            g = torch.Generator().manual_seed(int(self.seed * 7919 + int(self._h_cnt[0])))
-            self._d_tokens[:Bp] = ops.sample_tokens(logits, self._d_temp[:Bp], self._d_topk[:Bp], self._d_topp[:Bp],
-                                                    self.seed, self._d_cnt[:Bp], generator=g)
+            g = torch.Generator().manual_seed(int(self.seed * 7919 + int(dv.cnt[0])))
+            self._d_tokens[:Bp] = ops.sample_tokens(logits, dv.temp, dv.topk, dv.topp, self.seed, dv.cnt, generator=g)
             self._h_tokens[:Bp] = self._d_tokens[:Bp]
 
     def _capture(self, Bp: int):
         try:
+            dv = self._dv(Bp)
+            ids0, cnt0 = dv.ids.clone(), dv.cnt.clone()
             s = torch.cuda.Stream(self.device)
             s.wait_stream(torch.cuda.current_stream(self.device))
             with torch.cuda.stream(s):
                 self._decode_body(Bp)
             torch.cuda.current_stream(self.device).wait_stream(s)
             torch.cuda.synchronize(self.device)
-            self._d_cnt[:Bp].copy_(self._h_cnt[:Bp])
+            dv.cnt.copy_(cnt0)
+            dv.ids.copy_(ids0)
             g = torch.cuda.CUDAGraph()
             if self._graph_pool is None:
                 self._graph_pool = torch.cuda.graph_pool_handle()
@@ -971,4 +1042,5 @@
         self._masked = False
         for b in sizes or self._buckets:
             if (b, True, False) not in self._graphs:
+                self._reset_step_inputs(b)
                 self._capture(b)
diff --git a/django_assistant_bot_amd/ops/kernels.py b/django_assistant_bot_amd/ops/kernels.py
--- a/django_assistant_bot_amd/ops/kernels.py
+++ b/django_assistant_bot_amd/ops/kernels.py
@@ -882,8 +882,17 @@
     return torch.empty((rows * ncand * 8,), dtype=torch.uint8, device=device)
 
 
+def _ids_out_ptr(ids_out, out, rows: int) -> int:
+    if ids_out is None:
+        return 0
+    expect(ids_out.dtype == torch.int32 and ids_out.is_contiguous() and ids_out.numel() >= rows
+           and ids_out.device == out.device, "ids_out: contiguous int32 [>= rows] on the sampler's device")
+    expect(ids_out.data_ptr() != out.data_ptr(), "ids_out must not be the token output itself")
+    return ptr(ids_out)
+
+
 def sample_tokens(logits, temperature, top_k, top_p, seed: int, counters, generator=None, out=None,
-                  fast: bool | None = None, workspace: torch.Tensor | None = None):
+                  fast: bool | None = None, workspace: torch.Tensor | None = None, ids_out=None):
     if not logits.is_cuda:
         return ref.sample_hf(logits, temperature, top_k, top_p, generator)
     rows, vocab = logits.shape
@@ -894,6 +903,7 @@
     _i32(top_k)
     expect(counters.dtype == torch.int64 and counters.numel() >= rows, "counters")
     out = torch.empty((rows,), dtype=torch.int32, device=logits.device) if out is None else out
+    ids2 = _ids_out_ptr(ids_out, out, rows)
     if fast is None:
         fast = False
     ncand = -(-vocab // _CHUNK) * SAMPLE_FAST_MAX_K
@@ -902,11 +912,11 @@
         expect(ws.numel() >= rows * ncand * 8, "sampling workspace too small")
         native().sample_tokens_2stage(ptr(logits), int(logits.dtype == torch.float32), logits.stride(0), rows, vocab,
                                       ptr(temperature), ptr(top_k), ptr(top_p), int(seed) & ((1 << 64) - 1),
-                                      ptr(counters), ptr(out), ptr(ws), ws.numel(), stream(logits))
+                                      ptr(counters), ptr(out), ptr(ws), ws.numel(), stream(logits), ids2)
     else:
         native().sample_tokens(ptr(logits), int(logits.dtype == torch.float32), logits.stride(0), rows, vocab,
                                ptr(temperature), ptr(top_k), ptr(top_p), int(seed) & ((1 << 64) - 1), ptr(counters),
-                               ptr(out), 0, stream(logits))
+                               ptr(out), 0, stream(logits), ids2)
     return out
 
 
@@ -947,14 +957,15 @@
     return -(-int(vocab) // _CHUNK) * SAMPLE_FAST_MAX_K
 
 
-def sample_merge(cands, temperature, top_k, top_p, seed: int, counters, vocab: int, out=None):
+def sample_merge(cands, temperature, top_k, top_p, seed: int, counters, vocab: int, out=None, ids_out=None):
     two, rows, n = cands.shape
     expect(two == 2 and n <= 1024 and cands.dtype == torch.int32 and cands.is_contiguous(),
            "candidates: contiguous int32 [2, rows, <= 1024]")
     out = torch.empty((rows,), dtype=torch.int32, device=cands.device) if out is None else out
     _i32(top_k)
     native().sample_merge(ptr(cands[0]), ptr(cands[1]), n, rows, int(vocab), ptr(temperature), ptr(top_k), ptr(top_p),
-                          int(seed) & ((1 << 64) - 1), ptr(counters), ptr(out), stream(cands))
+                          int(seed) & ((1 << 64) - 1), ptr(counters), ptr(out), stream(cands),
+                          _ids_out_ptr(ids_out, out, rows))
     return out
 
 
```

Result: no change. 40.27 queries/s, median of 6 (+0.1%).
